# OFA-Sys/ONE-PEACE

Measured on AMD Instinct MI355X. Metric: pretrain samples/s (tri-modal global batch) ONE-PEACE-4B, higher is better.
Workload: dtype bf16

## Files before the change

include/onepeace_hip.h:

```cpp
#ifndef ONEPEACE_HIP_H
#define ONEPEACE_HIP_H

#include <stdint.h>

#ifdef __cplusplus
extern "C" {
#endif

int op_abi_version(void);
const char* op_last_error(void);

int op_prof_enable(int on);
int op_prof_reserve(int events);
int op_prof_collect(double* ms, int64_t* count, double* work, int n_families);

int op_layernorm_fwd(const void* x, const void* w, const void* b, void* y, float* mean, float* rstd, int64_t rows,
                     int64_t cols, float eps, int act_gelu, int dtype, const int* x_rows, void* stream);
int64_t op_layernorm_bwd_workspace_bytes(int64_t rows, int64_t cols);
int op_layernorm_bwd(const void* dy, const void* x, const void* w, const void* b, const float* mean, const float* rstd,
                     const void* add, void* dx, void* dw, void* db, void* workspace, int64_t rows, int64_t cols,
                     int act_gelu, int accumulate, int dtype, const int* x_rows, void* stream);

int op_gemm_nt(const void* A, int64_t lda, const void* B0, const void* B1, const void* B2, int64_t ldb, int64_t n_seg,
               const void* bias0, const void* bias1, const void* bias2, void* C, int64_t ldc, void* h0, void* h1,
               const void* resid, int64_t ldr, const void* gamma, const float* rowscale, int64_t rows_per_sample,
               const float* alpha, int64_t M, int64_t N, int64_t K, int epilogue, void* workspace, int64_t workspace_bytes,
               int64_t tune, const int* resid_rows, int64_t resid_rows_total, void* stream);
int op_gemm_tn(const void* A, int64_t lda, const void* B, int64_t ldb, void* C, int64_t ldc, int64_t M, int64_t N, int64_t K,
               int accumulate, void* workspace, int64_t workspace_bytes, int64_t tune, void* stream);
int op_gemm_nt_grouped(int64_t nprob, const void* const* A, const int64_t* M, int64_t lda, const void* const* B, int64_t ldb,
                       const void* const* bias, void* const* C, int64_t ldc, void* const* h0, void* const* h1,
                       const void* const* resid, int64_t ldr, const void* const* gamma, const float* const* rowscale,
                       const int64_t* rows_per_sample, int64_t N, int64_t K, int epilogue, int64_t tune, const int* const* resid_rows,
                       int64_t resid_rows_total, void* stream);
int op_gemm_nt_batched(const void* A, int64_t lda, int64_t stride_a, const void* W, int64_t ldb, int64_t stride_b, const void* bias,
                       int64_t stride_bias, void* C, int64_t ldc, int64_t stride_c, int64_t M, int64_t N, int64_t K, int64_t batch,
                       void* stream);
int op_audio_conv1_ln_gelu_fwd(const void* wav, int64_t stride, const void* w0, const void* b0, const void* lnw, const void* lnb, void* y,
                               float* mean, float* rstd, int64_t rows, int64_t C, float eps, void* stream);
int64_t op_audio_conv1_ln_gelu_bwd_workspace_bytes(int64_t C);
int op_audio_conv1_ln_gelu_bwd(const void* dy, const void* wav, int64_t stride, const void* w0, const void* b0, const void* lnw, const void* lnb,
                               const float* mean, const float* rstd, void* dw0, void* db0, void* dlnw, void* dlnb, void* workspace,
                               int64_t rows, int64_t C, int accumulate, void* stream);
int64_t op_gemm_tn_grouped_counter_bytes(void);
int64_t op_gemm_tn_grouped_plan(int64_t nprob, const int64_t* M, const int64_t* N, const int64_t* K, int64_t workgroups, int64_t tune,
                                int32_t* out, int64_t cap);
int op_gemm_tn_grouped(int64_t nprob, const void* const* A, const int64_t* lda, const void* const* B, const int64_t* ldb, void* const* C,
                       const int64_t* ldc, const int64_t* M, const int64_t* N, const int64_t* K, const int32_t* accumulate,
                       const void* const* W, const int64_t* ldw, float* const* rowdot, const void* const* rscale, void* counters,
                       int64_t tune, void* stream);
int op_gemm_tn_grouped_lists(int64_t nprob, const void* const* A, const int64_t* lda, const void* const* B, const int64_t* ldb, void* const* C,
                             const int64_t* ldc, const int64_t* M, const int64_t* N, const int64_t* K, const int32_t* accumulate,
                             const void* const* W, const int64_t* ldw, float* const* rowdot, const void* const* rscale,
                             const int32_t* const* ktiles, const int32_t* const* n_ktiles, void* counters, int64_t tune, void* stream);
int op_live_ktiles(int64_t nseg, const float* const* ps, const int64_t* row0, const int64_t* S, const int64_t* B, int64_t nprob,
                   const int64_t* prob_row0, const int64_t* prob_rows, int32_t* const* ktiles, int32_t* const* n_ktiles, void* stream);
int op_gemm_plan(int64_t M, int64_t N, int64_t K, int epilogue, int has_bias, int64_t workspace_bytes, int64_t tune, int* plan);

int op_quant_fp8_rows(const void* x, int64_t ldx, void* q, int64_t ldq, float* scale, int64_t rows, int64_t cols, void* stream);
int op_layernorm_fwd_q8(const void* x, const void* w, const void* b, void* y, float* mean, float* rstd, void* q8, float* q8_scale,
                        int64_t rows, int64_t cols, float eps, void* stream);
int op_ln_geglu_fwd_q8(const void* h0, const void* h1, int64_t ldh, const void* w, const void* b, void* y, float* mean, float* rstd, void* q8,
                       float* q8_scale, int64_t rows, int64_t cols, float eps, void* stream);
int op_gemm_nt_fp8(const void* A8, int64_t lda, const float* sa, const void* B0, const void* B1, int64_t ldb, const float* sb0,
                   const float* sb1, const void* bias, void* C, int64_t ldc, void* h0, void* h1, const void* resid, int64_t ldr,
                   const void* gamma, const float* rowscale, int64_t rows_per_sample, int64_t M, int64_t N, int64_t K, int epilogue,
                   int64_t tune, void* stream);

int op_attn_fwd(const void* q, const void* k, const void* v, int64_t ld, const void* bias, int64_t bias_batch_stride,
                const void* bias_frag, const void* key_pad, void* out, int64_t ldo, float* lse, int64_t lse_ld, int64_t B,
                int64_t S, int64_t Spad, int64_t heads, int64_t head_dim, float scale, int64_t tune, void* stream);
int64_t op_attn_bias_frag_elems(int64_t n_img, int64_t S);
int op_attn_bias_pack(const void* src, void* dst, int64_t n_img, int64_t S, int64_t Spad, void* stream);
int op_attn_bwd_delta(const void* dout, const void* out, int64_t ldo, float* delta, int64_t B, int64_t S, int64_t Spad,
                      int64_t heads, void* stream);
int64_t op_attn_bwd_dbias_slabs(int64_t B, int64_t S, int64_t heads, int64_t tune);
int op_attn_bwd(const void* q, const void* k, const void* v, int64_t ld, const void* dout, const void* out, int64_t ldo,
                const void* bias, const void* biasT, const void* bias_frag, int64_t bias_batch_stride, const void* key_pad,
                const float* lse, float* delta, void* dq,
                void* dk, void* dv, int64_t ldg, float* dbias, int64_t B, int64_t S, int64_t Spad, int64_t heads,
                int64_t head_dim, float scale, int64_t tune, void* stream);

int op_relpos_bias_build(const void* table, const int* bucket, int64_t bucket_ld, void* out, int64_t heads, int64_t S,
                         int64_t Spad, int transposed, void* stream);
int op_relpos_bias_bwd(const float* dbias, int64_t S, int64_t Spad, const int* pos, const int* seg, int64_t nseg, const int* bucket_seg,
                       int64_t num_rel, float* partial_ws, float* dtable, int64_t heads, void* stream);
int op_relpos_bias_build_ids(const void* table, const int* bucket, int64_t bucket_ld, const int* ids, void* out, int64_t B,
                             int64_t heads, int64_t K, int64_t Kpad, int transposed, void* stream);
int op_relpos_bias_fold_ids(const float* dbias, const int* ids, float* dense_ws, int64_t Sfull, int64_t B, int64_t heads, int64_t K,
                            int64_t Kpad, void* stream);

int op_transpose(const void* in, void* out, int64_t rows, int64_t cols, int64_t ld_in, int64_t ld_out, void* stream);
int op_transpose_scaled(const void* in, void* out, int64_t rows, int64_t cols, int64_t ld_in, int64_t ld_out, const void* scale,
                        void* stream);
int op_transpose_batched(const void* table, int64_t n, int64_t total_tiles, void* stream);
int64_t op_transpose_desc_bytes(void);
int64_t op_colsum_workspace_bytes(int64_t N);
int op_colsum_segments(const void* x, void* out0, void* out1, void* out2, void* workspace, int64_t M, int64_t n_seg,
                       int64_t seg_cols, int accumulate, void* stream);
int64_t op_resid_bwd_workspace_bytes(int64_t N);
int op_resid_bwd(const void* dout, const void* y, const void* gamma, const float* rowscale, int64_t rows_per_sample,
                 void* dbranch, void* dgamma, void* dbias, float* g0, void* workspace, int64_t M, int64_t N, int accumulate,
                 const int* dout_rows, void* stream);
int op_gamma_grad_finish(const float* rowdot, int64_t slots, const void* b0, const float* g00, const void* b1, const float* g01,
                         const void* b2, const float* g02, void* dgamma, int64_t N, int accumulate, void* stream);
int op_ln_geglu_bwd(const void* dy, const void* h0, const void* h1, const void* w, const float* mean, const float* rstd,
                    void* dh0, void* dh1, int64_t ldd, int64_t ldh, void* dw, void* db, void* workspace, int64_t rows,
                    int64_t cols, int accumulate, void* stream);
int op_ln_geglu_fwd(const void* h0, const void* h1, int64_t ldh, const void* w, const void* b, void* y, float* mean, float* rstd,
                    int64_t rows, int64_t cols, float eps, void* stream);
int op_colsum(const void* x, const void* y, const float* rowscale, int64_t rows_per_sample, const void* mul, void* out,
              void* workspace, int64_t M, int64_t N, int accumulate, int out_dtype, void* stream);
int op_geglu_bwd(const void* dg, const void* h0, const void* h1, void* dh0, void* dh1, int64_t numel, void* stream);
int op_scale_rows(const void* dout, const void* gamma, const float* rowscale, int64_t rows_per_sample, void* dbranch,
                  int64_t M, int64_t N, void* stream);

int op_l2norm_fwd(const void* x, void* y, float* inv_norm, int64_t rows, int64_t cols, float eps, int out_dtype, void* stream);
int op_l2norm_bwd(const void* dy, const void* y, const float* inv_norm, void* dx, int64_t rows, int64_t cols, int y_dtype,
                  void* stream);
int op_infonce_rows(float* sim, int64_t rows, int64_t n, int64_t ld, int64_t target0, float label_smoothing, float gscale,
                    float* row_loss, float* row_hit, float* row_dot, int write_grad, void* stream);

int op_adamw_step(void* p, const void* g, float* m, float* v, int64_t numel, float lr, float beta1, float beta2, float eps,
                  float weight_decay, int64_t step, float grad_scale, const float* grad_sqnorm, float clip_norm,
                  void* stream);
int op_adamw_step_groups(void* p, const void* g, float* m, float* v, int64_t numel, const int64_t* group_end8,
                         const float* group_lr_scale, const float* group_weight_decay, int64_t n_groups, float lr, float beta1,
                         float beta2, float eps, int64_t step, float grad_scale, const float* grad_sqnorm, float clip_norm,
                         void* stream);
int op_sqnorm(const void* x, int64_t numel, float* workspace, float* out, void* stream);

int op_rows_gather(const void* src, void* dst, const int* list, int64_t nseg, const int64_t* src_row0, const int64_t* dst_row0,
                   const int64_t* S, const int64_t* n_kept, const int64_t* dst_rows, const int64_t* n_samples, const int64_t* list_off,
                   int64_t dst_total, int64_t cols, void* stream);
int op_rows_merge(const void* base, const void* upd, void* out, const int* list, int64_t nseg, const int64_t* src_row0,
                  const int64_t* dst_row0, const int64_t* S, const int64_t* n_kept, const int64_t* dst_rows, const int64_t* n_samples,
                  const int64_t* list_off, int64_t total, int64_t cols, void* stream);
int op_rows_map(int* map, const int* list, int64_t nseg, const int64_t* src_row0, const int64_t* dst_row0, const int64_t* S,
                const int64_t* n_kept, const int64_t* dst_rows, const int64_t* n_samples, const int64_t* list_off, int64_t dst_total,
                void* stream);

int64_t op_sim_topk_splits(int64_t M, int64_t N, int64_t splits);
int64_t op_sim_topk_workspace_bytes(int64_t M, int64_t N, int64_t k, int64_t splits);
int op_sim_topk(const void* Q, int64_t ldq, const void* G, int64_t ldg, int64_t M, int64_t N, int64_t D, int64_t k, float* vals, int* idx,
                void* workspace, int64_t workspace_bytes, int64_t splits, void* stream);

int op_image_resize_normalize(const void* src, int64_t src_bytes, const int64_t* desc, const int64_t* desc_host, int64_t B,
                              const int* coef, int64_t coef_count, int64_t S, const float* mean, const float* stdev, void* out,
                              int out_dtype, void* workspace, int64_t workspace_bytes, void* stream);

int op_audio_normalize_pad(const void* src, int64_t src_bytes, const int64_t* desc, const int64_t* desc_host, int64_t B, int64_t max_len,
                           int64_t min_len, void* out, int64_t T, int out_dtype, void* workspace, int64_t workspace_bytes, void* stream);

int op_audio_resample(const void* src, int64_t src_bytes, const int64_t* desc, const int64_t* desc_host, int64_t B, const float* coef,
                      int64_t coef_count, void* out, int64_t out_bytes, void* stream);

int64_t op_average_precision_workspace_bytes(int64_t N, int64_t C);
int op_average_precision(const float* scores, int64_t ld_scores, const uint8_t* targets, int64_t ld_targets, int64_t N, int64_t C,
                         double* ap, int* npos, void* workspace, int64_t workspace_bytes, void* stream);

int op_row_loss(const void* logits, int dtype, int64_t ld, const void* targets, int target_dtype, int64_t ld_targets, int64_t B, int64_t C,
                int mode, float label_smoothing, float margin, float gscale, float* row_loss, float* row_correct, float* dlogits,
                float* sums, void* stream);
int op_box_loss(const void* logits, int dtype, const float* targets, int64_t B, float gscale, float* out, float* dlogits, void* stream);

#ifdef __cplusplus
}
#endif
#endif
```

one-peace_amd/csrc/layernorm.hip:

```cpp
#include "common.h"

namespace {

constexpr int LN_MAX_BLOCKS = 4096;
constexpr int g_ln_blocks_fwd = 512, g_ln_blocks_bwd = 512;
#ifndef OP_LN_GEGLU_BLOCKS_FWD
#define OP_LN_GEGLU_BLOCKS_FWD 2048
#endif
#ifndef OP_LN_GEGLU_BLOCKS_BWD
#define OP_LN_GEGLU_BLOCKS_BWD 512
#endif

template <int NW>
__device__ __forceinline__ float group_sum(float v, float* red) {
  v = wave_sum(v);
  if (NW == 1) return v;
  const int wid = threadIdx.x >> 6;
  __syncthreads();
  if ((threadIdx.x & 63) == 0) red[wid] = v;
  __syncthreads();
  float t = 0.f;
#pragma unroll
  for (int i = 0; i < NW; ++i) t += red[i];
  return t;
}

template <int NW>
__device__ __forceinline__ void group_sum2(float& a, float& b, float* red) {
  a = wave_sum(a);
  b = wave_sum(b);
  if (NW == 1) return;
  const int wid = threadIdx.x >> 6;
  __syncthreads();
  if ((threadIdx.x & 63) == 0) { red[wid] = a; red[NW + wid] = b; }
  __syncthreads();
  float ta = 0.f, tb = 0.f;
#pragma unroll
  for (int i = 0; i < NW; ++i) { ta += red[i]; tb += red[NW + i]; }
  a = ta;
  b = tb;
}

template <int NW>
__device__ __forceinline__ float group_amax(int m, float* red) {
  const float v = fp8_wave_amax(m);
  if (NW == 1) return v;
  const int wid = threadIdx.x >> 6;
  __syncthreads();
  if ((threadIdx.x & 63) == 0) red[wid] = v;
  __syncthreads();
  int t = __float_as_int(red[0]);
#pragma unroll
  for (int i = 1; i < NW; ++i) t = max(t, __float_as_int(red[i]));
  return __int_as_float(t);
}

template <typename T, int CH, int NW, bool GELU, bool NT, bool Q8 = false>
__global__ __launch_bounds__(256) void ln_fwd_kernel(const T* __restrict__ x, const T* __restrict__ w,
                                                     const T* __restrict__ b, T* __restrict__ y,
                                                     float* __restrict__ mean_out, float* __restrict__ rstd_out,
                                                     int64_t rows, int cols, float eps, uint8_t* __restrict__ q8 = nullptr,
                                                     float* __restrict__ q8_scale = nullptr, const int* __restrict__ xmap = nullptr) {
  __shared__ float red[4];
  constexpr int G = 64 * NW;
  const int tig = (NW == 1) ? (threadIdx.x & 63) : threadIdx.x;
  const int64_t row0 = (NW == 1) ? ((int64_t)blockIdx.x * 4 + (threadIdx.x >> 6)) : blockIdx.x;
  const int64_t rstep = (NW == 1) ? (int64_t)gridDim.x * 4 : gridDim.x;
  const float inv = 1.0f / (float)cols;

  float wv[CH][8], bv[CH][8];
#pragma unroll
  for (int i = 0; i < CH; ++i) {
    const int c = (tig + G * i) * 8;
#pragma unroll
    for (int j = 0; j < 8; ++j) { wv[i][j] = 1.f; bv[i][j] = 0.f; }
    if (c < cols) {
      if (w) Vec8<T>::load(w + c, wv[i]);
      if (b) Vec8<T>::load(b + c, bv[i]);
    }
  }
  typedef typename Vec8<T>::raw_t raw_t;
  raw_t cur[CH], nxt[CH];
  auto fetch = [&](int64_t src, raw_t (&dst)[CH]) {
#pragma unroll
    for (int i = 0; i < CH; ++i) {
      const int c = (tig + G * i) * 8;
      if (c < cols) {
        if (src >= 0) dst[i] = ldraw_sel<T, NT>(x + src * (int64_t)cols + c);
        else dst[i] = raw_t{};
      }
    }
  };
  int64_t nsrc = row0 + rstep < rows ? (xmap ? (int64_t)xmap[row0 + rstep] : row0 + rstep) : -1;
  if (row0 < rows) fetch(xmap ? (int64_t)xmap[row0] : row0, cur);
  for (int64_t row = row0; row < rows; row += rstep) {
    const int64_t nrow = row + rstep, nnrow = nrow + rstep;
    if (nrow < rows) fetch(nsrc, nxt);
    if (nnrow < rows) nsrc = xmap ? (int64_t)xmap[nnrow] : nnrow;
    float v[CH][8];
    float s = 0.f;
#pragma unroll
    for (int i = 0; i < CH; ++i) {
      const int c = (tig + G * i) * 8;
      if (c < cols) {
        Vec8<T>::cvt(cur[i], v[i]);
#pragma unroll
        for (int j = 0; j < 8; ++j) s += v[i][j];
      } else {
#pragma unroll
        for (int j = 0; j < 8; ++j) v[i][j] = 0.f;
      }
    }
    const float mean = group_sum<NW>(s, red) * inv;
    float ss = 0.f;
#pragma unroll
    for (int i = 0; i < CH; ++i) {
      const int c = (tig + G * i) * 8;
      if (c < cols) {
#pragma unroll
        for (int j = 0; j < 8; ++j) { const float d = v[i][j] - mean; ss += d * d; }
      }
    }
    const float rstd = rsqrtf(group_sum<NW>(ss, red) * inv + eps);
    T* yr = y + row * (int64_t)cols;
    int amax = 0;
#pragma unroll
    for (int i = 0; i < CH; ++i) {
      const int c = (tig + G * i) * 8;
      if (c < cols) {
        float o[8];
#pragma unroll
        for (int j = 0; j < 8; ++j) {
          float t = (v[i][j] - mean) * rstd * wv[i][j] + bv[i][j];
          o[j] = GELU ? gelu_erf(t) : t;
        }
        store_sel<T, NT>(yr + c, o);
        if constexpr (Q8) {
#pragma unroll
          for (int j = 0; j < 8; ++j) { v[i][j] = (float)(T)o[j]; amax = fp8_amax_acc(amax, v[i][j]); }
        }
      }
    }
    if constexpr (Q8) {
      float qinv;
      const float sc = fp8_row_scale(group_amax<NW>(amax, red), qinv);
      uint8_t* qr = q8 + row * (int64_t)cols;
#pragma unroll
      for (int i = 0; i < CH; ++i) {
        const int c = (tig + G * i) * 8;
        if (c < cols) *reinterpret_cast<u32x2*>(qr + c) = fp8_pack8(v[i], qinv);
      }
      if (tig == 0) q8_scale[row] = sc;
    }
    if (tig == 0) {
      if (mean_out) mean_out[row] = mean;
      if (rstd_out) rstd_out[row] = rstd;
    }
#pragma unroll
    for (int i = 0; i < CH; ++i) cur[i] = nxt[i];
  }
}

template <int CH, int NW, bool Q8 = false>
__global__ __launch_bounds__(NW == 1 ? 256 : 64 * NW) void ln_geglu_fwd_kernel(const bf16_t* __restrict__ h0, const bf16_t* __restrict__ h1,
                                                           int64_t ldh, const bf16_t* __restrict__ w, const bf16_t* __restrict__ b,
                                                           bf16_t* __restrict__ y, float* __restrict__ mean_out,
                                                           float* __restrict__ rstd_out, int64_t rows, int cols, float eps,
                                                           uint8_t* __restrict__ q8 = nullptr, float* __restrict__ q8_scale = nullptr) {
  __shared__ float red[4];
  constexpr int G = 64 * NW;
  const int tig = (NW == 1) ? (threadIdx.x & 63) : threadIdx.x;
  const int64_t row0 = (NW == 1) ? ((int64_t)blockIdx.x * 4 + (threadIdx.x >> 6)) : blockIdx.x;
  const int64_t rstep = (NW == 1) ? (int64_t)gridDim.x * 4 : gridDim.x;
  const float inv = 1.0f / (float)cols;
  float wv[CH][8], bv[CH][8];
#pragma unroll
  for (int i = 0; i < CH; ++i) {
    const int c = (tig + G * i) * 8;
#pragma unroll
    for (int j = 0; j < 8; ++j) { wv[i][j] = 1.f; bv[i][j] = 0.f; }
    if (c < cols) {
      if (w) Vec8<bf16_t>::load(w + c, wv[i]);
      if (b) Vec8<bf16_t>::load(b + c, bv[i]);
    }
  }
  bf16x8 c0[CH], c1[CH], n0[CH], n1[CH];
  if (row0 < rows) {
#pragma unroll
    for (int i = 0; i < CH; ++i) {
      const int c = (tig + G * i) * 8;
      if (c < cols) {
        c0[i] = Vec8<bf16_t>::ldraw_nt(h0 + row0 * ldh + c);
        c1[i] = Vec8<bf16_t>::ldraw_nt(h1 + row0 * ldh + c);
      }
    }
  }
  for (int64_t row = row0; row < rows; row += rstep) {
    const int64_t nrow = row + rstep;
    if (nrow < rows) {
#pragma unroll
      for (int i = 0; i < CH; ++i) {
        const int c = (tig + G * i) * 8;
        if (c < cols) {
          n0[i] = Vec8<bf16_t>::ldraw_nt(h0 + nrow * ldh + c);
          n1[i] = Vec8<bf16_t>::ldraw_nt(h1 + nrow * ldh + c);
        }
      }
    }
    float v[CH][8];
    float s = 0.f;
#pragma unroll
    for (int i = 0; i < CH; ++i) {
      const int c = (tig + G * i) * 8;
      if (c < cols) {
        float a[8], bb[8];
        Vec8<bf16_t>::cvt(c0[i], a);
        Vec8<bf16_t>::cvt(c1[i], bb);
#pragma unroll
        for (int j = 0; j < 8; ++j) {
          v[i][j] = (float)(bf16_t)(gelu_erf(a[j]) * bb[j]);
          s += v[i][j];
        }
      } else {
#pragma unroll
        for (int j = 0; j < 8; ++j) v[i][j] = 0.f;
      }
    }
    const float mean = group_sum<NW>(s, red) * inv;
    float ss = 0.f;
#pragma unroll
    for (int i = 0; i < CH; ++i) {
      const int c = (tig + G * i) * 8;
      if (c < cols) {
#pragma unroll
        for (int j = 0; j < 8; ++j) { const float d = v[i][j] - mean; ss += d * d; }
      }
    }
    const float rstd = rsqrtf(group_sum<NW>(ss, red) * inv + eps);
    bf16_t* yr = y + row * (int64_t)cols;
    int amax = 0;
#pragma unroll
    for (int i = 0; i < CH; ++i) {
      const int c = (tig + G * i) * 8;
      if (c < cols) {
        float o[8];
#pragma unroll
        for (int j = 0; j < 8; ++j) o[j] = (v[i][j] - mean) * rstd * wv[i][j] + bv[i][j];
        Vec8<bf16_t>::store_nt(yr + c, o);
        if constexpr (Q8) {
#pragma unroll
          for (int j = 0; j < 8; ++j) { v[i][j] = (float)(bf16_t)o[j]; amax = fp8_amax_acc(amax, v[i][j]); }
        }
      }
    }
    if constexpr (Q8) {
      float qinv;
      const float sc = fp8_row_scale(group_amax<NW>(amax, red), qinv);
      uint8_t* qr = q8 + row * (int64_t)cols;
#pragma unroll
      for (int i = 0; i < CH; ++i) {
        const int c = (tig + G * i) * 8;
        if (c < cols) *reinterpret_cast<u32x2*>(qr + c) = fp8_pack8(v[i], qinv);
      }
      if (tig == 0) q8_scale[row] = sc;
    }
    if (tig == 0) {
      if (mean_out) mean_out[row] = mean;
      if (rstd_out) rstd_out[row] = rstd;
    }
#pragma unroll
    for (int i = 0; i < CH; ++i) { c0[i] = n0[i]; c1[i] = n1[i]; }
  }
}

template <typename T, int CH, int NW, bool GELU, bool NT>
__global__ __launch_bounds__(256) void ln_bwd_kernel(const T* __restrict__ dy, const T* __restrict__ x,
                                                     const T* __restrict__ w, const T* __restrict__ b,
                                                     const float* __restrict__ mean_in,
                                                     const float* __restrict__ rstd_in, const T* __restrict__ add,
                                                     T* __restrict__ dx, float* __restrict__ ws, int64_t rows, int cols,
                                                     const int* __restrict__ xmap = nullptr) {
  extern __shared__ __attribute__((aligned(16))) float smem[];
  float* red = smem;
  constexpr int G = 64 * NW;
  const int tig = (NW == 1) ? (threadIdx.x & 63) : threadIdx.x;
  const int wid = threadIdx.x >> 6;
  const int64_t row0 = (NW == 1) ? ((int64_t)blockIdx.x * 4 + wid) : blockIdx.x;
  const int64_t rstep = (NW == 1) ? (int64_t)gridDim.x * 4 : gridDim.x;
  const float inv = 1.0f / (float)cols;

  float wv[CH][8], bv[CH][8], dwa[CH][8], dba[CH][8];
#pragma unroll
  for (int i = 0; i < CH; ++i) {
    const int c = (tig + G * i) * 8;
#pragma unroll
    for (int j = 0; j < 8; ++j) { wv[i][j] = 1.f; bv[i][j] = 0.f; dwa[i][j] = 0.f; dba[i][j] = 0.f; }
    if (c < cols) {
      if (w) Vec8<T>::load(w + c, wv[i]);
      if (GELU && b) Vec8<T>::load(b + c, bv[i]);
    }
  }
  typedef typename Vec8<T>::raw_t raw_t;
  raw_t curx[CH], curg[CH], nxtx[CH], nxtg[CH], addv[CH];
  int64_t src = row0 < rows ? (xmap ? (int64_t)xmap[row0] : row0) : -1;
  int64_t nsrc = row0 + rstep < rows ? (xmap ? (int64_t)xmap[row0 + rstep] : row0 + rstep) : -1, nnsrc = -1;
  if (row0 < rows) {
#pragma unroll
    for (int i = 0; i < CH; ++i) {
      const int c = (tig + G * i) * 8;
      if (c < cols) {
        if (src >= 0) curx[i] = ldraw_sel<T, NT>(x + src * (int64_t)cols + c);
        else curx[i] = raw_t{};
        curg[i] = ldraw_sel<T, NT>(dy + row0 * (int64_t)cols + c);
      }
    }
  }
  for (int64_t row = row0; row < rows; row += rstep) {
    const float mean = mean_in[row], rstd = rstd_in[row];
    const int64_t nrow = row + rstep, nnrow = nrow + rstep;
    if (nnrow < rows) nnsrc = xmap ? (int64_t)xmap[nnrow] : nnrow;
#pragma unroll
    for (int i = 0; i < CH; ++i) {
      const int c = (tig + G * i) * 8;
      if (c < cols) {
        if (add && src >= 0) addv[i] = ldraw_sel<T, NT>(add + src * (int64_t)cols + c);
        if (nrow < rows) {
          if (nsrc >= 0) nxtx[i] = ldraw_sel<T, NT>(x + nsrc * (int64_t)cols + c);
          else nxtx[i] = raw_t{};
          nxtg[i] = ldraw_sel<T, NT>(dy + nrow * (int64_t)cols + c);
        }
      }
    }
    float xh[CH][8], g[CH][8];
    float s1 = 0.f, s2 = 0.f;
#pragma unroll
    for (int i = 0; i < CH; ++i) {
      const int c = (tig + G * i) * 8;
      if (c < cols) {
        Vec8<T>::cvt(curx[i], xh[i]);
        Vec8<T>::cvt(curg[i], g[i]);
#pragma unroll
        for (int j = 0; j < 8; ++j) {
          xh[i][j] = (xh[i][j] - mean) * rstd;
          if (GELU) g[i][j] *= gelu_erf_grad(xh[i][j] * wv[i][j] + bv[i][j]);
          dwa[i][j] += g[i][j] * xh[i][j];
          dba[i][j] += g[i][j];
          const float gw = g[i][j] * wv[i][j];
          g[i][j] = gw;
          s1 += gw;
          s2 += gw * xh[i][j];
        }
      }
    }
    group_sum2<NW>(s1, s2, red);
    const float c1 = s1 * inv, c2 = s2 * inv;
    T* dr = dx + (src >= 0 ? src : 0) * (int64_t)cols;
#pragma unroll
    for (int i = 0; i < CH; ++i) {
      const int c = (tig + G * i) * 8;
      if (c < cols && src >= 0) {
        float o[8];
#pragma unroll
        for (int j = 0; j < 8; ++j) o[j] = rstd * (g[i][j] - c1 - xh[i][j] * c2);
        if (add) {
          float av[8];
          Vec8<T>::cvt(addv[i], av);
#pragma unroll
          for (int j = 0; j < 8; ++j) o[j] += av[j];
        }
        store_sel<T, NT>(dr + c, o);
      }
    }
#pragma unroll
    for (int i = 0; i < CH; ++i) { curx[i] = nxtx[i]; curg[i] = nxtg[i]; }
    src = nsrc;
    nsrc = nnsrc;
  }
  if (ws == nullptr) return;
  float* wsb = ws + (int64_t)blockIdx.x * 2 * cols;
  if (NW == 1) {
#pragma unroll
    for (int pass = 0; pass < 2; ++pass) {
      __syncthreads();
#pragma unroll
      for (int i = 0; i < CH; ++i) {
        const int c = (tig + G * i) * 8;
        if (c < cols) {
#pragma unroll
          for (int j = 0; j < 8; ++j) smem[wid * cols + c + j] = pass == 0 ? dwa[i][j] : dba[i][j];
        }
      }
      __syncthreads();
      for (int c = threadIdx.x; c < cols; c += 256)
        wsb[pass * cols + c] = smem[c] + smem[cols + c] + smem[2 * cols + c] + smem[3 * cols + c];
    }
  } else {
#pragma unroll
    for (int i = 0; i < CH; ++i) {
      const int c = (tig + G * i) * 8;
      if (c < cols) {
#pragma unroll
        for (int j = 0; j < 8; ++j) { wsb[c + j] = dwa[i][j]; wsb[cols + c + j] = dba[i][j]; }
      }
    }
  }
}

template <int CH, int NW>
__global__ __launch_bounds__(NW == 1 ? 256 : 64 * NW) void ln_geglu_bwd_kernel(const bf16_t* __restrict__ dy, const bf16_t* __restrict__ h0,
                                                           const bf16_t* __restrict__ h1, const bf16_t* __restrict__ w,
                                                           const float* __restrict__ mean_in,
                                                           const float* __restrict__ rstd_in, bf16_t* __restrict__ dh0,
                                                           bf16_t* __restrict__ dh1, int64_t ldd, int64_t ldh, float* __restrict__ ws,
                                                           int64_t rows, int cols) {
  extern __shared__ __attribute__((aligned(16))) float smem[];
  float* red = smem;
  constexpr int G = 64 * NW;
  const int tig = (NW == 1) ? (threadIdx.x & 63) : threadIdx.x;
  const int wid = threadIdx.x >> 6;
  const int64_t row0 = (NW == 1) ? ((int64_t)blockIdx.x * 4 + wid) : blockIdx.x;
  const int64_t rstep = (NW == 1) ? (int64_t)gridDim.x * 4 : gridDim.x;
  const float inv = 1.0f / (float)cols;
  float dwa[CH][8], dba[CH][8];
  bf16x8 wraw[CH];
#pragma unroll
  for (int i = 0; i < CH; ++i) {
    const int c = (tig + G * i) * 8;
#pragma unroll
    for (int j = 0; j < 8; ++j) { dwa[i][j] = 0.f; dba[i][j] = 0.f; }
#pragma unroll
    for (int j = 0; j < 8; ++j) wraw[i][j] = (bf16_t)1.0f;
    if (c < cols && w) wraw[i] = Vec8<bf16_t>::ldraw(w + c);
  }
  bf16x8 r0[CH], r1[CH], rg[CH], n0[CH], n1[CH], ng[CH];
  if (row0 < rows) {
#pragma unroll
    for (int i = 0; i < CH; ++i) {
      const int c = (tig + G * i) * 8;
      if (c < cols) {
        r0[i] = Vec8<bf16_t>::ldraw_nt(h0 + row0 * ldh + c);
        r1[i] = Vec8<bf16_t>::ldraw_nt(h1 + row0 * ldh + c);
        rg[i] = Vec8<bf16_t>::ldraw_nt(dy + row0 * (int64_t)cols + c);
      }
    }
  }
  for (int64_t row = row0; row < rows; row += rstep) {
    const float mean = mean_in[row], rstd = rstd_in[row];
    const int64_t base = row * (int64_t)cols;
    const int64_t nrow = row + rstep;
    if (nrow < rows) {
#pragma unroll
      for (int i = 0; i < CH; ++i) {
        const int c = (tig + G * i) * 8;
        if (c < cols) {
          n0[i] = Vec8<bf16_t>::ldraw_nt(h0 + nrow * ldh + c);
          n1[i] = Vec8<bf16_t>::ldraw_nt(h1 + nrow * ldh + c);
          ng[i] = Vec8<bf16_t>::ldraw_nt(dy + nrow * (int64_t)cols + c);
        }
      }
    }
    float gw[CH][8], cdfs[CH][8], gps[CH][8];
    float s1 = 0.f, s2 = 0.f;
#pragma unroll
    for (int i = 0; i < CH; ++i) {
      const int c = (tig + G * i) * 8;
      if (c < cols) {
        float a[8], b[8];
        Vec8<bf16_t>::cvt(r0[i], a);
        Vec8<bf16_t>::cvt(r1[i], b);
        Vec8<bf16_t>::cvt(rg[i], gw[i]);
        float wv[8];
        asm volatile("" : "+v"(wraw[i]));
        Vec8<bf16_t>::cvt(wraw[i], wv);
#pragma unroll
        for (int j = 0; j < 8; ++j) {
          float cdf, pdf;
          gelu_parts(a[j], cdf, pdf);
          cdfs[i][j] = cdf;
          gps[i][j] = cdf + a[j] * pdf;
          const float gval = (float)(bf16_t)(a[j] * cdf * b[j]);
          const float xh = (gval - mean) * rstd;
          const float d = gw[i][j];
          dwa[i][j] += d * xh;
          dba[i][j] += d;
          const float t = d * wv[j];
          gw[i][j] = t;
          s1 += t;
          s2 += t * xh;
        }
      }
    }
    group_sum2<NW>(s1, s2, red);
    const float c1 = s1 * inv, c2 = s2 * inv;
#pragma unroll
    for (int i = 0; i < CH; ++i) {
      const int c = (tig + G * i) * 8;
      if (c < cols) {
        float a[8], b[8], o0[8], o1[8];
        Vec8<bf16_t>::cvt(r0[i], a);
        Vec8<bf16_t>::cvt(r1[i], b);
#pragma unroll
        for (int j = 0; j < 8; ++j) {
          const float ge = a[j] * cdfs[i][j];
          const float xh = ((float)(bf16_t)(ge * b[j]) - mean) * rstd;
          const float dg = rstd * (gw[i][j] - c1 - xh * c2);
          o0[j] = dg * b[j] * gps[i][j];
          o1[j] = dg * ge;
        }
        Vec8<bf16_t>::store_nt(dh0 + row * ldd + c, o0);
        Vec8<bf16_t>::store_nt(dh1 + row * ldd + c, o1);
      }
    }
#pragma unroll
    for (int i = 0; i < CH; ++i) { r0[i] = n0[i]; r1[i] = n1[i]; rg[i] = ng[i]; }
  }
  if (ws == nullptr) return;
  float* wsb = ws + (int64_t)blockIdx.x * 2 * cols;
  if (NW == 1) {
#pragma unroll
    for (int pass = 0; pass < 2; ++pass) {
      __syncthreads();
#pragma unroll
      for (int i = 0; i < CH; ++i) {
        const int c = (tig + G * i) * 8;
        if (c < cols) {
#pragma unroll
          for (int j = 0; j < 8; ++j) smem[wid * cols + c + j] = pass == 0 ? dwa[i][j] : dba[i][j];
        }
      }
      __syncthreads();
      for (int c = threadIdx.x; c < cols; c += 256)
        wsb[pass * cols + c] = smem[c] + smem[cols + c] + smem[2 * cols + c] + smem[3 * cols + c];
    }
  } else {
#pragma unroll
    for (int i = 0; i < CH; ++i) {
      const int c = (tig + G * i) * 8;
      if (c < cols) {
#pragma unroll
        for (int j = 0; j < 8; ++j) { wsb[c + j] = dwa[i][j]; wsb[cols + c + j] = dba[i][j]; }
      }
    }
  }
}

inline int ln_grid(int64_t rows, int nw, int cap) {
  int64_t blocks = nw == 1 ? (rows + 3) / 4 : rows;
  if (blocks > cap) blocks = cap;
  if (blocks < 1) blocks = 1;
  return (int)blocks;
}

template <typename T, bool GELU>
int ln_fwd_dispatch(const void* x, const void* w, const void* b, void* y, float* mean, float* rstd, int64_t rows,
                    int cols, float eps, hipStream_t s, const int* xmap = nullptr) {
  const T* X = (const T*)x; const T* W = (const T*)w; const T* B = (const T*)b; T* Y = (T*)y;
  const bool nt = mean != nullptr && (int64_t)rows * cols * (int64_t)sizeof(T) >= ((int64_t)64 << 20);
#define LN_F(CH, NW)                                                                                                                      \
  do {                                                                                                                                    \
    if (nt) hipLaunchKernelGGL((ln_fwd_kernel<T, CH, NW, GELU, true>), dim3(ln_grid(rows, NW, g_ln_blocks_fwd)), dim3(256), 0, s, X, W, B, Y, mean, rstd, rows, cols, eps, (uint8_t*)nullptr, (float*)nullptr, xmap); \
    else hipLaunchKernelGGL((ln_fwd_kernel<T, CH, NW, GELU, false>), dim3(ln_grid(rows, NW, g_ln_blocks_fwd)), dim3(256), 0, s, X, W, B, Y, mean, rstd, rows, cols, eps, (uint8_t*)nullptr, (float*)nullptr, xmap); \
  } while (0)
  if (cols <= 512) LN_F(1, 1);
  else if (cols <= 1024) LN_F(2, 1);
  else if (cols <= 1536) LN_F(3, 1);
  else if (cols <= 2048) LN_F(4, 1);
  else if (cols <= 4096) LN_F(2, 4);
  else if (cols <= 6144) LN_F(3, 4);
  else if (cols <= 8192) LN_F(4, 4);
  else { op_set_error("layernorm: cols %d > 8192 unsupported", cols); return OP_ENOTSUP; }
#undef LN_F
  OP_LAUNCH_CHECK();
  return OP_OK;
}

template <typename T, bool GELU>
int ln_bwd_dispatch(const void* dy, const void* x, const void* w, const void* b, const float* mean, const float* rstd,
                    const void* add, void* dx, void* dw, void* db, float* ws, int64_t rows, int cols, int accumulate,
                    hipStream_t s, const int* xmap = nullptr) {
  const T* DY = (const T*)dy; const T* X = (const T*)x; const T* W = (const T*)w; const T* B = (const T*)b; T* DX = (T*)dx;
  const T* ADD = (const T*)add;
  int grid = 0;
  float* wsk = (dw || db) ? ws : nullptr;
  const bool nt = (int64_t)rows * cols * (int64_t)sizeof(T) >= ((int64_t)64 << 20);
#define LN_B(CH, NW)                                                                                        \
  do {                                                                                                      \
    grid = ln_grid(rows, NW, g_ln_blocks_bwd);                                                                               \
    size_t sh = (NW == 1) ? (size_t)4 * cols * sizeof(float) : 64;                                          \
    if (nt) hipLaunchKernelGGL((ln_bwd_kernel<T, CH, NW, GELU, true>), dim3(grid), dim3(256), sh, s, DY, X, W, B, mean,   \
                       rstd, ADD, DX, wsk, rows, cols, xmap);                                                    \
    else hipLaunchKernelGGL((ln_bwd_kernel<T, CH, NW, GELU, false>), dim3(grid), dim3(256), sh, s, DY, X, W, B, mean,   \
                       rstd, ADD, DX, wsk, rows, cols, xmap);                                                    \
  } while (0)
  if (cols <= 512) LN_B(1, 1);
  else if (cols <= 1024) LN_B(2, 1);
  else if (cols <= 1536) LN_B(3, 1);
  else if (cols <= 2048) LN_B(4, 1);
  else if (cols <= 4096) LN_B(2, 4);
  else if (cols <= 6144) LN_B(3, 4);
  else if (cols <= 8192) LN_B(4, 4);
  else { op_set_error("layernorm: cols %d > 8192 unsupported", cols); return OP_ENOTSUP; }
#undef LN_B
  OP_LAUNCH_CHECK();
  if (wsk) {
    hipLaunchKernelGGL((partials_reduce3_kernel<T>), dim3(ceil_div(cols, 32), 2), dim3(256), 0, s, ws, ws + cols,
                       (const float*)nullptr, (const bf16_t*)nullptr, (const bf16_t*)nullptr, (const bf16_t*)nullptr, (T*)dw,
                       (T*)db, (T*)nullptr, grid, (int64_t)2 * cols, cols, accumulate);
    OP_LAUNCH_CHECK();
  }
  return OP_OK;
}

}

extern "C" {


int64_t op_layernorm_bwd_workspace_bytes(int64_t rows, int64_t cols) {
  (void)rows;
  return (int64_t)LN_MAX_BLOCKS * 2 * cols * (int64_t)sizeof(float);
}

int op_layernorm_fwd(const void* x, const void* w, const void* b, void* y, float* mean, float* rstd, int64_t rows,
                     int64_t cols, float eps, int act_gelu, int dtype, const int* x_rows, void* stream) {
  OP_CHECK_ARG(x && y, "layernorm_fwd: null x/y");
  OP_CHECK_ARG(rows >= 0 && cols > 0 && cols % 8 == 0, "layernorm_fwd: cols=%lld must be a positive multiple of 8",
               (long long)cols);
  if (rows == 0) return OP_OK;
  hipStream_t s = (hipStream_t)stream;
  if (dtype == OP_DT_BF16)
    return act_gelu ? ln_fwd_dispatch<bf16_t, true>(x, w, b, y, mean, rstd, rows, (int)cols, eps, s, x_rows)
                    : ln_fwd_dispatch<bf16_t, false>(x, w, b, y, mean, rstd, rows, (int)cols, eps, s, x_rows);
  if (dtype == OP_DT_F32)
    return act_gelu ? ln_fwd_dispatch<float, true>(x, w, b, y, mean, rstd, rows, (int)cols, eps, s, x_rows)
                    : ln_fwd_dispatch<float, false>(x, w, b, y, mean, rstd, rows, (int)cols, eps, s, x_rows);
  op_set_error("layernorm_fwd: bad dtype %d", dtype);
  return OP_EINVAL;
}

int op_layernorm_fwd_q8(const void* x, const void* w, const void* b, void* y, float* mean, float* rstd, void* q8, float* q8_scale,
                        int64_t rows, int64_t cols, float eps, void* stream) {
  OP_CHECK_ARG(x && y && q8 && q8_scale, "layernorm_fwd_q8: null pointer");
  OP_CHECK_ARG(rows >= 0 && cols > 0 && cols % 8 == 0 && cols <= 8192, "layernorm_fwd_q8: cols=%lld unsupported", (long long)cols);
  if (rows == 0) return OP_OK;
  hipStream_t s = (hipStream_t)stream;
#define LN_Q(CH, NW)                                                                                                                         \
  hipLaunchKernelGGL((ln_fwd_kernel<bf16_t, CH, NW, false, false, true>), dim3(ln_grid(rows, NW, g_ln_blocks_fwd)), dim3(256), 0, s,        \
                     (const bf16_t*)x, (const bf16_t*)w, (const bf16_t*)b, (bf16_t*)y, mean, rstd, rows, (int)cols, eps, (uint8_t*)q8, q8_scale)
  if (cols <= 512) LN_Q(1, 1);
  else if (cols <= 1024) LN_Q(2, 1);
  else if (cols <= 1536) LN_Q(3, 1);
  else if (cols <= 2048) LN_Q(4, 1);
  else if (cols <= 4096) LN_Q(2, 4);
  else if (cols <= 6144) LN_Q(3, 4);
  else LN_Q(4, 4);
#undef LN_Q
  OP_LAUNCH_CHECK();
  return OP_OK;
}

int op_layernorm_bwd(const void* dy, const void* x, const void* w, const void* b, const float* mean, const float* rstd,
                     const void* add, void* dx, void* dw, void* db, void* workspace, int64_t rows, int64_t cols,
                     int act_gelu, int accumulate, int dtype, const int* x_rows, void* stream) {
  OP_CHECK_ARG(dy && x && dx && mean && rstd, "layernorm_bwd: null pointer");
  OP_CHECK_ARG(rows >= 0 && cols > 0 && cols % 8 == 0, "layernorm_bwd: cols=%lld must be a positive multiple of 8",
               (long long)cols);
  OP_CHECK_ARG(!(dw || db) || workspace, "layernorm_bwd: dw/db requested without workspace");
  if (rows == 0) return OP_OK;
  hipStream_t s = (hipStream_t)stream;
  if (dtype == OP_DT_BF16)
    return act_gelu ? ln_bwd_dispatch<bf16_t, true>(dy, x, w, b, mean, rstd, add, dx, dw, db, (float*)workspace, rows,
                                                    (int)cols, accumulate, s, x_rows)
                    : ln_bwd_dispatch<bf16_t, false>(dy, x, w, b, mean, rstd, add, dx, dw, db, (float*)workspace, rows,
                                                     (int)cols, accumulate, s, x_rows);
  if (dtype == OP_DT_F32)
    return act_gelu ? ln_bwd_dispatch<float, true>(dy, x, w, b, mean, rstd, add, dx, dw, db, (float*)workspace, rows,
                                                   (int)cols, accumulate, s, x_rows)
                    : ln_bwd_dispatch<float, false>(dy, x, w, b, mean, rstd, add, dx, dw, db, (float*)workspace, rows,
                                                    (int)cols, accumulate, s, x_rows);
  op_set_error("layernorm_bwd: bad dtype %d", dtype);
  return OP_EINVAL;
}

int op_ln_geglu_fwd(const void* h0, const void* h1, int64_t ldh, const void* w, const void* b, void* y, float* mean, float* rstd,
                    int64_t rows, int64_t cols, float eps, void* stream) {
  OP_CHECK_ARG(h0 && h1 && y, "ln_geglu_fwd: null pointer");
  if (ldh <= 0) ldh = cols;
  OP_CHECK_ARG(rows >= 0 && cols > 0 && cols % 8 == 0 && cols <= 8192 && ldh >= cols && ldh % 8 == 0, "ln_geglu_fwd: cols=%lld ldh=%lld unsupported",
               (long long)cols, (long long)ldh);
  if (rows == 0) return OP_OK;
  hipStream_t s = (hipStream_t)stream;
#define LNG_F(CH, NW)                                                                                                       \
  hipLaunchKernelGGL((ln_geglu_fwd_kernel<CH, NW>), dim3(ln_grid(rows, NW, OP_LN_GEGLU_BLOCKS_FWD)), dim3(NW == 1 ? 256 : 64 * NW), 0, s, \
                     (const bf16_t*)h0, (const bf16_t*)h1, ldh, (const bf16_t*)w, (const bf16_t*)b, (bf16_t*)y, mean, rstd, rows, \
                     (int)cols, eps)
  if (cols <= 512) LNG_F(1, 1);
  else if (cols <= 1024) LNG_F(2, 1);
  else if (cols <= 1536) LNG_F(3, 1);
  else if (cols <= 2048) LNG_F(4, 1);
  else if (cols <= 4096) LNG_F(2, 4);
  else if (cols <= 6144) LNG_F(3, 4);
  else LNG_F(4, 4);
#undef LNG_F
  OP_LAUNCH_CHECK();
  return OP_OK;
}

int op_ln_geglu_fwd_q8(const void* h0, const void* h1, int64_t ldh, const void* w, const void* b, void* y, float* mean, float* rstd, void* q8,
                       float* q8_scale, int64_t rows, int64_t cols, float eps, void* stream) {
  OP_CHECK_ARG(h0 && h1 && y && q8 && q8_scale, "ln_geglu_fwd_q8: null pointer");
  if (ldh <= 0) ldh = cols;
  OP_CHECK_ARG(rows >= 0 && cols > 0 && cols % 8 == 0 && cols <= 8192 && ldh >= cols && ldh % 8 == 0, "ln_geglu_fwd_q8: cols=%lld ldh=%lld unsupported",
               (long long)cols, (long long)ldh);
  if (rows == 0) return OP_OK;
  hipStream_t s = (hipStream_t)stream;
#define LNG_Q(CH, NW)                                                                                                       \
  hipLaunchKernelGGL((ln_geglu_fwd_kernel<CH, NW, true>), dim3(ln_grid(rows, NW, OP_LN_GEGLU_BLOCKS_FWD)), dim3(NW == 1 ? 256 : 64 * NW), 0, s, \
                     (const bf16_t*)h0, (const bf16_t*)h1, ldh, (const bf16_t*)w, (const bf16_t*)b, (bf16_t*)y, mean, rstd, rows, \
                     (int)cols, eps, (uint8_t*)q8, q8_scale)
  if (cols <= 512) LNG_Q(1, 1);
  else if (cols <= 1024) LNG_Q(2, 1);
  else if (cols <= 1536) LNG_Q(3, 1);
  else if (cols <= 2048) LNG_Q(4, 1);
  else if (cols <= 4096) LNG_Q(2, 4);
  else if (cols <= 6144) LNG_Q(3, 4);
  else LNG_Q(4, 4);
#undef LNG_Q
  OP_LAUNCH_CHECK();
  return OP_OK;
}

int op_ln_geglu_bwd(const void* dy, const void* h0, const void* h1, const void* w, const float* mean, const float* rstd,
                    void* dh0, void* dh1, int64_t ldd, int64_t ldh, void* dw, void* db, void* workspace, int64_t rows, int64_t cols,
                    int accumulate, void* stream) {
  OP_CHECK_ARG(dy && h0 && h1 && dh0 && dh1 && mean && rstd, "ln_geglu_bwd: null pointer");
  if (ldd <= 0) ldd = cols;
  if (ldh <= 0) ldh = cols;
  OP_CHECK_ARG(ldd >= cols && ldd % 8 == 0 && ldh >= cols && ldh % 8 == 0, "ln_geglu_bwd: row strides %lld / %lld", (long long)ldd, (long long)ldh);
  OP_CHECK_ARG(rows >= 0 && cols > 0 && cols % 8 == 0 && cols <= 8192, "ln_geglu_bwd: cols=%lld unsupported", (long long)cols);
  OP_CHECK_ARG(!(dw || db) || workspace, "ln_geglu_bwd: dw/db requested without workspace");
  if (rows == 0) return OP_OK;
  hipStream_t s = (hipStream_t)stream;
  float* wsk = (dw || db) ? (float*)workspace : nullptr;
  int grid = 0;
#define LNG_B(CH, NW)                                                                                              \
  do {                                                                                                             \
    grid = ln_grid(rows, NW, OP_LN_GEGLU_BLOCKS_BWD);                                                                     \
    size_t sh = (NW == 1) ? (size_t)4 * cols * sizeof(float) : 64;                                                 \
    hipLaunchKernelGGL((ln_geglu_bwd_kernel<CH, NW>), dim3(grid), dim3(NW == 1 ? 256 : 64 * NW), sh, s,           \
                       (const bf16_t*)dy, (const bf16_t*)h0, (const bf16_t*)h1, (const bf16_t*)w, mean, rstd,      \
                       (bf16_t*)dh0, (bf16_t*)dh1, ldd, ldh, wsk, rows, (int)cols);                                \
  } while (0)
  if (cols <= 512) LNG_B(1, 1);
  else if (cols <= 1024) LNG_B(2, 1);
  else if (cols <= 1536) LNG_B(3, 1);
  else if (cols <= 2048) LNG_B(4, 1);
  else if (cols <= 4096) LNG_B(2, 4);
  else if (cols <= 6144) LNG_B(3, 4);
  else LNG_B(4, 4);
#undef LNG_B
  OP_LAUNCH_CHECK();
  if (wsk) {
    hipLaunchKernelGGL((partials_reduce3_kernel<bf16_t>), dim3(ceil_div(cols, 32), 2), dim3(256), 0, s, wsk, wsk + cols,
                       (const float*)nullptr, (const bf16_t*)nullptr, (const bf16_t*)nullptr, (const bf16_t*)nullptr,
                       (bf16_t*)dw, (bf16_t*)db, (bf16_t*)nullptr, grid, (int64_t)2 * cols, (int)cols, accumulate);
    OP_LAUNCH_CHECK();
  }
  return OP_OK;
}

}
```

one-peace_amd/hip.py:

```python
import ctypes
import os
from ctypes import c_double, c_float, c_int, c_int64, c_void_p

import torch

_HERE = os.path.dirname(os.path.abspath(__file__))
LIB_PATH = os.environ.get("ONEPEACE_HIP_LIB") or os.path.join(_HERE, "lib", "libonepeace_hip.so")
_lib = None

DT_BF16, DT_F32 = 0, 1
EPI_BIAS, EPI_F32, EPI_GEGLU, EPI_RESID = 0, 1, 2, 3
PROF_GEMM, PROF_ATTN = 0, 1
ATTN_RESIDENT_MAX_S = 320

P = c_void_p
I64 = c_int64

SIGNATURES = {
    "op_abi_version": (c_int, []),
    "op_last_error": (ctypes.c_char_p, []),
    "op_prof_enable": (c_int, [c_int]),
    "op_prof_reserve": (c_int, [c_int]),
    "op_prof_collect": (c_int, [P, P, P, c_int]),
    "op_layernorm_fwd": (c_int, [P, P, P, P, P, P, I64, I64, c_float, c_int, c_int, P, P]),
    "op_layernorm_bwd_workspace_bytes": (I64, [I64, I64]),
    "op_attn_bwd_dbias_slabs": (I64, [I64, I64, I64, I64]),
    "op_layernorm_bwd": (c_int, [P, P, P, P, P, P, P, P, P, P, P, I64, I64, c_int, c_int, c_int, P, P]),
    "op_gemm_plan": (c_int, [c_int64, c_int64, c_int64, c_int, c_int, c_int64, I64, P]),
    "op_gemm_nt": (c_int, [P, I64, P, P, P, I64, I64, P, P, P, P, I64, P, P, P, I64, P, P, I64, P, I64, I64, I64,
                           c_int, P, I64, I64, P, I64, P]),
    "op_gemm_nt_grouped": (c_int, [I64, P, P, I64, P, I64, P, P, I64, P, P, P, I64, P, P, P, I64, I64, c_int, I64, P, I64, P]),
    "op_gemm_tn": (c_int, [P, I64, P, I64, P, I64, I64, I64, I64, c_int, P, I64, I64, P]),
    "op_gemm_tn_grouped_counter_bytes": (I64, []),
    "op_gemm_tn_grouped_plan": (I64, [I64, P, P, P, I64, I64, P, I64]),
    "op_gemm_tn_grouped": (c_int, [I64, P, P, P, P, P, P, P, P, P, P, P, P, P, P, P, I64, P]),
    "op_gemm_tn_grouped_lists": (c_int, [I64, P, P, P, P, P, P, P, P, P, P, P, P, P, P, P, P, P, I64, P]),
    "op_live_ktiles": (c_int, [I64, P, P, P, P, I64, P, P, P, P, P]),
    "op_gemm_nt_batched": (c_int, [P, I64, I64, P, I64, I64, P, I64, P, I64, I64, I64, I64, I64, I64, P]),
    "op_audio_conv1_ln_gelu_fwd": (c_int, [P, I64, P, P, P, P, P, P, P, I64, I64, c_float, P]),
    "op_audio_conv1_ln_gelu_bwd_workspace_bytes": (I64, [I64]),
    "op_audio_conv1_ln_gelu_bwd": (c_int, [P, P, I64, P, P, P, P, P, P, P, P, P, P, P, I64, I64, c_int, P]),
    "op_transpose": (c_int, [P, P, I64, I64, I64, I64, P]),
    "op_transpose_scaled": (c_int, [P, P, I64, I64, I64, I64, P, P]),
    "op_transpose_batched": (c_int, [P, I64, I64, P]),
    "op_transpose_desc_bytes": (I64, []),
    "op_colsum_workspace_bytes": (I64, [I64]),
    "op_colsum_segments": (c_int, [P, P, P, P, P, I64, I64, I64, c_int, P]),
    "op_resid_bwd_workspace_bytes": (I64, [I64]),
    "op_resid_bwd": (c_int, [P, P, P, P, I64, P, P, P, P, P, I64, I64, c_int, P, P]),
    "op_gamma_grad_finish": (c_int, [P, I64, P, P, P, P, P, P, P, I64, c_int, P]),
    "op_ln_geglu_bwd": (c_int, [P, P, P, P, P, P, P, P, I64, I64, P, P, P, I64, I64, c_int, P]),
    "op_ln_geglu_fwd": (c_int, [P, P, I64, P, P, P, P, P, I64, I64, c_float, P]),
    "op_colsum": (c_int, [P, P, P, I64, P, P, P, I64, I64, c_int, c_int, P]),
    "op_geglu_bwd": (c_int, [P, P, P, P, P, I64, P]),
    "op_scale_rows": (c_int, [P, P, P, I64, P, I64, I64, P]),
    "op_l2norm_fwd": (c_int, [P, P, P, I64, I64, c_float, c_int, P]),
    "op_l2norm_bwd": (c_int, [P, P, P, P, I64, I64, c_int, P]),
    "op_infonce_rows": (c_int, [P, I64, I64, I64, I64, c_float, c_float, P, P, P, c_int, P]),
    "op_adamw_step": (c_int, [P, P, P, P, I64, c_float, c_float, c_float, c_float, c_float, I64, c_float, P, c_float, P]),
    "op_adamw_step_groups": (c_int, [P, P, P, P, I64, P, P, P, I64, c_float, c_float, c_float, c_float, I64, c_float, P, c_float, P]),
    "op_sqnorm": (c_int, [P, I64, P, P, P]),
    "op_relpos_bias_build": (c_int, [P, P, I64, P, I64, I64, I64, c_int, P]),
    "op_relpos_bias_bwd": (c_int, [P, I64, I64, P, P, I64, P, I64, P, P, I64, P]),
    "op_relpos_bias_build_ids": (c_int, [P, P, I64, P, P, I64, I64, I64, I64, c_int, P]),
    "op_relpos_bias_fold_ids": (c_int, [P, P, P, I64, I64, I64, I64, I64, P]),
    "op_attn_fwd": (c_int, [P, P, P, I64, P, I64, P, P, P, I64, P, I64, I64, I64, I64, I64, I64, c_float, I64, P]),
    "op_attn_bias_frag_elems": (I64, [I64, I64]),
    "op_attn_bias_pack": (c_int, [P, P, I64, I64, I64, P]),
    "op_attn_bwd_delta": (c_int, [P, P, I64, P, I64, I64, I64, I64, P]),
    "op_attn_bwd": (c_int, [P, P, P, I64, P, P, I64, P, P, P, I64, P, P, P, P, P, P, I64, P, I64, I64, I64, I64, I64, c_float, I64, P]),
    "op_quant_fp8_rows": (c_int, [P, I64, P, I64, P, I64, I64, P]),
    "op_layernorm_fwd_q8": (c_int, [P, P, P, P, P, P, P, P, I64, I64, c_float, P]),
    "op_ln_geglu_fwd_q8": (c_int, [P, P, I64, P, P, P, P, P, P, P, I64, I64, c_float, P]),
    "op_gemm_nt_fp8": (c_int, [P, I64, P, P, P, I64, P, P, P, P, I64, P, P, P, I64, P, P, I64, I64, I64, I64, c_int, I64, P]),
    "op_rows_gather": (c_int, [P, P, P, I64, P, P, P, P, P, P, P, I64, I64, P]),
    "op_rows_merge": (c_int, [P, P, P, P, I64, P, P, P, P, P, P, P, I64, I64, P]),
    "op_rows_map": (c_int, [P, P, I64, P, P, P, P, P, P, P, I64, P]),
    "op_sim_topk_splits": (I64, [I64, I64, I64]),
    "op_sim_topk_workspace_bytes": (I64, [I64, I64, I64, I64]),
    "op_sim_topk": (c_int, [P, I64, P, I64, I64, I64, I64, I64, P, P, P, I64, I64, P]),
    "op_image_resize_normalize": (c_int, [P, I64, P, P, I64, P, I64, I64, P, P, P, c_int, P, I64, P]),
    "op_audio_normalize_pad": (c_int, [P, I64, P, P, I64, I64, I64, P, I64, c_int, P, I64, P]),
    "op_audio_resample": (c_int, [P, I64, P, P, I64, P, I64, P, I64, P]),
    "op_average_precision_workspace_bytes": (I64, [I64, I64]),
    "op_average_precision": (c_int, [P, I64, P, I64, I64, I64, P, P, P, I64, P]),
    "op_row_loss": (c_int, [P, c_int, I64, P, c_int, I64, I64, I64, c_int, c_float, c_float, c_float, P, P, P, P, P]),
    "op_box_loss": (c_int, [P, c_int, P, I64, c_float, P, P, P]),
}


PROBE_SIGNATURES = {
    "op_last_error": (ctypes.c_char_p, []),
    "op_probe_mfma16": (c_int, [P, P, P, c_int, P]),
    "op_probe_mfma32": (c_int, [P, P, P, c_int, P]),
    "op_probe_tr16": (c_int, [P, P, P, c_int, P]),
    "op_probe_glds": (c_int, [P, P, c_int, P, P]),
    "op_probe_mfma_f8": (c_int, [P, P, P, P, P, c_int, P]),
    "op_probe_mfma_rate": (c_int, [P, P, P, c_int, c_int, P]),
    "op_probe_lds_atomic": (c_int, [P, P, c_int, c_int, c_int, P]),
    "op_probe_occupy": (c_int, [P, ctypes.c_longlong, c_int, ctypes.c_longlong, P, P]),
}


class Tuning:

    def __init__(self):
        self.reset()

    def reset(self):
        self.tile_mode = 0
        self.fullline = 2
        self.tail_rows = 1
        self.gm = 0
        self.force_splits = 0
        self.glds = 1
        self.sched = int(os.environ.get("ONEPEACE_TUNE_SCHED", "0"))
        self.fp8_small = 0
        self.merge_dbias = 1
        self.resident = 1
        self.attn_waves = 0
        self.attn_pers = 1
        self.dbias_chunks_r2 = 0
        self.dkdv_keys = 0
        self.dbias_chunks = 0
        self.attn_pers_dkdv = 1
        self.attn_lone_keys = 1
        self.attn_pers_bwd = 1

    def gemm(self):
        fl = {2: 0, 0: 1, 1: 2, 3: 3}.get(self.fullline, 0)
        tr = 0 if self.tail_rows == 1 else self.tail_rows + 1
        return (self.tile_mode | fl << 2 | tr << 4 | (self.gm & 31) << 7 | (self.force_splits & 15) << 15
                | (0 if self.glds else 1) << 19 | (self.sched & 7) << 20)

    def attn_fwd(self):
        return (0 if self.resident & 1 else 1) | ((self.resident >> 1) & 3) << 1 | (self.attn_waves & 15) << 3 | (0 if self.attn_pers else 128)

    def attn_bwd(self):
        return ((0 if self.merge_dbias else 1) | (2 if self.dbias_chunks_r2 else 0) | (self.dkdv_keys & 3) << 2 | (self.dbias_chunks & 63) << 4
                | (0 if self.attn_pers_bwd else 1024) | (0 if self.attn_lone_keys else 2048) | (0 if self.attn_pers_dkdv else 4096))


TUNE = Tuning()


class _LibProxy:

    def __init__(self, cdll):
        self._cdll = cdll

    def __getattr__(self, name):
        return getattr(self._cdll, name)

    @staticmethod
    def op_gemm_set_tile(mode):
        old = TUNE.tile_mode
        if mode >= 60:
            TUNE.force_splits = mode - 60
        elif mode >= 50:
            TUNE.tail_rows = mode - 50
        elif mode >= 40:
            TUNE.gm = mode - 40
        elif mode >= 20:
            if 0 <= mode - 20 <= 3:
                TUNE.fullline = mode - 20
        elif mode >= 10:
            pass
        else:
            TUNE.tile_mode = mode
        return old

    @staticmethod
    def op_gemm_set_staging(glds):
        old, TUNE.glds = TUNE.glds, 1 if glds else 0
        return old

    @staticmethod
    def op_attn_set_merge_dbias(on):
        old, TUNE.merge_dbias = TUNE.merge_dbias, 1 if on else 0
        return old

    @staticmethod
    def op_attn_set_resident(mode):
        old, TUNE.resident = TUNE.resident, int(mode)
        return old


def lib():
    global _lib
    if _lib is None:
        if not os.path.exists(LIB_PATH):
            raise RuntimeError(
                "%s not found: build it with `python one-peace_amd/build.py` (hipcc, gfx950). "
                "There is no CPU fallback for the HIP path." % LIB_PATH)
        L = ctypes.CDLL(LIB_PATH)
        for name, (res, args) in SIGNATURES.items():
            fn = getattr(L, name)
            fn.restype = res
            fn.argtypes = args
        _lib = _LibProxy(L)
    return _lib


_probe_lib = None


def probe_lib():
    global _probe_lib
    if _probe_lib is None:
        path = os.path.join(os.path.dirname(LIB_PATH), "libonepeace_probe.so")
        if not os.path.exists(path):
            raise RuntimeError("%s not found: build it with `python one-peace_amd/build.py`" % path)
        L = ctypes.CDLL(path)
        for name, (res, args) in PROBE_SIGNATURES.items():
            fn = getattr(L, name)
            fn.restype = res
            fn.argtypes = args
        _probe_lib = L
    return _probe_lib


def _check_probe(rc, what):
    if rc != 0:
        msg = probe_lib().op_last_error()
        raise RuntimeError("%s failed (rc=%d): %s" % (what, rc, msg.decode() if msg else ""))


def available():
    return os.path.exists(LIB_PATH) and torch.cuda.is_available()


def _check(rc, what):
    if rc != 0:
        msg = lib().op_last_error()
        raise RuntimeError("%s failed (rc=%d): %s" % (what, rc, msg.decode() if msg else ""))


def ptr(t):
    return None if t is None else c_void_p(t.data_ptr())


def stream():
    return c_void_p(torch.cuda.current_stream().cuda_stream)


def _dt(t):
    if t.dtype == torch.bfloat16:
        return DT_BF16
    if t.dtype == torch.float32:
        return DT_F32
    raise TypeError("unsupported dtype %s" % t.dtype)


def _req(t, name, dtype=None):
    if t is None:
        return
    if not t.is_cuda:
        raise RuntimeError("%s must be a CUDA(HIP) tensor" % name)
    if not t.is_contiguous():
        raise RuntimeError("%s must be contiguous" % name)
    if dtype is not None and t.dtype != dtype:
        raise TypeError("%s must be %s, got %s" % (name, dtype, t.dtype))


def layernorm_fwd(x2d, w, b, eps=1e-5, gelu=False, want_stats=True, q8=False, x_rows=None):
    _req(x2d, "x")
    rows, cols = x2d.shape
    if x_rows is not None:
        assert not q8 and x_rows.dtype == torch.int32 and x_rows.is_contiguous()
        rows = x_rows.numel()
    y = torch.empty(rows, cols, dtype=x2d.dtype, device=x2d.device)
    mean = rstd = None
    if want_stats:
        mean = torch.empty(rows, dtype=torch.float32, device=x2d.device)
        rstd = torch.empty(rows, dtype=torch.float32, device=x2d.device)
    if q8:
        assert not gelu and x2d.dtype == torch.bfloat16
        q = torch.empty(rows, cols, dtype=torch.uint8, device=x2d.device)
        qs = torch.empty(rows, dtype=torch.float32, device=x2d.device)
        _check(lib().op_layernorm_fwd_q8(ptr(x2d), ptr(w), ptr(b), ptr(y), ptr(mean), ptr(rstd), ptr(q), ptr(qs), rows, cols, eps, stream()),
               "op_layernorm_fwd_q8")
        return y, mean, rstd, (q, qs)
    _check(lib().op_layernorm_fwd(ptr(x2d), ptr(w), ptr(b), ptr(y), ptr(mean), ptr(rstd), rows, cols, eps,
                                  int(gelu), _dt(x2d), ptr(x_rows), stream()), "op_layernorm_fwd")
    return y, mean, rstd


_ws_cache = {}


def workspace(nbytes, device, tag="ws"):
    key = (device, tag, torch.cuda.current_stream(device).cuda_stream)
    buf = _ws_cache.get(key)
    if buf is None or buf.numel() < nbytes:
        buf = torch.empty(max(int(nbytes), 1 << 20), dtype=torch.uint8, device=device)
        _ws_cache[key] = buf
    return buf


def layernorm_bwd(dy, x, w, b, mean, rstd, gelu=False, need_wgrad=True, dw=None, db=None, accumulate=False, add=None,
                  dx=None, x_rows=None):
    rows, cols = x.shape
    if x_rows is not None:
        assert dx is not None and dx.shape == x.shape and (add is None or add.shape == x.shape) and x_rows.dtype == torch.int32
        rows = x_rows.numel()
        assert dy.shape[0] == rows
    if dx is None:
        dx = torch.empty_like(x)
    ws = None
    if need_wgrad and w is not None:
        if dw is None:
            dw = torch.empty_like(w)
            db = torch.empty_like(w)
            accumulate = False
        ws = workspace(lib().op_layernorm_bwd_workspace_bytes(rows, cols), x.device, "ln")
    else:
        dw = db = None
    _check(lib().op_layernorm_bwd(ptr(dy), ptr(x), ptr(w), ptr(b), ptr(mean), ptr(rstd), ptr(add), ptr(dx), ptr(dw), ptr(db),
                                  ptr(ws), rows, cols, int(gelu), int(accumulate), _dt(x), ptr(x_rows), stream()), "op_layernorm_bwd")
    return dx, dw, db


SPLITK_WS_BYTES = 768 << 20
GEMM_ALGO_BYTES = [0, 0]


def gemm_nt(A, Bs, biases=None, out=None, epilogue=EPI_BIAS, n_seg=0, h0=None, h1=None, resid=None, gamma=None,
            rowscale=None, rows_per_sample=0, alpha=None, N=None, ldc=None, splitk=True, resid_rows=None):
    M, K = A.shape
    if resid_rows is not None:
        assert epilogue == EPI_RESID and out is not None and resid is not None and out.shape == resid.shape and resid_rows.numel() == M
        assert resid_rows.dtype == torch.int32 and resid_rows.is_contiguous()
    Bs = list(Bs) + [None] * (3 - len(Bs))
    biases = list(biases or []) + [None] * (3 - len(biases or []))
    if epilogue == EPI_GEGLU:
        Nn = Bs[0].shape[0]
    else:
        Nn = N if N is not None else sum(b.shape[0] for b in Bs if b is not None)
        if n_seg == 0:
            n_seg = Bs[0].shape[0]
    if out is None:
        out = torch.empty(M, Nn, dtype=torch.float32 if epilogue == EPI_F32 else torch.bfloat16, device=A.device)
    ldc_ = ldc if ldc is not None else out.stride(0)
    ws, ws_bytes = None, 0
    if splitk and epilogue in (EPI_BIAS, EPI_RESID) and (K >= 2048 or M <= 1024):
        ws = workspace(min(SPLITK_WS_BYTES, 32 * M * Nn), A.device, "gemm_splitk")
        ws_bytes = ws.numel()
    outs = 1 + (2 if h1 is not None else (1 if h0 is not None else 0))
    GEMM_ALGO_BYTES[0] += 2 * (M * K + Nn * K * (2 if epilogue == EPI_GEGLU else 1) + (M * Nn if resid is not None else 0)) \
        + out.element_size() * M * Nn * outs
    GEMM_ALGO_BYTES[1] += 1
    _check(lib().op_gemm_nt(ptr(A), A.stride(0), ptr(Bs[0]), ptr(Bs[1]), ptr(Bs[2]), Bs[0].stride(0), n_seg,
                            ptr(biases[0]), ptr(biases[1]), ptr(biases[2]), ptr(out), ldc_, ptr(h0), ptr(h1),
                            ptr(resid), resid.stride(0) if resid is not None else 0, ptr(gamma), ptr(rowscale),
                            rows_per_sample, ptr(alpha), M, Nn, K, epilogue, ptr(ws), ws_bytes, TUNE.gemm(), ptr(resid_rows),
                            out.shape[0] if resid_rows is not None else 0, stream()), "op_gemm_nt")
    return out


def _ptr_array(items, n):
    arr = (c_void_p * n)()
    for i, t in enumerate(items or ()):
        arr[i] = None if t is None else t.data_ptr()
    return arr


def gemm_nt_grouped(As, Ws, biases=None, outs=None, epilogue=EPI_BIAS, h0s=None, h1s=None, resids=None, gammas=None,
                    rowscales=None, rows_per_sample=None, resid_rows=None):
    n = len(As)
    K = As[0].shape[1]
    pairs = [w if isinstance(w, (tuple, list)) else (w, None) for w in Ws]
    N = pairs[0][0].shape[0]
    if outs is None:
        outs = [torch.empty(a.shape[0], N, dtype=torch.bfloat16, device=a.device) for a in As]
    lda, ldb, ldc = As[0].stride(0), pairs[0][0].stride(0), outs[0].stride(0)
    ldr = resids[0].stride(0) if resids and resids[0] is not None else 0
    if any(a.stride(0) != lda or a.shape[1] != K for a in As) or any(w[0].stride(0) != ldb or w[0].shape != (N, K) for w in pairs) \
            or any(o.stride(0) != ldc for o in outs) or (ldr and any(r.stride(0) != ldr for r in resids)):
        return None
    flatB, flatb = [], []
    for i, (w0, w1) in enumerate(pairs):
        flatB += [w0, w1]
        flatb += [biases[i] if biases else None, None]
    Ms = (c_int64 * n)(*[a.shape[0] for a in As])
    rps = (c_int64 * n)(*[(rows_per_sample[i] if rows_per_sample else 0) for i in range(n)])
    for i, a in enumerate(As):
        outs_n = 1 + (2 if h1s and h1s[i] is not None else (1 if h0s and h0s[i] is not None else 0))
        GEMM_ALGO_BYTES[0] += 2 * (a.shape[0] * K + N * K * (2 if epilogue == EPI_GEGLU else 1)
                                   + (a.shape[0] * N if resids and resids[i] is not None else 0)) + 2 * a.shape[0] * N * outs_n
    GEMM_ALGO_BYTES[1] += 1
    rc = lib().op_gemm_nt_grouped(n, _ptr_array(As, n), Ms, lda, _ptr_array(flatB, 2 * n), ldb, _ptr_array(flatb, 2 * n),
                                  _ptr_array(outs, n), ldc, _ptr_array(h0s, n), _ptr_array(h1s, n), _ptr_array(resids, n), ldr,
                                  _ptr_array(gammas, n), _ptr_array(rowscales, n), rps, N, K, epilogue, TUNE.gemm(),
                                  _ptr_array(resid_rows, n) if resid_rows is not None else None,
                                  outs[0].shape[0] if resid_rows is not None else 0, stream())
    if rc == -95:
        return None
    _check(rc, "op_gemm_nt_grouped")
    return outs


def quant_fp8_rows(x2d, out=None):
    rows, cols = x2d.shape
    if out is not None:
        q, scale = out
    else:
        q = torch.empty(rows, cols, dtype=torch.uint8, device=x2d.device)
        scale = torch.empty(rows, dtype=torch.float32, device=x2d.device)
    _check(lib().op_quant_fp8_rows(ptr(x2d), x2d.stride(0), ptr(q), q.stride(0), ptr(scale), rows, cols, stream()), "op_quant_fp8_rows")
    return q, scale


def gemm_nt_fp8(A8, sa, B8s, sbs, bias=None, out=None, epilogue=EPI_BIAS, h0=None, h1=None, resid=None, gamma=None, rowscale=None,
                rows_per_sample=0):
    M, K = A8.shape
    N = B8s[0].shape[0]
    if out is None:
        out = torch.empty(M, N, dtype=torch.bfloat16, device=A8.device)
    B1, sb1 = (B8s[1], sbs[1]) if len(B8s) > 1 else (None, None)
    _check(lib().op_gemm_nt_fp8(ptr(A8), A8.stride(0), ptr(sa), ptr(B8s[0]), ptr(B1), B8s[0].stride(0), ptr(sbs[0]), ptr(sb1),
                                ptr(bias), ptr(out), out.stride(0), ptr(h0), ptr(h1), ptr(resid),
                                resid.stride(0) if resid is not None else 0, ptr(gamma), ptr(rowscale), rows_per_sample, M, N, K,
                                epilogue, int(TUNE.fp8_small), stream()), "op_gemm_nt_fp8")
    return out


def gemm_plan(M, N, K, epilogue=EPI_BIAS, has_bias=True, workspace_bytes=SPLITK_WS_BYTES):
    out = (ctypes.c_int * 4)()
    _check(lib().op_gemm_plan(M, N, K, epilogue, int(has_bias), workspace_bytes, TUNE.gemm(), ctypes.cast(out, P)), "op_gemm_plan")
    return out[0], out[1], bool(out[2]), out[3]


def gemm_tn_supported(K, M, N, lda, ldb, ldc=0):
    return (K % 64 == 0 and M % 8 == 0 and N % 8 == 0 and lda % 8 == 0 and ldb % 8 == 0 and ldc % 8 == 0 and M >= 8 and N >= 8
            and 31 * lda + M < (1 << 30) and 31 * ldb + N < (1 << 30))


def gemm_nt_batched(A, W, bias, out, rows, K):
    G, N = W.shape[0], W.shape[1]
    assert W.is_contiguous() and out.is_contiguous() and out.shape == (G, rows, N) and A.stride(2) == 1
    GEMM_ALGO_BYTES[0] += 2 * G * (rows * K + N * K + rows * N)
    GEMM_ALGO_BYTES[1] += 1
    _check(lib().op_gemm_nt_batched(ptr(A), A.stride(1), A.stride(0), ptr(W), K, N * K, ptr(bias), N if bias is not None else 0, ptr(out), N,
                                    rows * N, rows, N, K, G, stream()), "op_gemm_nt_batched")
    return out


def audio_conv1_ln_gelu_fwd(wav, stride, w0, b0, lnw, lnb, rows, eps, slack_rows=0):
    C = w0.shape[0]
    assert w0.is_contiguous() and w0.numel() == C * 10 and wav.is_contiguous() and wav.numel() >= stride * (rows - 1) + 10
    y = torch.empty(rows + slack_rows, C, dtype=torch.bfloat16, device=wav.device)
    if slack_rows:
        y[rows:].zero_()
    mean = torch.empty(rows, dtype=torch.float32, device=wav.device)
    rstd = torch.empty(rows, dtype=torch.float32, device=wav.device)
    _check(lib().op_audio_conv1_ln_gelu_fwd(ptr(wav), stride, ptr(w0), ptr(b0), ptr(lnw), ptr(lnb), ptr(y), ptr(mean), ptr(rstd), rows, C, eps,
                                            stream()), "op_audio_conv1_ln_gelu_fwd")
    return y, mean, rstd


def audio_conv1_ln_gelu_bwd(dy, wav, stride, w0, b0, lnw, lnb, mean, rstd):
    rows, C = dy.shape
    mk = lambda ref, shape: torch.empty(shape, dtype=torch.bfloat16, device=dy.device) if ref is not None else None
    dw0, db0, dlw, dlb = torch.empty(C, 10, dtype=torch.bfloat16, device=dy.device), mk(b0, C), mk(lnw, C), mk(lnb, C)
    ws = workspace(lib().op_audio_conv1_ln_gelu_bwd_workspace_bytes(C), dy.device, "audio_conv1")
    _check(lib().op_audio_conv1_ln_gelu_bwd(ptr(dy), ptr(wav), stride, ptr(w0), ptr(b0), ptr(lnw), ptr(lnb), ptr(mean), ptr(rstd), ptr(dw0), ptr(db0),
                                            ptr(dlw), ptr(dlb), ptr(ws), rows, C, 0, stream()), "op_audio_conv1_ln_gelu_bwd")
    return dw0, db0, dlw, dlb


def gemm_tn_grouped_plan(sizes, workgroups=256, tune=0):
    n = len(sizes)
    cap = sum(((m + 255) // 256) * ((nn + 255) // 256) for m, nn, _ in sizes)
    out = (ctypes.c_int32 * (4 * cap))()
    arr = lambda j: (c_int64 * n)(*[q[j] for q in sizes])
    cnt = lib().op_gemm_tn_grouped_plan(n, arr(0), arr(1), arr(2), int(workgroups), int(tune), ctypes.cast(out, P), cap)
    if cnt < 0:
        raise RuntimeError("op_gemm_tn_grouped_plan failed (%d)" % cnt)
    return [tuple(out[4 * i:4 * i + 4]) for i in range(cnt)]


def gemm_tn(A_km, B_kn, out=None, accumulate=False, splitk=True):
    K, M = A_km.shape
    N = B_kn.shape[1]
    if out is None:
        out = torch.empty(M, N, dtype=torch.bfloat16, device=A_km.device)
        accumulate = False
    ws = workspace(SPLITK_WS_BYTES, A_km.device, "gemm_splitk") if splitk else None
    GEMM_ALGO_BYTES[0] += 2 * (K * M + K * N + M * N * (2 if accumulate else 1))
    GEMM_ALGO_BYTES[1] += 1
    _check(lib().op_gemm_tn(ptr(A_km), A_km.stride(0), ptr(B_kn), B_kn.stride(0), ptr(out), out.stride(0), M, N, K,
                            int(accumulate), ptr(ws), ws.numel() if ws is not None else 0, TUNE.gemm(), stream()), "op_gemm_tn")
    return out


_tn_counters = {}
TN_GROUP_MAX = 16


def live_ktiles(segs, probs, device):
    ns, n = len(segs), len(probs)
    sizes = [rows // 64 for _, rows in probs]
    buf = torch.empty(sum(sizes) + n, dtype=torch.int32, device=device)
    lists, off = [], n
    for p, k in enumerate(sizes):
        lists.append((buf[off:off + k], buf[p:p + 1]))
        off += k
    i64 = lambda k, vals: (c_int64 * k)(*[int(v) for v in vals])
    for ps, _, _, B in segs:
        assert ps is None or (ps.dtype == torch.float32 and ps.is_contiguous() and ps.numel() >= B and ps.device == buf.device)
    _check(lib().op_live_ktiles(ns, _ptr_array([q[0] for q in segs], ns), i64(ns, [q[1] for q in segs]), i64(ns, [q[2] for q in segs]),
                                i64(ns, [q[3] for q in segs]), n, i64(n, [q[0] for q in probs]), i64(n, [q[1] for q in probs]),
                                _ptr_array([q[0] for q in lists], n), _ptr_array([q[1] for q in lists], n), stream()), "op_live_ktiles")
    return lists


def gemm_tn_grouped(problems, tune=0, ktiles=None):
    n = len(problems)
    dev = problems[0][0].device
    key = (dev, torch.cuda.current_stream(dev).cuda_stream)
    ctr = _tn_counters.get(key)
    if ctr is None:
        ctr = _tn_counters[key] = torch.zeros(int(lib().op_gemm_tn_grouped_counter_bytes()), dtype=torch.uint8, device=dev)
    arr = lambda vals: (c_int64 * n)(*vals)
    As, Bs, Cs = [q[0] for q in problems], [q[1] for q in problems], [q[2] for q in problems]
    acc = (ctypes.c_int32 * n)(*[int(bool(q[3])) for q in problems])
    side = [tuple(q[4]) + (None,) * (3 - len(q[4])) if len(q) > 4 and q[4] is not None else (None, None, None) for q in problems]
    Ws, Rs, Ss = [x[0] for x in side], [x[1] for x in side], [x[2] for x in side]
    has_side = any(r is not None for r in Rs)
    for sc, r, a, b in zip(Ss, Rs, As, Bs):
        assert sc is None or (sc.dtype == torch.bfloat16 and sc.is_contiguous() and sc.numel() == a.shape[1])
        assert r is None or (r.dtype == torch.float32 and r.is_contiguous() and r.shape == (b.shape[1] // 128, a.shape[1])), "rowdot: fp32 [N / 128, M]"
    head = (n, _ptr_array(As, n), arr([a.stride(0) for a in As]), _ptr_array(Bs, n), arr([b.stride(0) for b in Bs]),
            _ptr_array(Cs, n), arr([c.stride(0) for c in Cs]), arr([a.shape[1] for a in As]),
            arr([b.shape[1] for b in Bs]), arr([a.shape[0] for a in As]), acc,
            _ptr_array(Ws, n) if has_side else None, arr([w.stride(0) if w is not None else 0 for w in Ws]) if has_side else None,
            _ptr_array(Rs, n) if has_side else None, _ptr_array(Ss, n) if any(x is not None for x in Ss) else None)
    if ktiles is not None and any(k is not None for k in ktiles):
        for k, a in zip(ktiles, As):
            assert k is None or (k[0].dtype == torch.int32 and k[1].dtype == torch.int32 and k[0].numel() >= a.shape[0] // 64)
        rc = lib().op_gemm_tn_grouped_lists(*head, _ptr_array([k[0] if k is not None else None for k in ktiles], n),
                                            _ptr_array([k[1] if k is not None else None for k in ktiles], n), ptr(ctr), int(tune), stream())
    else:
        rc = lib().op_gemm_tn_grouped(*head, ptr(ctr), int(tune), stream())
    if rc == -95:
        return False
    _check(rc, "op_gemm_tn_grouped")
    for a, b, c, ac in [q[:4] for q in problems]:
        K, M = a.shape
        GEMM_ALGO_BYTES[0] += 2 * (K * M + K * b.shape[1] + M * b.shape[1] * (2 if ac else 1))
    GEMM_ALGO_BYTES[1] += 1
    return True


def transpose(x2d, out=None, scale=None):
    rows, cols = x2d.shape
    if out is None:
        out = torch.empty(cols, rows, dtype=x2d.dtype, device=x2d.device)
    assert scale is None or (scale.dtype == torch.bfloat16 and scale.is_contiguous() and scale.numel() == rows)
    _check(lib().op_transpose_scaled(ptr(x2d), ptr(out), rows, cols, x2d.stride(0), out.stride(0), ptr(scale), stream()), "op_transpose")
    return out


def transpose_table(jobs, device):
    import struct
    assert lib().op_transpose_desc_bytes() == 56
    raw, tile0 = b"", 0
    for job in jobs:
        src, dst = job[:2]
        scale = job[2] if len(job) > 2 else None
        rows, cols = src.shape
        tx, ty = (cols + 63) // 64, (rows + 63) // 64
        raw += struct.pack("<QQiiqqiiQ", src.data_ptr(), dst.data_ptr(), rows, cols, src.stride(0), dst.stride(0), tile0, tx,
                           scale.data_ptr() if scale is not None else 0)
        tile0 += tx * ty
    table = torch.frombuffer(bytearray(raw), dtype=torch.uint8).to(device)
    return table, tile0


def transpose_batched(table, n, total_tiles):
    _check(lib().op_transpose_batched(ptr(table), n, total_tiles, stream()), "op_transpose_batched")


def colsum(x, y=None, rowscale=None, rows_per_sample=0, mul=None, out=None, accumulate=False, out_dtype=torch.bfloat16):
    M, N = x.shape
    if out is None:
        out = torch.empty(N, dtype=out_dtype, device=x.device)
        accumulate = False
    ws = workspace(lib().op_colsum_workspace_bytes(N), x.device, "colsum")
    _check(lib().op_colsum(ptr(x), ptr(y), ptr(rowscale), rows_per_sample, ptr(mul), ptr(out), ptr(ws), M, N,
                           int(accumulate), _dt(out), stream()), "op_colsum")
    return out


def colsum_segments(x, seg_cols, outs=None, accumulate=False):
    M, N = x.shape
    n_seg = N // seg_cols
    if outs is None:
        outs = [torch.empty(seg_cols, dtype=x.dtype, device=x.device) for _ in range(n_seg)]
        accumulate = False
    o = list(outs) + [None] * (3 - len(outs))
    ws = workspace(lib().op_colsum_workspace_bytes(N), x.device, "colsum")
    _check(lib().op_colsum_segments(ptr(x), ptr(o[0]), ptr(o[1]), ptr(o[2]), ptr(ws), M, n_seg, seg_cols, int(accumulate),
                                    stream()), "op_colsum_segments")
    return outs


def resid_bwd(dout, y=None, gamma=None, rowscale=None, rows_per_sample=0, dgamma=None, dbias=None, accumulate=False, g0=None,
              dout_rows=None):
    M, N = dout.shape
    if dout_rows is not None:
        assert dout_rows.dtype == torch.int32 and dout_rows.is_contiguous() and dout.is_contiguous()
        M = dout_rows.numel()
    out = torch.empty(M, N, dtype=dout.dtype, device=dout.device)
    if dgamma is True:
        dgamma = torch.empty(N, dtype=dout.dtype, device=dout.device)
    if dbias is True:
        dbias = torch.empty(N, dtype=dout.dtype, device=dout.device)
    ws = None
    if dgamma is not None or dbias is not None or g0 is not None:
        ws = workspace(lib().op_resid_bwd_workspace_bytes(N), dout.device, "resid")
    assert g0 is None or (g0.dtype == torch.float32 and g0.is_contiguous() and g0.numel() == N)
    _check(lib().op_resid_bwd(ptr(dout), ptr(y if dgamma is not None else None), ptr(gamma), ptr(rowscale), rows_per_sample,
                              ptr(out), ptr(dgamma), ptr(dbias), ptr(g0), ptr(ws), M, N, int(accumulate), ptr(dout_rows), stream()),
           "op_resid_bwd")
    return out, dgamma, dbias


def gamma_grad_finish(rowdot, pairs, dgamma, accumulate):
    assert rowdot.dtype == torch.float32 and rowdot.dim() == 2 and rowdot.is_contiguous() and len(pairs) <= 3 and dgamma.dtype == torch.bfloat16
    assert rowdot.shape[1] == dgamma.numel()
    flat = []
    for b, g0 in list(pairs) + [(None, None)] * (3 - len(pairs)):
        flat += [ptr(b), ptr(g0)]
    _check(lib().op_gamma_grad_finish(ptr(rowdot), rowdot.shape[0], *flat, ptr(dgamma), rowdot.shape[1], int(accumulate), stream()),
           "op_gamma_grad_finish")
    return dgamma


def ln_geglu_bwd(dy, h0, h1, w, mean, rstd, dw=None, db=None, accumulate=False, need_wgrad=True, dh0=None, dh1=None):
    rows, cols = h0.shape
    if dh0 is None:
        dh0, dh1 = torch.empty_like(h0), torch.empty_like(h1)
    assert dh0.stride(0) == dh1.stride(0) and dh0.stride(1) == 1 and dh1.stride(1) == 1
    assert h0.stride(0) == h1.stride(0) and h0.stride(1) == 1 and h1.stride(1) == 1
    ws = None
    if need_wgrad:
        if dw is None:
            dw, db, accumulate = torch.empty_like(w), torch.empty_like(w), False
        ws = workspace(lib().op_layernorm_bwd_workspace_bytes(rows, cols), h0.device, "ln")
    else:
        dw = db = None
    _check(lib().op_ln_geglu_bwd(ptr(dy), ptr(h0), ptr(h1), ptr(w), ptr(mean), ptr(rstd), ptr(dh0), ptr(dh1), dh0.stride(0),
                                 h0.stride(0), ptr(dw), ptr(db), ptr(ws), rows, cols, int(accumulate), stream()), "op_ln_geglu_bwd")
    return dh0, dh1, dw, db


def ln_geglu_fwd(h0, h1, w, b, eps=1e-5, want_stats=True, out=None, mean=None, rstd=None, q8=None):
    rows, cols = h0.shape
    assert h0.stride(0) == h1.stride(0) and h0.stride(1) == 1 and h1.stride(1) == 1
    y = out if out is not None else torch.empty(rows, cols, dtype=h0.dtype, device=h0.device)
    if want_stats and mean is None:
        mean = torch.empty(rows, dtype=torch.float32, device=h0.device)
        rstd = torch.empty(rows, dtype=torch.float32, device=h0.device)
    if q8 is not None:
        assert q8[0].is_contiguous() and q8[0].shape == (rows, cols) and y.is_contiguous()
        _check(lib().op_ln_geglu_fwd_q8(ptr(h0), ptr(h1), h0.stride(0), ptr(w), ptr(b), ptr(y), ptr(mean), ptr(rstd), ptr(q8[0]), ptr(q8[1]),
                                        rows, cols, eps, stream()), "op_ln_geglu_fwd_q8")
        return y, mean, rstd
    _check(lib().op_ln_geglu_fwd(ptr(h0), ptr(h1), h0.stride(0), ptr(w), ptr(b), ptr(y), ptr(mean), ptr(rstd), rows, cols, eps, stream()),
           "op_ln_geglu_fwd")
    return y, mean, rstd


def geglu_bwd(dg, h0, h1):
    dh0, dh1 = torch.empty_like(h0), torch.empty_like(h1)
    _check(lib().op_geglu_bwd(ptr(dg), ptr(h0), ptr(h1), ptr(dh0), ptr(dh1), dg.numel(), stream()), "op_geglu_bwd")
    return dh0, dh1


def scale_rows(dout, gamma=None, rowscale=None, rows_per_sample=0):
    M, N = dout.shape
    out = torch.empty_like(dout)
    _check(lib().op_scale_rows(ptr(dout), ptr(gamma), ptr(rowscale), rows_per_sample, ptr(out), M, N, stream()),
           "op_scale_rows")
    return out


def l2norm_fwd(x, out_dtype=torch.bfloat16, eps=1e-12):
    rows, cols = x.shape
    y = torch.empty(rows, cols, dtype=out_dtype, device=x.device)
    inv = torch.empty(rows, dtype=torch.float32, device=x.device)
    _check(lib().op_l2norm_fwd(ptr(x), ptr(y), ptr(inv), rows, cols, eps, _dt(y), stream()), "op_l2norm_fwd")
    return y, inv


def l2norm_bwd(dy, y, inv):
    rows, cols = y.shape
    dx = torch.empty(rows, cols, dtype=torch.bfloat16, device=y.device)
    _check(lib().op_l2norm_bwd(ptr(dy), ptr(y), ptr(inv), ptr(dx), rows, cols, _dt(y), stream()), "op_l2norm_bwd")
    return dx


def infonce_rows(sim, target0, label_smoothing=0.0, gscale=1.0, write_grad=True):
    rows, n = sim.shape
    dev = sim.device
    loss = torch.empty(rows, dtype=torch.float32, device=dev)
    hit = torch.empty(rows, dtype=torch.float32, device=dev)
    dot = torch.empty(rows, dtype=torch.float32, device=dev)
    _check(lib().op_infonce_rows(ptr(sim), rows, n, sim.stride(0), target0, label_smoothing, gscale, ptr(loss), ptr(hit),
                                 ptr(dot), int(write_grad), stream()), "op_infonce_rows")
    return loss, hit, dot


def adamw_step(p, g, m, v, lr, beta1, beta2, eps, weight_decay, step, grad_scale=1.0, grad_sqnorm=None, clip_norm=0.0):
    _check(lib().op_adamw_step(ptr(p), ptr(g), ptr(m), ptr(v), p.numel(), lr, beta1, beta2, eps, weight_decay, step,
                               grad_scale, ptr(grad_sqnorm), clip_norm, stream()), "op_adamw_step")


def adamw_step_groups(p, g, m, v, group_end8, group_lr_scale, group_wd, lr, beta1, beta2, eps, step, grad_scale=1.0,
                      grad_sqnorm=None, clip_norm=0.0):
    _check(lib().op_adamw_step_groups(ptr(p), ptr(g), ptr(m), ptr(v), p.numel(), ptr(group_end8), ptr(group_lr_scale),
                                      ptr(group_wd), group_end8.numel(), lr, beta1, beta2, eps, step, grad_scale, ptr(grad_sqnorm),
                                      clip_norm, stream()), "op_adamw_step_groups")


def sqnorm(x, out=None):
    if out is None:
        out = torch.empty(1, dtype=torch.float32, device=x.device)
    ws = workspace(4096, x.device, "sqnorm")
    _check(lib().op_sqnorm(ptr(x), x.numel(), ptr(ws), ptr(out), stream()), "op_sqnorm")
    return out


def relpos_bias_build(table, bucket_i32, S, Spad, transposed=False):
    heads = table.shape[1]
    out = torch.empty(heads, S, Spad, dtype=torch.bfloat16, device=table.device)
    _check(lib().op_relpos_bias_build(ptr(table), ptr(bucket_i32), bucket_i32.stride(0), ptr(out), heads, S, Spad,
                                      int(transposed), stream()), "op_relpos_bias_build")
    return out


PAIR_SEG = 32


def relpos_pairs(bucket_i32, S, num_rel):
    key = (S, num_rel, bucket_i32._version)
    cached = getattr(bucket_i32, "_op_pairs", None)
    if cached is not None and cached[0] == key:
        return cached[1]
    dev = bucket_i32.device
    vals, order = torch.sort(bucket_i32[:S, :S].reshape(-1).long(), stable=True)
    pair_off = torch.searchsorted(vals, torch.arange(num_rel + 1, device=dev))
    bucket_seg = torch.zeros(num_rel + 1, dtype=torch.int64, device=dev)
    bucket_seg[1:] = ((pair_off[1:] - pair_off[:-1] + PAIR_SEG - 1) // PAIR_SEG).cumsum(0)
    nseg = S * S // PAIR_SEG + num_rel
    t = torch.arange(nseg, device=dev)
    r = torch.searchsorted(bucket_seg[1:], t, right=True)
    rc = r.clamp(max=num_rel - 1)
    seg = torch.full((nseg + 1,), S * S, dtype=torch.int64, device=dev)
    seg[:nseg] = torch.where(r < num_rel, pair_off[rc] + (t - bucket_seg[rc]) * PAIR_SEG, S * S)
    res = (order.to(torch.int32), seg.to(torch.int32), bucket_seg.to(torch.int32), nseg)
    bucket_i32._op_pairs = (key, res)
    return res


def relpos_bias_bwd(dbias_f32, bucket_i32, num_rel, S, Spad):
    heads = dbias_f32.shape[0]
    pos, seg, bucket_seg, nseg = relpos_pairs(bucket_i32, S, num_rel)
    dtable = torch.empty(num_rel, heads, dtype=torch.float32, device=dbias_f32.device)
    partial = torch.empty(nseg, heads, dtype=torch.float32, device=dbias_f32.device)
    _check(lib().op_relpos_bias_bwd(ptr(dbias_f32), S, Spad, ptr(pos), ptr(seg), nseg, ptr(bucket_seg), num_rel, ptr(partial), ptr(dtable),
                                    heads, stream()), "op_relpos_bias_bwd")
    return dtable


def relpos_bias_build_ids(table, bucket_i32, ids_i32, Kpad, transposed=False):
    B, K = ids_i32.shape
    heads = table.shape[1]
    out = torch.empty(B, heads, K, Kpad, dtype=torch.bfloat16, device=table.device)
    _check(lib().op_relpos_bias_build_ids(ptr(table), ptr(bucket_i32), bucket_i32.stride(0), ptr(ids_i32), ptr(out), B, heads, K, Kpad,
                                          int(transposed), stream()), "op_relpos_bias_build_ids")
    return out


def relpos_bias_bwd_ids(dbias_f32, bucket_i32, ids_i32, num_rel):
    B, heads, K, Kpad = dbias_f32.shape
    Sfull = bucket_i32.shape[0]
    dense = torch.zeros(heads, Sfull, Sfull, dtype=torch.float32, device=dbias_f32.device)
    _check(lib().op_relpos_bias_fold_ids(ptr(dbias_f32), ptr(ids_i32), ptr(dense), Sfull, B, heads, K, Kpad, stream()),
           "op_relpos_bias_fold_ids")
    return relpos_bias_bwd(dense, bucket_i32, num_rel, Sfull, Sfull)


def attn_spad(S):
    return ((S + 127) // 128) * 128


def _bias_bstride(bias):
    return bias.stride(0) if bias is not None and bias.dim() == 4 else 0


def attn_bias_pack(image, S):
    n_img = image.numel() // (image.shape[-2] * image.shape[-1])
    out = torch.empty(lib().op_attn_bias_frag_elems(n_img, S), dtype=torch.bfloat16, device=image.device)
    _check(lib().op_attn_bias_pack(ptr(image), ptr(out), n_img, S, image.shape[-1], stream()), "op_attn_bias_pack")
    return out


def attn_fwd(q, k, v, ld, B, S, heads, scale, bias=None, key_pad=None, Spad=0, out=None, want_lse=True, bias_frag=None):
    dev = q.device
    H = heads * 64
    Spad = Spad or attn_spad(S)
    if out is None:
        out = torch.empty(B * S, H, dtype=torch.bfloat16, device=dev)
    lse = torch.empty(B, heads, Spad, dtype=torch.float32, device=dev) if want_lse else None
    _check(lib().op_attn_fwd(ptr(q), ptr(k), ptr(v), ld, ptr(bias), _bias_bstride(bias), ptr(bias_frag), ptr(key_pad), ptr(out), out.stride(0),
                             ptr(lse), Spad, B, S, Spad, heads, 64, scale, TUNE.attn_fwd(), stream()), "op_attn_fwd")
    return out, lse


def attn_bwd(q, k, v, ld, dout, out, lse, B, S, heads, scale, bias=None, biasT=None, key_pad=None, Spad=0, dqkv=None,
             want_dbias=False, bias_frag=None):
    dev = q.device
    H = heads * 64
    Spad = Spad or attn_spad(S)
    delta = torch.empty(B, heads, Spad, dtype=torch.float32, device=dev)
    assert out.stride(0) == dout.stride(0)
    if dqkv is None:
        dqkv = torch.empty(B * S, 3 * H, dtype=torch.bfloat16, device=dev)
    per_sample = bias is not None and bias.dim() == 4
    dbias = attn_dbias_buffer(B, S, heads, Spad, dev, per_sample) if want_dbias else None
    dq, dk, dv = dqkv[:, :H], dqkv[:, H:2 * H], dqkv[:, 2 * H:]
    attn_bwd_launch(q, k, v, ld, dout, bias, biasT, key_pad, lse, delta, dq, dk, dv, dqkv.stride(0), dbias, B, S, Spad, heads, scale,
                    bias_frag, out=out)
    if dbias is None:
        return dqkv, None
    return dqkv, (dbias if per_sample else dbias.sum(0))


def attn_bwd_launch(q, k, v, ld, dout, bias, biasT, key_pad, lse, delta, dq, dk, dv, ldg, dbias, B, S, Spad, heads, scale,
                    bias_frag=None, out=None):
    _check(lib().op_attn_bwd(ptr(q), ptr(k), ptr(v), ld, ptr(dout), ptr(out), dout.stride(0), ptr(bias), ptr(biasT), ptr(bias_frag),
                             _bias_bstride(bias),
                             ptr(key_pad), ptr(lse), ptr(delta), ptr(dq), ptr(dk), ptr(dv), ldg, ptr(dbias), B, S, Spad, heads,
                             64, scale, TUNE.attn_bwd(), stream()), "op_attn_bwd")


def attn_dbias_buffer(B, S, heads, Spad, device, per_sample=False):
    slabs = B if per_sample else lib().op_attn_bwd_dbias_slabs(B, S, heads, TUNE.attn_bwd())
    return torch.zeros(slabs, heads, S, Spad, dtype=torch.float32, device=device)


class profile_kernels:

    def __enter__(self):
        lib().op_prof_enable(1)
        return self

    def __exit__(self, *exc):
        lib().op_prof_enable(0)

    @staticmethod
    def collect(n=4):
        ms = (c_double * n)()
        cnt = (c_int64 * n)()
        work = (c_double * n)()
        lib().op_prof_collect(ms, cnt, work, n)
        return [dict(ms=ms[i], count=cnt[i], work=work[i]) for i in range(n)]


class KeptRows:

    def __init__(self, segs, lists, base, full_rows, scale, pad=256):
        n = len(segs)
        assert 1 <= n <= 4
        self.lists, self.full_rows, self.scale, self.nseg = lists, int(full_rows), float(scale), n
        self.S = [int(s[1]) for s in segs]
        self.n_samples = [int(s[2]) for s in segs]
        self.n_kept = [len(s[3]) for s in segs]
        self.src_row0 = [int(s[0]) for s in segs]
        self.dst_rows = [-(-(k * S) // pad) * pad for k, S in zip(self.n_kept, self.S)]
        self.dst_row0, self.off_kept, self.off_inv = [], [], []
        r, o = 0, int(base)
        for k, ns, dr in zip(self.n_kept, self.n_samples, self.dst_rows):
            self.dst_row0.append(r)
            self.off_kept.append(o)
            self.off_inv.append(o + k)
            r, o = r + dr, o + k + ns
        self.total, self.list_end = r, o
        arr = lambda v: (c_int64 * n)(*v)
        self._c = tuple(arr(v) for v in (self.src_row0, self.dst_row0, self.S, self.n_kept, self.dst_rows, self.n_samples))
        self._c_kept, self._c_inv = arr(self.off_kept), arr(self.off_inv)

    def kept_list(self, i):
        return self.lists[self.off_kept[i]:self.off_kept[i] + self.n_kept[i]]

    def rowmap(self):
        m = getattr(self, "_rowmap", None)
        if m is None:
            m = torch.empty(self.total, dtype=torch.int32, device=self.lists.device)
            c = self._c
            _check(lib().op_rows_map(ptr(m), ptr(self.lists), self.nseg, c[0], c[1], c[2], c[3], c[4], c[5], self._c_kept, self.total,
                                     stream()), "op_rows_map")
            self._rowmap = m
        return m


def pack_kept_lists(plans):
    out, bases = [], []
    for segs in plans:
        bases.append(len(out))
        for _, _, ns, kept in segs:
            inv = [-1] * ns
            for j, smp in enumerate(kept):
                inv[smp] = j
            out.extend(int(v) for v in kept)
            out.extend(inv)
    return torch.tensor(out if out else [0], dtype=torch.int32), bases


def rows_gather(src, kr):
    assert src.dim() == 2 and src.is_contiguous() and src.shape[0] == kr.full_rows and src.dtype == torch.bfloat16
    dst = torch.empty(kr.total, src.shape[1], dtype=src.dtype, device=src.device)
    c = kr._c
    _check(lib().op_rows_gather(ptr(src), ptr(dst), ptr(kr.lists), kr.nseg, c[0], c[1], c[2], c[3], c[4], c[5], kr._c_kept, kr.total,
                                src.shape[1], stream()), "op_rows_gather")
    return dst


def rows_merge(base, upd, kr, out=None):
    assert base.dim() == 2 and base.is_contiguous() and base.shape[0] == kr.full_rows and base.dtype == torch.bfloat16
    if upd is None:
        assert out is not None and out is not base and out.shape == base.shape and out.is_contiguous()
    else:
        assert upd.is_contiguous() and upd.shape[0] == kr.total and upd.dtype == torch.bfloat16 and base.shape[1] == upd.shape[1]
    if out is None:
        out = torch.empty_like(base)
    c = kr._c
    _check(lib().op_rows_merge(ptr(base), ptr(upd), ptr(out), ptr(kr.lists), kr.nseg, c[0], c[1], c[2], c[3], c[4], c[5], kr._c_inv,
                               kr.full_rows, base.shape[1], stream()), "op_rows_merge")
    return out


SIM_TOPK_MAX_K = 64


def sim_topk(q, g, k, splits=None):
    assert q.dtype == torch.bfloat16 and g.dtype == torch.bfloat16 and q.is_cuda and g.is_cuda, "sim_topk takes bf16 CUDA tensors"
    assert q.dim() == 2 and g.dim() == 2 and q.shape[1] == g.shape[1], "sim_topk: q [M, D] and g [N, D]"
    M, D = q.shape
    N = g.shape[0]
    if not 1 <= k <= min(N, SIM_TOPK_MAX_K):
        raise ValueError("sim_topk: need 1 <= k <= min(N, %d), got k = %d, N = %d" % (SIM_TOPK_MAX_K, k, N))

    def operand(x):
        if D % 32 or x.stride(1) != 1 or x.stride(0) % 8 or x.data_ptr() % 16:
            Dp = (D + 31) // 32 * 32
            y = torch.zeros(x.shape[0], Dp, dtype=x.dtype, device=x.device)
            y[:, :D] = x
            return y
        return x

    q, g = operand(q), operand(g)
    vals = torch.empty(M, k, dtype=torch.float32, device=q.device)
    idx = torch.empty(M, k, dtype=torch.int32, device=q.device)
    if M == 0:
        return vals, idx.long()
    s = int(splits or 0)
    ws_bytes = lib().op_sim_topk_workspace_bytes(M, N, k, s)
    ws = torch.empty(ws_bytes, dtype=torch.uint8, device=q.device) if ws_bytes else None
    _check(lib().op_sim_topk(ptr(q), q.stride(0), ptr(g), g.stride(0), M, N, q.shape[1], k, ptr(vals), ptr(idx), ptr(ws), ws_bytes, s,
                             stream()), "op_sim_topk")
    return vals, idx.long()


DT_U8 = 2
_IMAGE_OUT = {torch.bfloat16: DT_BF16, torch.float32: DT_F32, torch.uint8: DT_U8}


def image_resize_normalize(packed, mean=None, std=None, dtype=torch.bfloat16, device=None):
    if dtype not in _IMAGE_OUT:
        raise TypeError("image_resize_normalize: dtype must be bfloat16, float32 or uint8, got %s" % dtype)
    if dtype != torch.uint8 and (mean is None or std is None):
        raise ValueError("image_resize_normalize: mean and std are required for a normalised output")
    dev = torch.device(device) if device is not None else torch.device("cuda", torch.cuda.current_device())
    B, S = len(packed), packed.size
    out = torch.empty((B, S, S, 3) if dtype == torch.uint8 else (B, 3, S, S), dtype=dtype, device=dev)
    if B == 0:
        return out
    with torch.cuda.device(dev):
        buf = packed.host.to(dev, non_blocking=packed.host.is_pinned())
        ws = torch.empty(packed.workspace_bytes, dtype=torch.uint8, device=dev)
        base = buf.data_ptr()
        m = (c_float * 3)(*mean) if mean is not None else None
        sd = (c_float * 3)(*std) if std is not None else None
        _check(lib().op_image_resize_normalize(c_void_p(base), packed.src_bytes, c_void_p(base + packed.desc_off),
                                               packed.desc.ctypes.data_as(c_void_p), B, c_void_p(base + packed.coef_off),
                                               packed.coef_count, S, m, sd, ptr(out), _IMAGE_OUT[dtype], ptr(ws), ws.numel(), stream()),
               "op_image_resize_normalize")
    return out


def audio_normalize_pad(packed, dtype=torch.float32, device=None):
    if dtype not in (torch.bfloat16, torch.float32):
        raise TypeError("audio_normalize_pad: dtype must be bfloat16 or float32, got %s" % dtype)
    dev = torch.device(device) if device is not None else torch.device("cuda", torch.cuda.current_device())
    B, T = len(packed), packed.T
    out = torch.empty((B, T), dtype=dtype, device=dev)
    if B == 0:
        return out
    with torch.cuda.device(dev):
        buf = packed.host.to(dev, non_blocking=packed.host.is_pinned())
        ws = torch.empty(max(packed.workspace_bytes, 16), dtype=torch.uint8, device=dev)
        base = buf.data_ptr()
        _check(lib().op_audio_normalize_pad(c_void_p(base), packed.src_bytes, c_void_p(base + packed.desc_off),
                                            packed.desc.ctypes.data_as(c_void_p), B, packed.max_len, packed.min_len, ptr(out), T,
                                            DT_BF16 if dtype == torch.bfloat16 else DT_F32, ptr(ws), ws.numel(), stream()),
               "op_audio_normalize_pad")
    return out


def audio_resample(packed, device=None):
    dev = torch.device(device) if device is not None else torch.device("cuda", torch.cuda.current_device())
    with torch.cuda.device(dev):
        buf = torch.empty(packed.total_bytes, dtype=torch.uint8, device=dev)
        buf[:packed.host.numel()].copy_(packed.host, non_blocking=packed.host.is_pinned())
        base = buf.data_ptr()
        if packed.norm_desc is None:
            out = torch.zeros((len(packed), packed.rows), dtype=torch.float32, device=dev)
            out_ptr = out.data_ptr()
        else:
            out, out_ptr = buf, base + packed.out_off
        if len(packed.which):
            _check(lib().op_audio_resample(c_void_p(base), packed.src_bytes, c_void_p(base + packed.desc_off),
                                           packed.desc.ctypes.data_as(c_void_p), len(packed.which), c_void_p(base + packed.coef_off),
                                           packed.coef_count, c_void_p(out_ptr), packed.out_bytes, stream()), "op_audio_resample")
    return out


def audio_normalize_pad_device(buf, packed, dtype=torch.float32):
    if dtype not in (torch.bfloat16, torch.float32):
        raise TypeError("audio_normalize_pad_device: dtype must be bfloat16 or float32, got %s" % dtype)
    B, T = len(packed), packed.T
    out = torch.empty((B, T), dtype=dtype, device=buf.device)
    if B == 0:
        return out
    with torch.cuda.device(buf.device):
        ws = torch.empty(max(packed.workspace_bytes, 16), dtype=torch.uint8, device=buf.device)
        base = buf.data_ptr()
        _check(lib().op_audio_normalize_pad(c_void_p(base), packed.total_bytes, c_void_p(base + packed.norm_desc_off),
                                            packed.norm_desc.ctypes.data_as(c_void_p), B, packed.max_len, packed.min_len, ptr(out), T,
                                            DT_BF16 if dtype == torch.bfloat16 else DT_F32, ptr(ws), ws.numel(), stream()),
               "op_audio_normalize_pad")
    return out


def average_precision(scores, targets):
    assert scores.dtype == torch.float32 and targets.dtype == torch.uint8 and scores.is_cuda and targets.is_cuda, \
        "average_precision takes fp32 scores and uint8 targets on a CUDA device"
    assert scores.dim() == 2 and scores.shape == targets.shape, "average_precision: scores and targets [N, C]"
    N, C = scores.shape
    if N < 1 or C < 1:
        raise ValueError("average_precision: need N >= 1 and C >= 1, got [%d, %d]" % (N, C))
    if scores.stride(1) != 1 or scores.stride(0) < C:
        scores = scores.contiguous()
    if targets.stride(1) != 1 or targets.stride(0) < C:
        targets = targets.contiguous()
    with torch.cuda.device(scores.device):
        ap = torch.empty(C, dtype=torch.float64, device=scores.device)
        npos = torch.empty(C, dtype=torch.int32, device=scores.device)
        ws_bytes = lib().op_average_precision_workspace_bytes(N, C)
        ws = torch.empty(ws_bytes, dtype=torch.uint8, device=scores.device)
        _check(lib().op_average_precision(ptr(scores), scores.stride(0), ptr(targets), targets.stride(0), N, C, ptr(ap), ptr(npos),
                                          ptr(ws), ws_bytes, stream()), "op_average_precision")
    return ap, npos


ROW_LOSS_HARD, ROW_LOSS_SOFT, ROW_LOSS_MULTI, ROW_LOSS_HINGE = 0, 1, 2, 3


def row_loss(logits, targets, mode, label_smoothing=0.0, margin=1.0, gscale=1.0, write_grad=True):
    assert logits.is_cuda and logits.dim() == 2 and logits.stride(1) == 1, "row_loss takes CUDA logits [B, C] with unit column stride"
    B, C = logits.shape
    dense = mode in (ROW_LOSS_SOFT, ROW_LOSS_MULTI)
    if dense:
        assert targets.is_cuda and tuple(targets.shape) == (B, C) and targets.stride(1) == 1, "row_loss: targets [B, C], unit column stride"
        tdt, ldt = _dt(targets), targets.stride(0)
    else:
        _req(targets, "targets", torch.int64)
        assert tuple(targets.shape) == (B,), "row_loss: targets [B]"
        tdt, ldt = 0, 0
    dev = logits.device
    loss = torch.empty(B, dtype=torch.float32, device=dev)
    correct = torch.empty(B, dtype=torch.float32, device=dev)
    dlogits = torch.empty(B, C, dtype=torch.float32, device=dev) if write_grad else None
    sums = torch.zeros(2, dtype=torch.float32, device=dev) if B == 0 else torch.empty(2, dtype=torch.float32, device=dev)
    _check(lib().op_row_loss(ptr(logits), _dt(logits), logits.stride(0) if B > 1 else max(C, logits.stride(0)), ptr(targets), tdt,
                             ldt if B > 1 else max(C, ldt), B, C, mode, label_smoothing, margin, gscale, ptr(loss), ptr(correct),
                             ptr(dlogits), ptr(sums), stream()), "op_row_loss")
    return sums, loss, correct, dlogits


def box_loss(logits, targets, gscale=1.0, write_grad=True):
    _req(logits, "logits")
    _req(targets, "targets", torch.float32)
    assert logits.dim() == 2 and logits.shape[1] == 4 and tuple(targets.shape) == tuple(logits.shape), "box_loss: logits, targets [B, 4]"
    B = logits.shape[0]
    out = torch.full((2,), float("nan"), dtype=torch.float32, device=logits.device) if B == 0 else torch.empty(
        2, dtype=torch.float32, device=logits.device)
    dlogits = torch.empty(B, 4, dtype=torch.float32, device=logits.device) if write_grad else None
    _check(lib().op_box_loss(ptr(logits), _dt(logits), ptr(targets), B, gscale, ptr(out), ptr(dlogits), stream()), "op_box_loss")
    return out, dlogits


def mfma_rate_probe(seconds=1.0, waves_per_cu=8, data="normal", device=None):
    device = device or torch.device("cuda", torch.cuda.current_device())
    cus = torch.cuda.get_device_properties(device).multi_processor_count
    wgs = cus * max(1, (int(waves_per_cu) + 3) // 4)
    g = torch.Generator().manual_seed(1)
    img = (torch.randn(8 * 64 * 8, generator=g) * 0.5 if data == "normal" else torch.zeros(8 * 64 * 8)).to(device=device, dtype=torch.bfloat16)
    out = torch.empty(wgs * 256, dtype=torch.float32, device=device)
    clk = torch.zeros(wgs * 2, dtype=torch.int64, device=device)
    iters, ms = 20000, 0.0
    for leg in range(3):
        e0, e1 = torch.cuda.Event(enable_timing=True), torch.cuda.Event(enable_timing=True)
        e0.record(torch.cuda.current_stream(device))
        _check_probe(probe_lib().op_probe_mfma_rate(ptr(img), ptr(out), ptr(clk), wgs, iters, stream()), "op_probe_mfma_rate")
        e1.record(torch.cuda.current_stream(device))
        e1.synchronize()
        ms = e0.elapsed_time(e1)
        if leg == 0:
            iters = max(1, int(iters * seconds * 1e3 / ms))
    c = clk.view(wgs, 2).double().cpu()
    mhz = c[:, 0] / (c[:, 1] * 0.01)
    return {"tflops": wgs * 4 * iters * 64 * 16384.0 / (ms * 1e-3) / 1e12, "ms": ms, "workgroups": wgs,
            "mhz": {"mean": float(mhz.mean()), "min": float(mhz.min()), "max": float(mhz.max())}}
```

one-peace_amd/ops.py:

```python
import math
import os
import weakref

import torch
import torch.nn.functional as F

from . import hip

_wt_cache = {}
_cache_epoch = 0


_refresh_plan = None


def invalidate_weight_cache():
    global _cache_epoch
    _cache_epoch += 1


def refresh_weight_cache():
    global _cache_epoch, _refresh_plan
    _cache_epoch += 1
    if not FP8_FFN and (_fp8_cache or _fp8_derived_cache):
        _fp8_cache.clear()
        _fp8_pairs.clear()
        _fp8_derived_cache.clear()
    for k, (ref, _, qs) in list(_fp8_cache.items()):
        w = ref()
        if w is None:
            del _fp8_cache[k]
            continue
        hip.quant_fp8_rows(w.detach(), out=qs)
        _fp8_cache[k] = (ref, (w._version, w.data_ptr(), _cache_epoch), qs)
    live = [(k, v) for k, v in _wt_cache.items() if all(r() is not None for r in v[0]) and (v[3] is None or v[3]() is not None)]
    if not live:
        return
    sig = tuple((k, tuple(r().data_ptr() for r in v[0]), v[2].data_ptr(), v[3]().data_ptr() if v[3] is not None else 0) for k, v in live)
    if _refresh_plan is None or _refresh_plan[0] != sig:
        jobs = []
        for k, v in live:
            off = 0
            for r in v[0]:
                w = r().detach()
                jobs.append((w, v[2][:, off:off + w.shape[0]], v[3]().detach() if v[3] is not None else None))
                off += w.shape[0]
        table, tiles = hip.transpose_table(jobs, live[0][1][2].device)
        _refresh_plan = (sig, table, len(jobs), tiles)
    hip.transpose_batched(_refresh_plan[1], _refresh_plan[2], _refresh_plan[3])
    torch.autograd.graph.increment_version([v[2] for _, v in live])
    for k, v in live:
        _wt_cache[k] = (v[0], _wt_version(tuple(r() for r in v[0]), v[3]() if v[3] is not None else None), v[2], v[3])
    for k, (_, qs, tref) in list(_fp8_derived_cache.items()):
        t = tref()
        if t is None:
            del _fp8_derived_cache[k]
            continue
        hip.quant_fp8_rows(t, out=qs)
        _fp8_derived_cache[k] = ((_cache_epoch, t._version), qs, tref)


def _wt_version(ws, scale):
    return (tuple(w._version for w in ws), tuple(w.data_ptr() for w in ws), _cache_epoch,
            (scale._version, scale.data_ptr()) if scale is not None else None)


def _transposed(ws, scale=None):
    ws = ws if isinstance(ws, (tuple, list)) else (ws,)
    assert scale is None or len(ws) == 1
    key = tuple(id(w) for w in ws) + ((id(scale),) if scale is not None else ())
    ver = _wt_version(ws, scale)
    hit = _wt_cache.get(key)
    if hit is not None and all(r() is w for r, w in zip(hit[0], ws)) and (scale is None or (hit[3] is not None and hit[3]() is scale)):
        if hit[1] == ver:
            return hit[2]
        out = hit[2]
    else:
        out = None
        if len(_wt_cache) > 4096:
            for k in [k for k, v in _wt_cache.items() if any(r() is None for r in v[0]) or (v[3] is not None and v[3]() is None)]:
                del _wt_cache[k]
    src = ws[0] if len(ws) == 1 else torch.cat([w.detach() for w in ws], dim=0)
    t = hip.transpose(src.detach(), out, scale=scale.detach() if scale is not None else None)
    if out is not None:
        torch.autograd.graph.increment_version(t)
    _wt_cache[key] = (tuple(weakref.ref(w) for w in ws), ver, t, weakref.ref(scale) if scale is not None else None)
    return t


FP8_FFN = False
_fp8_cache = {}


FP8_FFN_DGRAD = os.environ.get("ONEPEACE_FP8_DGRAD", "1") != "0"


def set_fp8_ffn(on, dgrad=None):
    global FP8_FFN, FP8_FFN_DGRAD
    old, FP8_FFN = FP8_FFN, bool(on)
    if dgrad is not None:
        FP8_FFN_DGRAD = bool(dgrad)
    return old


_fp8_derived_cache = {}


def _fp8_derived(t):
    key = (t.data_ptr(), tuple(t.shape))
    ver = (_cache_epoch, t._version)
    hit = _fp8_derived_cache.get(key)
    if hit is not None and hit[2]() is t:
        if hit[0] != ver:
            hip.quant_fp8_rows(t, out=hit[1])
            _fp8_derived_cache[key] = (ver, hit[1], hit[2])
        return hit[1]
    if hit is None and len(_fp8_derived_cache) > 4096:
        for k in [k for k, v in _fp8_derived_cache.items() if v[2]() is None]:
            del _fp8_derived_cache[k]
    qs = hip.quant_fp8_rows(t, out=hit[1] if hit is not None else None)
    _fp8_derived_cache[key] = (ver, qs, weakref.ref(t))
    return qs


RECOMPUTE_CHEAP = os.environ.get("ONEPEACE_RECOMPUTE_CHEAP", "0") == "1"


def set_recompute_cheap(on):
    global RECOMPUTE_CHEAP
    old, RECOMPUTE_CHEAP = RECOMPUTE_CHEAP, bool(on)
    return old


def _fp8_weight(w):
    key = id(w)
    ver = (w._version, w.data_ptr(), _cache_epoch)
    hit = _fp8_cache.get(key)
    if hit is not None and hit[0]() is w:
        if hit[1] != ver:
            hip.quant_fp8_rows(w.detach(), out=hit[2])
            _fp8_cache[key] = (hit[0], ver, hit[2])
        return hit[2]
    if len(_fp8_cache) > 4096:
        for k in [k for k, v in _fp8_cache.items() if v[0]() is None]:
            del _fp8_cache[k]
    qs = hip.quant_fp8_rows(w.detach())
    _fp8_cache[key] = (weakref.ref(w), ver, qs)
    return qs


_fp8_pairs = {}


def _fp8_weight_pair(w0, w1):
    key = (id(w0), id(w1))
    hit = _fp8_pairs.get(key)
    if hit is None or hit[0]() is not w0 or hit[1]() is not w1:
        F0, K = w0.shape
        q = torch.empty(F0 + w1.shape[0], K, dtype=torch.uint8, device=w0.device)
        sc = torch.empty(F0 + w1.shape[0], dtype=torch.float32, device=w0.device)
        for w, lo, hi in ((w0, 0, F0), (w1, F0, q.shape[0])):
            view = (q[lo:hi], sc[lo:hi])
            hip.quant_fp8_rows(w.detach(), out=view)
            _fp8_cache[id(w)] = (weakref.ref(w), (w._version, w.data_ptr(), _cache_epoch), view)
        if len(_fp8_pairs) > 1024:
            for k in [k for k, v in _fp8_pairs.items() if v[0]() is None or v[1]() is None]:
                del _fp8_pairs[k]
        hit = _fp8_pairs[key] = (weakref.ref(w0), weakref.ref(w1), (q, sc))
    else:
        _fp8_weight(w0)
        _fp8_weight(w1)
    return hit[2]


def _round_up(n, m):
    return ((n + m - 1) // m) * m


def _t_pad(x2d):
    M, C = x2d.shape
    Mp = _round_up(M, 64)
    out = torch.empty(C, Mp, dtype=x2d.dtype, device=x2d.device)
    if Mp != M:
        out[:, M:].zero_()
    hip.transpose(x2d, out)
    return out


_tail_pads = {}


def _tail_pad(t, rows0, operand):
    r, cols = t.shape[0] - rows0, t.shape[1]
    key = (t.device, torch.cuda.current_stream(t.device).cuda_stream, operand, r, cols)
    buf = _tail_pads.get(key)
    if buf is None:
        if len(_tail_pads) > 64:
            _tail_pads.clear()
        buf = _tail_pads[key] = torch.zeros(64, cols, dtype=t.dtype, device=t.device)
    buf[:r].copy_(t[rows0:])
    return buf


def wgrad_tn_rows(K):
    return K - K % 64


def wgrad(dy, x, out=None, accumulate=False):
    K, M = dy.shape
    N = x.shape[1]
    K0 = wgrad_tn_rows(K)
    if K0 >= 64 and hip.gemm_tn_supported(K0, M, N, dy.stride(0), x.stride(0), out.stride(0) if out is not None else 0):
        out = hip.gemm_tn(dy[:K0], x[:K0], out, accumulate)
        if K0 != K:
            hip.gemm_tn(_tail_pad(dy, K0, 0), _tail_pad(x, K0, 1), out, True)
        return out
    if out is not None and accumulate:
        return out.add_(hip.gemm_nt(_t_pad(dy), [_t_pad(x)]))
    return hip.gemm_nt(_t_pad(dy), [_t_pad(x)], out=out)


GROUPED_WGRAD = os.environ.get("ONEPEACE_GROUPED_WGRAD", "1") != "0"
SKIP_ZERO_BACKWARD = os.environ.get("ONEPEACE_SKIP_ZERO_BACKWARD", "1") != "0"


def _live_ktiles(segs, probs, device):
    if not (SKIP_ZERO_BACKWARD and GROUPED_WGRAD) or all(q[0] is None for q in segs):
        return [None] * len(probs)
    if any(rows % 64 != 0 or rows < 64 for _, rows in probs) or len(segs) > 4 or len(probs) > 8:
        return [None] * len(probs)
    if any(ps is not None and (ps.dtype != torch.float32 or not ps.is_contiguous() or ps.numel() < B) for ps, _, _, B in segs):
        return [None] * len(probs)
    return hip.live_ktiles(segs, probs, device)


class _WgradQueue:

    def __init__(self):
        self.items, self.done, self.after, self.armed, self.epoch = [], [], [], False, 0
        self.lists = []

    def reset(self):
        self.items, self.done, self.after, self.armed = [], [], [], False
        self.lists = []
        self.epoch += 1

    @staticmethod
    def _span(out):
        lo = out.data_ptr()
        return lo, lo + ((out.shape[0] - 1) * out.stride(0) + out.shape[1]) * out.element_size()

    def add(self, dy, x, out, params, side=None, after=None, ktiles=None):
        lo, hi = self._span(out)
        for it in self.items:
            l2, h2 = self._span(it[2])
            if lo < h2 and l2 < hi:
                self.flush()
                break
        self.items.append((dy, x, out, True, side))
        self.lists.append(ktiles)
        self.done.extend(params)
        if after is not None:
            self.after.append(after)
        if not self.armed:
            self.armed = True
            epoch = self.epoch
            torch.autograd.Variable._execution_engine.queue_callback(lambda: self._end_of_backward(epoch))
        if len(self.items) >= hip.TN_GROUP_MAX:
            self.flush()

    def _end_of_backward(self, epoch):
        if epoch != self.epoch:
            return
        self.armed = False
        self.flush()

    def flush(self):
        items, done, after, lists = self.items, self.done, self.after, self.lists
        self.items, self.done, self.after, self.lists = [], [], [], []
        if items:
            kw = {"ktiles": lists} if any(k is not None for k in lists) else {}
            if len(items) == 1 or not hip.gemm_tn_grouped(items, **kw):
                for dy, x, out, _, side in items:
                    if side is None:
                        hip.gemm_tn(dy, x, out, True)
                    else:
                        prod = hip.gemm_tn(dy, x, None, False)
                        W, rowdot, gamma = side
                        out.addcmul_(prod, gamma.detach().unsqueeze(1))
                        rowdot.zero_()
                        for r0 in range(0, prod.shape[0], 256):
                            rowdot[0, r0:r0 + 256] = (W.detach()[r0:r0 + 256].float() * prod[r0:r0 + 256].float()).sum(1)
        for f in after:
            f()
        for q in done:
            _direct_grad_done(q)


_wgrad_queue = _WgradQueue()


def _wgrad_queueable(K, M, N, ldy, ldx, grad_view):
    return (GROUPED_WGRAD and K % 64 == 0 and K >= 64 and grad_view.stride(0) % 8 == 0 and grad_view.stride(1) == 1
            and grad_view.data_ptr() % 16 == 0
            and hip.gemm_tn_supported(K, M, N, ldy, ldx))


def wgrad_into(dy, x, grad_view, params, side=None, after=None, ktiles=None):
    K, M = dy.shape
    if _wgrad_queueable(K, M, x.shape[1], dy.stride(0), x.stride(0), grad_view):
        _wgrad_queue.add(dy, x, grad_view, params, side, after, ktiles)
        return
    assert side is None and after is None, "wgrad_into: a side product was promised for a problem the grouped launch does not take"
    wgrad(dy, x, out=grad_view, accumulate=True)
    for q in params:
        _direct_grad_done(q)


DGAMMA_FROM_WGRAD = os.environ.get("ONEPEACE_DGAMMA_FROM_WGRAD", "1") != "0"


def _rowdot_slots(device, weights):
    n = [w.shape[1] // 128 for w in weights]
    buf = torch.empty(sum(n), weights[0].shape[0], dtype=torch.float32, device=device)
    views, off = [], 0
    for k in n:
        views.append(buf[off:off + k])
        off += k
    return buf, views


def dgamma_from_wgrad_ok(rows, gamma, weights, biases, needs_g, needs_w):
    if not (DGAMMA_FROM_WGRAD and needs_g and all(needs_w) and gamma is not None and _direct_grad(gamma) and gamma.dtype == torch.bfloat16):
        return False
    for k, w in zip(rows, weights):
        if not (_direct_grad(w) and w.is_contiguous() and w.shape[0] % 256 == 0 and w.shape[1] % 256 == 0 and w.data_ptr() % 16 == 0
                and _wgrad_queueable(k, w.shape[0], w.shape[1], w.shape[0], w.shape[1], w.grad)):
            return False
    return all(b is None or _direct_grad(b) for b in biases)


def flush_wgrads():
    _wgrad_queue.flush()


def reset_wgrads():
    _wgrad_queue.reset()


def _direct_grad(param):
    return getattr(param, "_op_flat", False) and param.grad is not None


def _direct_grad_done(param):
    left = getattr(param, "_op_pending", 1) - 1
    param._op_pending = left
    if left <= 0:
        cb = getattr(param, "_op_on_final", None)
        if cb is not None:
            cb(param)


def gemm_any(A, W, bias=None, out_f32=False, alpha=None):
    M, K = A.shape
    N = W.shape[0]
    Kp, Np = _round_up(K, 64), _round_up(N, 8)
    if Kp != K:
        A = torch.nn.functional.pad(A, (0, Kp - K))
        W = torch.nn.functional.pad(W, (0, Kp - K))
    if Np != N:
        W = torch.nn.functional.pad(W, (0, 0, 0, Np - N))
        if bias is not None:
            bias = torch.nn.functional.pad(bias, (0, Np - N))
    A = A.contiguous()
    W = W.contiguous()
    if out_f32:
        out = hip.gemm_nt(A, [W], [bias] if bias is not None else None, epilogue=hip.EPI_F32, alpha=alpha)
    else:
        out = hip.gemm_nt(A, [W], [bias] if bias is not None else None)
    return out if Np == N else out[:, :N].contiguous()


def hip_eligible(x):
    return x.is_cuda and x.dtype == torch.bfloat16


def similarity_topk(query, gallery, k, splits=None):
    if hip_eligible(query) and hip_eligible(gallery):
        return hip.sim_topk(query, gallery, k, splits=splits)
    if not 1 <= k <= gallery.shape[0]:
        raise ValueError("similarity_topk: need 1 <= k <= N, got k = %d, N = %d" % (k, gallery.shape[0]))
    scores = query.float() @ gallery.float().t()
    scores = torch.where(scores == 0, torch.zeros_like(scores), scores)
    vals, idx = torch.sort(scores, dim=1, descending=True, stable=True)
    return vals[:, :k].contiguous(), idx[:, :k].contiguous()


def _average_precision_torch(scores, positive):
    N, C = scores.shape
    v, order = torch.sort(scores, dim=0, descending=True, stable=True)
    y = positive.gather(0, order).long()
    tp_upto = torch.cumsum(y, dim=0)
    pos = torch.arange(1, N + 1, device=scores.device).unsqueeze(1).expand(N, C)
    last = torch.ones(N, C, dtype=torch.bool, device=scores.device)
    last[:-1] = v[:-1] != v[1:]
    ends = torch.where(last, pos, torch.full_like(pos, N))
    cnt = torch.flip(torch.cummin(torch.flip(ends, (0,)), dim=0)[0], (0,))
    tp = tp_upto.gather(0, cnt - 1)
    terms = torch.where(y.bool(), tp.double() / cnt.double(), torch.zeros((), dtype=torch.float64, device=scores.device))
    npos = y.sum(0)
    ap = torch.where(npos > 0, terms.sum(0) / npos.clamp(min=1).double(), torch.zeros((), dtype=torch.float64, device=scores.device))
    return ap, npos


def average_precision(scores, targets):
    if scores.dim() != 2 or tuple(scores.shape) != tuple(targets.shape):
        raise ValueError("average_precision: scores and targets must be [N, C] of one shape, got %s and %s" % (
            tuple(scores.shape), tuple(targets.shape)))
    if scores.shape[0] < 1 or scores.shape[1] < 1:
        raise ValueError("average_precision: need N >= 1 and C >= 1, got %s" % (tuple(scores.shape),))
    if not scores.is_floating_point():
        raise ValueError("average_precision: scores must be floating point, got %s" % scores.dtype)
    targets = targets.to(scores.device)
    scores = scores.float()
    bad_target = ((targets != 0) & (targets != 1)).any() if targets.is_floating_point() else torch.zeros((), dtype=torch.bool, device=scores.device)
    has_nan, bad_target = torch.stack([torch.isnan(scores).any(), bad_target]).tolist()
    if has_nan:
        raise ValueError("average_precision: scores contain NaN")
    if bad_target:
        raise ValueError("average_precision: float targets must be 0 or 1")
    positive = targets != 0
    if scores.is_cuda:
        ap, npos = hip.average_precision(scores, positive.to(torch.uint8))
        return ap, npos.long()
    return _average_precision_torch(scores, positive)


def _is_pil(im):
    return type(im).__module__.startswith("PIL.") and hasattr(im, "convert")


def preprocess_images(images, size, mean=None, std=None, dtype=torch.float32, device="cpu"):
    import numpy as np

    from . import imageprep
    mean = imageprep.CLIP_MEAN if mean is None else tuple(mean)
    std = imageprep.CLIP_STD if std is None else tuple(std)
    imageprep.check_size(size)
    dev = torch.device(device)
    if dev.type == "cuda":
        arrs = [np.asarray(im.convert("RGB")) if _is_pil(im) else im for im in images]
        packed = imageprep.pack_images(arrs, size)
        kdt = dtype if dtype in (torch.bfloat16, torch.float32) else torch.float32
        return hip.image_resize_normalize(packed, mean, std, kdt, dev).to(dtype)
    from PIL import Image
    out = []
    for im in images:
        im = im.convert("RGB") if _is_pil(im) else Image.fromarray(imageprep.as_rgb_array(im))
        u8 = torch.from_numpy(np.array(im.resize((size, size), Image.BICUBIC), dtype=np.uint8))
        out.append(imageprep.to_tensor_normalize(u8, mean, std))
    return torch.stack(out).to(device=dev, dtype=dtype) if out else torch.empty(0, 3, size, size, dtype=dtype, device=dev)


def _audio_item(item, sample_rate, resample):
    import os

    import numpy as np

    from . import audioprep
    rate = sample_rate
    if isinstance(item, tuple) and len(item) == 2 and (torch.is_tensor(item[0]) or isinstance(item[0], (np.ndarray, list, str, bytes, os.PathLike))):
        item, rate = item
        audioprep._check_rates(rate, sample_rate)
    if isinstance(item, (str, bytes, os.PathLike)):
        item, rate = audioprep.read_wav(item)
    if not resample:
        audioprep.check_rate(rate, sample_rate)
    return audioprep.as_clip(item), int(rate)


def resample_audio(clips, rates, sample_rate=16000, device="cpu"):
    import numpy as np

    from . import audioprep
    if len(rates) != len(clips):
        raise ValueError("resample_audio: %d clips and %d rates" % (len(clips), len(rates)))
    arrs = [audioprep.as_clip(c) for c in clips]
    for r in rates:
        audioprep._check_rates(r, sample_rate)
    dev = torch.device(device)
    same = [int(r) == int(sample_rate) for r in rates]
    if dev.type == "cuda":
        packed = audioprep.pack_resample(arrs, rates, sample_rate)
        lengths = packed.lengths
        wavs = hip.audio_resample(packed, dev)
        for i, a in enumerate(arrs):
            if same[i]:
                wavs[i, : lengths[i]] = torch.from_numpy(audioprep.mono64(a).astype(np.float32)).to(dev)
        wavs = wavs[:, : max(lengths, default=0)]
    else:
        feats = [audioprep.mono64(a).astype(np.float32) if same[i] else audioprep.resample(a, int(rates[i]), int(sample_rate))
                 for i, a in enumerate(arrs)]
        lengths = [w.shape[0] for w in feats]
        wavs = torch.zeros(len(feats), max(lengths, default=0))
        for i, w in enumerate(feats):
            wavs[i, : lengths[i]] = torch.from_numpy(w)
        wavs = wavs.to(dev)
    return wavs, torch.tensor(lengths, dtype=torch.int64)


def preprocess_audio(clips, sample_rate=16000, max_seconds=15, min_seconds=1, dtype=torch.float32, device="cpu", resample=False):
    from . import audioprep
    items = [_audio_item(c, sample_rate, resample) for c in clips]
    arrs, rates = [a for a, _ in items], [r for _, r in items]
    max_len, min_len = int(sample_rate * max_seconds), int(sample_rate * min_seconds)
    dev = torch.device(device)
    other = any(r != int(sample_rate) for r in rates)
    if dev.type == "cuda":
        kdt = dtype if dtype in (torch.bfloat16, torch.float32) else torch.float32
        if other:
            packed = audioprep.pack_resample(arrs, rates, sample_rate, norm=(max_len, min_len))
            wavs = hip.audio_normalize_pad_device(hip.audio_resample(packed, dev), packed, kdt)
            return wavs.to(dtype), torch.tensor(packed.out_lengths, dtype=torch.int64)
        packed = audioprep.pack_clips(arrs, max_len, min_len)
        return hip.audio_normalize_pad(packed, kdt, dev).to(dtype), torch.tensor(packed.lengths, dtype=torch.int64)
    if other:
        arrs = [a if r == int(sample_rate) else audioprep.resample(a, r, int(sample_rate)) for a, r in items]
    feats = [audioprep.postprocess(a, sample_rate, max_seconds, min_seconds) for a in arrs]
    wavs = torch.zeros(len(feats), max([w.numel() for w in feats], default=0))
    for i, w in enumerate(feats):
        wavs[i, : w.numel()] = w
    return wavs.to(device=dev, dtype=dtype), torch.tensor([w.numel() for w in feats], dtype=torch.int64)


class LayerNormFn(torch.autograd.Function):
    @staticmethod
    def forward(ctx, x, w, b, eps, gelu):
        shape = x.shape
        x2 = x.reshape(-1, shape[-1])
        if not x2.is_contiguous():
            x2 = x2.contiguous()
        need = any(ctx.needs_input_grad[:3])
        y, mean, rstd = hip.layernorm_fwd(x2, w, b, eps, gelu=gelu, want_stats=need)
        if need:
            ctx.save_for_backward(x2, w, b, mean, rstd)
            ctx.gelu = gelu
        return y.view(shape)

    @staticmethod
    def backward(ctx, dy):
        x2, w, b, mean, rstd = ctx.saved_tensors
        dy2 = dy.reshape(x2.shape)
        if not dy2.is_contiguous():
            dy2 = dy2.contiguous()
        dx, dw, db = hip.layernorm_bwd(dy2, x2, w, b, mean, rstd, gelu=ctx.gelu,
                                       need_wgrad=w is not None and (ctx.needs_input_grad[1] or ctx.needs_input_grad[2]))
        return dx.view(dy.shape), dw, db, None, None


def layer_norm(x, w, b, eps=1e-5, gelu=False):
    return LayerNormFn.apply(x, w, b, eps, gelu)


class LinearFn(torch.autograd.Function):
    @staticmethod
    def forward(ctx, x, w, b):
        shape = x.shape
        x2 = x.reshape(-1, shape[-1])
        if not x2.is_contiguous():
            x2 = x2.contiguous()
        y = gemm_any(x2, w, b)
        ctx.save_for_backward(x2, w)
        ctx.has_bias = b is not None
        return y.view(*shape[:-1], w.shape[0])

    @staticmethod
    def backward(ctx, dy):
        x2, w = ctx.saved_tensors
        dy2 = dy.reshape(-1, w.shape[0])
        if not dy2.is_contiguous():
            dy2 = dy2.contiguous()
        dx = dw = db = None
        if ctx.needs_input_grad[0]:
            dx = gemm_any(dy2, _transposed(w)).view(*dy.shape[:-1], w.shape[1])
        if ctx.needs_input_grad[1]:
            if dy2.shape[1] % 8 == 0 and x2.shape[1] % 8 == 0:
                dw = wgrad(dy2, x2)
            else:
                dw = gemm_any(_t_pad(dy2), _t_pad(x2))
        if ctx.has_bias and ctx.needs_input_grad[2]:
            dy8 = dy2 if dy2.shape[1] % 8 == 0 else torch.nn.functional.pad(dy2, (0, 8 - dy2.shape[1] % 8))
            db = hip.colsum(dy8.contiguous())[: w.shape[0]]
        return dx, dw, db


def linear(x, w, b=None):
    return LinearFn.apply(x, w, b)


class RelPosBias:

    def __init__(self, table, bucket_i32, S, ids=None):
        self.ids = ids
        self.S, self.Spad = S, hip.attn_spad(S)
        self.num_rel, self.heads = table.shape
        self.bucket = bucket_i32
        self.table = table
        self.acc = None
        self._imageT = None
        self._frag = None
        self.image = _RelPosImageFn.apply(table, self)

    @property
    def frag(self):
        if self._frag is None:
            self._frag = hip.attn_bias_pack(self.image.detach(), self.S)
        return self._frag

    @property
    def imageT(self):
        if self._imageT is None:
            if self.ids is not None:
                self._imageT = hip.relpos_bias_build_ids(self.table.detach(), self.bucket, self.ids, self.Spad, transposed=True)
            else:
                self._imageT = hip.relpos_bias_build(self.table.detach(), self.bucket, self.S, self.Spad, transposed=True)
        return self._imageT

    def grad_accumulator(self, B):
        if self.acc is None:
            self.acc = hip.attn_dbias_buffer(B, self.S, self.heads, self.Spad, self.image.device, per_sample=self.ids is not None)
        elif self.ids is None:
            need = hip.lib().op_attn_bwd_dbias_slabs(B, self.S, self.heads, hip.TUNE.attn_bwd())
            if need > self.acc.shape[0]:
                grown = torch.zeros(need, *self.acc.shape[1:], dtype=self.acc.dtype, device=self.acc.device)
                grown[:self.acc.shape[0]] = self.acc
                self.acc = grown
        return self.acc


class DenseBias:

    def __init__(self, dense):
        B, self.heads, self.S, _ = dense.shape
        self.B, self.Spad = B, hip.attn_spad(self.S)
        self.acc = None
        self._imageT = None
        self._frag = None
        self.image = _DenseBiasFn.apply(dense, self)

    @property
    def frag(self):
        if self._frag is None:
            self._frag = hip.attn_bias_pack(self.image.detach(), self.S)
        return self._frag

    @property
    def imageT(self):
        if self._imageT is None:
            img = self.image.detach()
            t = torch.zeros_like(img)
            t[..., : self.S] = img[..., : self.S].transpose(2, 3)
            self._imageT = t
        return self._imageT

    def grad_accumulator(self, B):
        if self.acc is None:
            self.acc = hip.attn_dbias_buffer(B, self.S, self.heads, self.Spad, self.image.device, per_sample=True)
        return self.acc


class _DenseBiasFn(torch.autograd.Function):
    @staticmethod
    def forward(ctx, dense, handle):
        ctx.handle_ref = weakref.ref(handle)
        ctx.S = dense.shape[-1]
        B, heads, S, _ = dense.shape
        img = torch.zeros(B, heads, S, hip.attn_spad(S), dtype=dense.dtype, device=dense.device)
        img[..., :S] = dense
        return img

    @staticmethod
    def backward(ctx, _unused):
        h = ctx.handle_ref()
        if h is None or h.acc is None:
            return torch.zeros(_unused.shape[:-1] + (ctx.S,), dtype=_unused.dtype, device=_unused.device), None
        g = h.acc[..., : ctx.S].to(_unused.dtype)
        h.acc = None
        return g, None


class _RelPosImageFn(torch.autograd.Function):
    @staticmethod
    def forward(ctx, table, handle):
        ctx.handle_ref = weakref.ref(handle)
        ctx.shape = tuple(table.shape)
        if handle.ids is not None:
            return hip.relpos_bias_build_ids(table, handle.bucket, handle.ids, handle.Spad)
        return hip.relpos_bias_build(table, handle.bucket, handle.S, handle.Spad)

    @staticmethod
    def backward(ctx, _unused):
        h = ctx.handle_ref()
        if h is None or h.acc is None:
            return torch.zeros(ctx.shape, dtype=torch.bfloat16, device=_unused.device), None
        if h.ids is not None:
            dtable = hip.relpos_bias_bwd_ids(h.acc, h.bucket, h.ids, h.num_rel)
        else:
            dtable = hip.relpos_bias_bwd(h.acc.sum(0), h.bucket, h.num_rel, h.S, h.Spad)
        h.acc = None
        return dtable.to(torch.bfloat16), None


_DIRECT_WEIGHTS = ("wq", "wk", "wv", "wo", "w0", "w1", "w2")
ATTN_PARAMS = ("ln1_w", "ln1_b", "wq", "bq", "wk", "wv", "bv", "aln_w", "aln_b", "wo", "bo", "g1")
FFN_PARAMS = ("ln2_w", "ln2_b", "w0", "w1", "fln_w", "fln_b", "w2", "b2", "g2")
LAYER_PARAMS = ATTN_PARAMS + FFN_PARAMS


class StreamSeg:
    __slots__ = ("name", "B", "S", "row0", "bias", "key_pad", "pad")

    def __init__(self, name, B, S, row0, bias=None, key_pad=None, pad=0):
        self.name, self.B, self.S, self.row0, self.bias, self.key_pad, self.pad = name, B, S, row0, bias, key_pad, pad

    @property
    def tokens(self):
        return self.B * self.S

    @property
    def rows(self):
        return self.B * self.S + self.pad

    @property
    def end(self):
        return self.row0 + self.B * self.S + self.pad

    def frag(self, limit):
        return self.bias.frag if self.bias is not None and self.S <= limit else None


def _attn_forward(x2, P, segs, heads, scale, rowscale, rps, keep, want_y=True, xmap=None, out=None):
    H = x2.shape[1]
    xln1, mean1, rstd1 = hip.layernorm_fwd(x2, P["ln1_w"], P["ln1_b"], want_stats=keep, x_rows=xmap)
    if H % 128 == 0:
        Nr = xln1.shape[0]
        full = _qkv_rows_that_fill_whole_rounds(Nr, 3 * H) if QKV_ROUND_SPLIT else Nr
        if full < Nr:
            qkv = torch.empty(Nr, 3 * H, dtype=x2.dtype, device=x2.device)
            for lo, hi in ((0, full), (full, Nr)):
                hip.gemm_nt(xln1[lo:hi], [P["wq"], P["wk"], P["wv"]], [P["bq"], None, P["bv"]], n_seg=H, N=3 * H, out=qkv[lo:hi])
        else:
            qkv = hip.gemm_nt(xln1, [P["wq"], P["wk"], P["wv"]], [P["bq"], None, P["bv"]], n_seg=H, N=3 * H)
    else:
        qkv = torch.empty(xln1.shape[0], 3 * H, dtype=x2.dtype, device=x2.device)
        for i, (w, b) in enumerate(((P["wq"], P["bq"]), (P["wk"], None), (P["wv"], P["bv"]))):
            hip.gemm_nt(xln1, [w], [b] if b is not None else None, out=qkv[:, i * H:(i + 1) * H], ldc=3 * H)
    attn = torch.empty_like(xln1)
    lses = []
    for sg in segs:
        r = slice(sg.row0, sg.end)
        _, lse = hip.attn_fwd(qkv[r, :H], qkv[r, H:2 * H], qkv[r, 2 * H:], 3 * H, sg.B, sg.S, heads, scale,
                              sg.bias.image.detach() if sg.bias is not None else None, sg.key_pad, hip.attn_spad(sg.S), out=attn[r],
                              want_lse=keep, bias_frag=sg.frag(hip.ATTN_RESIDENT_MAX_S))
        lses.append(lse)
        if sg.pad:
            attn[sg.end - sg.pad:sg.end].zero_()
    if P["aln_w"] is not None:
        aln, mean_a, rstd_a = hip.layernorm_fwd(attn, P["aln_w"], P["aln_b"], want_stats=keep)
    else:
        aln, mean_a, rstd_a = attn, None, None
    y1 = torch.empty_like(xln1) if keep and want_y else None
    x_mid = hip.gemm_nt(aln, [P["wo"]], [P["bo"]], epilogue=hip.EPI_RESID, resid=x2, gamma=P["g1"], rowscale=rowscale,
                        rows_per_sample=rps, h0=y1, out=out, resid_rows=xmap)
    if not keep:
        return x_mid, None
    acts = dict(xln1=xln1, mean1=mean1, rstd1=rstd1, qkv=qkv, attn=attn, aln=aln, mean_a=mean_a, rstd_a=rstd_a, y1=y1)
    for i, lse in enumerate(lses):
        acts["lse%d" % i] = lse
    return x_mid, acts


QKV_ROUND_SPLIT = os.environ.get("ONEPEACE_QKV_ROUND_SPLIT", "1") != "0"
SKIP_ROW_TABLES = os.environ.get("ONEPEACE_SKIP_ROW_TABLES", "1") != "0"


def _row_tables(kept):
    return kept is not None and SKIP_ROW_TABLES and not FP8_FFN


def _qkv_rows_that_fill_whole_rounds(rows, n_out, cus=256, max_tail=512):
    tn, tm = (n_out + 255) // 256, (rows + 255) // 256
    rounds = -(-tm * tn // cus)
    tm_main = (rounds - 1) * cus // tn
    full = tm_main * 256
    return full if 0 < rows - full <= max_tail and tm_main > 0 else rows


GEGLU_SPLIT = os.environ.get("ONEPEACE_GEGLU_SPLIT", "1") != "0"
SEPARATE_DELTA = os.environ.get("ONEPEACE_SEPARATE_DELTA", "0") == "1"


def _geglu_split(Fd, fln_w):
    return GEGLU_SPLIT and fln_w is not None and Fd % 256 == 0


def _register_direct(ctx, names, params, needs):
    ctx.direct = tuple((n, q) for n, q, ng in zip(names, params, needs) if ng and q is not None and _direct_grad(q))
    for _, q in ctx.direct:
        q._op_pending = getattr(q, "_op_pending", 0) + 1


def _targets(direct, *names):
    if all(n in direct for n in names):
        return [direct[n].grad for n in names], True
    return [None] * len(names), False


def _finish(direct, G, names, values, accumulated):
    for n, v in zip(names, values):
        if accumulated:
            _direct_grad_done(direct[n])
        else:
            G[n] = v


def _return_grads(names, params, G, direct):
    out = []
    for n, q in zip(names, params):
        g = G.get(n) if q is not None else None
        if g is not None and n in direct:
            direct[n].grad.add_(g.view_as(direct[n].grad))
            _direct_grad_done(direct[n])
            g = None
        out.append(g)
    return out


def _resid_backward(dout, y, gamma, ps, S, gname, bname, direct, G, needs, g0=None, rows=None, fold=None):
    names = tuple(n for n, present in ((gname, gamma is not None and g0 is None), (bname, True)) if present and needs.get(n))
    tgt, acc = _targets(direct, *names) if names else ([], False)
    t = dict(zip(names, tgt))
    dgamma = (t[gname] if acc else True) if gname in t else None
    dbias = (t[bname] if acc else True) if bname in t else None
    dy, dg, db = hip.resid_bwd(dout, y if dgamma is not None else None, gamma, ps, S, dgamma=dgamma, dbias=dbias, accumulate=acc, g0=g0,
                               dout_rows=rows)
    if fold is not None and gname in t:
        if not acc:
            fold[gname] = fold[gname] + dg.float() if gname in fold else dg.float()
        names = tuple(n for n in names if n != gname)
    _finish(direct, G, names, tuple({gname: dg, bname: db}[n] for n in names), acc)
    return dy


def _adjacent_grads(direct, names):
    if not all(n in direct for n in names):
        return None
    order = sorted(names, key=lambda n: direct[n].grad.data_ptr())
    for a, b in zip(order, order[1:]):
        ga, gb = direct[a].grad, direct[b].grad
        if not ga.is_contiguous() or ga.data_ptr() + ga.numel() * ga.element_size() != gb.data_ptr() or ga.shape[1:] != gb.shape[1:]:
            return None
    return order


def _span(direct, order):
    g0 = direct[order[0]].grad
    return torch.as_strided(g0, (sum(direct[n].grad.shape[0] for n in order), g0.shape[1]), (g0.shape[1], 1))


def _weight_grad_fn(ctx, G):
    direct = dict(ctx.direct)

    def weight_grad(name, dyv, xv, side=None, after=None, ktiles=None):
        target = direct.get(name)
        if target is not None:
            wgrad_into(dyv, xv, target.grad, (target,), side, after, ktiles)
        else:
            assert side is None and after is None
            G[name] = wgrad(dyv, xv)
    return weight_grad, direct


def _gamma_finish_hook(rowdot, gamma_param, pairs, done):
    def run():
        hip.gamma_grad_finish(rowdot, pairs, gamma_param.grad, True)
        if done:
            _direct_grad_done(gamma_param)
    return run


def _save(ctx, keep, acts, *tensors):
    if keep:
        ctx.act_names = [k for k, v in acts.items() if v is not None]
        ctx.save_for_backward(*tensors, *[acts[k] for k in ctx.act_names])
    else:
        ctx.act_names = None
        ctx.save_for_backward(*tensors)


def _restore(ctx, saved_acts, optional):
    A = dict(zip(ctx.act_names, saved_acts))
    for k in optional:
        A.setdefault(k, None)
    return A


class AttnBranchFn(torch.autograd.Function):

    @staticmethod
    def forward(ctx, x2, segs, rowscale, rps, heads, save_acts, kept, *rest):
        nseg = len(segs)
        params = rest[nseg:]
        P = dict(zip(ATTN_PARAMS, params))
        need_grad = any(ctx.needs_input_grad) and bool(int(save_acts) & 2)
        keep = bool(int(save_acts) & 1) and need_grad
        first_param = 7 + nseg
        needs = dict(zip(ATTN_PARAMS, ctx.needs_input_grad[first_param:]))
        x_full = x2
        mapped = _row_tables(kept)
        if kept is not None and not mapped:
            x2 = hip.rows_gather(x_full, kept)
        H = x2.shape[1]
        N = kept.total if mapped else x2.shape[0]
        scale = (H // heads) ** -0.5
        ctx.dg_fused = need_grad and dgamma_from_wgrad_ok([N], P["g1"], [P["wo"]], [P["bo"]], needs["g1"], [needs["wo"]])
        if mapped:
            x_mid = torch.empty_like(x_full)
            _, acts = _attn_forward(x_full, P, segs, heads, scale, rowscale, rps, keep, want_y=needs["g1"] and not ctx.dg_fused,
                                    xmap=kept.rowmap(), out=x_mid)
            hip.rows_merge(x_full, None, kept, out=x_mid)
        else:
            x_mid, acts = _attn_forward(x2, P, segs, heads, scale, rowscale, rps, keep, want_y=needs["g1"] and not ctx.dg_fused)
            if kept is not None:
                x_mid = hip.rows_merge(x_full, x_mid, kept)
        ctx.kept, ctx.mapped = kept, mapped
        ctx.segs, ctx.dims, ctx.n_params, ctx.first_param = segs, (N, H, heads, scale, rps), len(params), first_param
        ctx.direct = ()
        if need_grad:
            _register_direct(ctx, ATTN_PARAMS, params, ctx.needs_input_grad[first_param:])
        if keep:
            if not needs["wo"]:
                acts["aln"] = None if P["aln_w"] is not None else acts["aln"]
            if not (needs["wq"] or needs["wk"] or needs["wv"]):
                acts["xln1"] = None
        ctx.cheap = keep and bool(int(save_acts) & 4)
        if ctx.cheap:
            acts["xln1"] = None
            if P["aln_w"] is not None:
                acts["aln"] = None
        _save(ctx, keep, acts, x2, rowscale, *params)
        return x_mid

    @staticmethod
    def backward(ctx, dx_mid):
        x2, rowscale, *rest = ctx.saved_tensors
        params, saved_acts = rest[:ctx.n_params], rest[ctx.n_params:]
        N, H, heads, scale, rps = ctx.dims
        segs = ctx.segs
        nseg = len(segs)
        P = dict(zip(ATTN_PARAMS, params))
        needs = {n: bool(ng) and q is not None for n, q, ng in zip(ATTN_PARAMS, params, ctx.needs_input_grad[ctx.first_param:])}
        need_x = bool(ctx.needs_input_grad[0])
        want_dbias = [sg.bias is not None and sg.bias.image.requires_grad for sg in segs]
        kept, mapped = ctx.kept, ctx.mapped
        xmap = kept.rowmap() if mapped else None
        if ctx.act_names is not None:
            A = _restore(ctx, saved_acts, ("mean_a", "rstd_a", "y1", "xln1", "aln"))
            if ctx.cheap:
                if needs["wq"] or needs["wk"] or needs["wv"]:
                    A["xln1"] = hip.layernorm_fwd(x2, P["ln1_w"], P["ln1_b"], x_rows=xmap)[0]
                if needs["wo"] and P["aln_w"] is not None:
                    A["aln"] = hip.layernorm_fwd(A["attn"], P["aln_w"], P["aln_b"])[0]
        else:
            _, A = _attn_forward(x2, P, segs, heads, scale, rowscale, rps, True, want_y=not ctx.dg_fused, xmap=xmap,
                                 out=torch.empty_like(x2) if mapped else None)
        if not dx_mid.is_contiguous():
            dx_mid = dx_mid.contiguous()
        dx_full = dx_mid
        if kept is not None and not mapped:
            dx_mid = hip.rows_gather(dx_full, kept)
        G = {}
        weight_grad, direct = _weight_grad_fn(ctx, G)
        kt1 = None
        if rowscale is not None and kept is None and N % rps == 0 and not any(sg.pad for sg in segs) and sum(sg.rows for sg in segs) == N:
            kt1 = _live_ktiles([(rowscale, 0, rps, N // rps)], [(0, N)], dx_mid.device)[0]
        if ctx.dg_fused:
            g0 = torch.empty(H, dtype=torch.float32, device=dx_mid.device)
            dy1 = _resid_backward(dx_mid, None, P["g1"], rowscale, rps, "g1", "bo", direct, G, needs, g0=g0, rows=xmap)
            rowdot, (rd_wo,) = _rowdot_slots(dx_mid.device, [P["wo"]])
            weight_grad("wo", dy1, A["aln"], side=(P["wo"], rd_wo, P["g1"]),
                        after=_gamma_finish_hook(rowdot, direct["g1"], [(P["bo"], g0)] if P["bo"] is not None else [], True), ktiles=kt1)
            wo_t = _transposed(P["wo"], scale=P["g1"])
        else:
            dy1 = _resid_backward(dx_mid, A["y1"], P["g1"], rowscale, rps, "g1", "bo", direct, G, needs, rows=xmap)
            if needs["wo"]:
                weight_grad("wo", dy1, A["aln"], ktiles=kt1)
            wo_t = None
        upstream = ("ln1_w", "ln1_b", "wq", "bq", "wk", "wv", "bv", "aln_w", "aln_b")
        dx = None
        if need_x or any(want_dbias) or any(needs[n] for n in upstream):
            daln = hip.gemm_nt(dy1, [wo_t if wo_t is not None else _transposed(P["wo"])])
            if P["aln_w"] is not None:
                want = needs["aln_w"] or needs["aln_b"]
                (tw, tb), acc = _targets(direct, "aln_w", "aln_b") if want else ((None, None), False)
                dattn, dw_, db_ = hip.layernorm_bwd(daln, A["attn"], P["aln_w"], P["aln_b"], A["mean_a"], A["rstd_a"], dw=tw, db=tb,
                                                    accumulate=acc, need_wgrad=want)
                if want:
                    _finish(direct, G, ("aln_w", "aln_b"), (dw_, db_), acc)
            else:
                dattn = daln
            qkv_names = ("wq", "wk", "wv")
            order = _adjacent_grads(direct, qkv_names) if all(needs[n] for n in qkv_names) and H % 8 == 0 else None
            cols = tuple(order) if order else qkv_names
            slot = {n: i for i, n in enumerate(cols)}
            qkv = A["qkv"]
            dqkv = torch.empty_like(qkv)
            for i, sg in enumerate(segs):
                r = slice(sg.row0, sg.end)
                if sg.pad:
                    dqkv[sg.end - sg.pad:sg.end].zero_()
                dparts = {n: dqkv[r, slot[n] * H:(slot[n] + 1) * H] for n in qkv_names}
                _attn_backward(qkv[r], dattn[r], A["attn"][r], A["lse%d" % i], sg.B, sg.S, heads, scale,
                               sg.bias.image.detach() if sg.bias is not None else None, sg.bias.imageT if sg.bias is not None else None,
                               sg.key_pad, sg.bias.grad_accumulator(sg.B) if want_dbias[i] else None, sg.frag(384),
                               dparts["wq"], dparts["wk"], dparts["wv"])
            bias_of = {"wq": "bq", "wv": "bv"}
            bnames = tuple(bias_of[n] for n in cols if n in bias_of and needs[bias_of[n]])
            if bnames:
                tgt, acc = _targets(direct, *bnames)
                if H % 8 == 0:
                    outs = [None, None, None]
                    for n, t_ in zip(bnames, tgt):
                        outs[slot["wq" if n == "bq" else "wv"]] = t_ if acc else torch.empty(H, dtype=dqkv.dtype, device=dqkv.device)
                    hip.colsum_segments(dqkv, H, outs, accumulate=acc)
                    _finish(direct, G, bnames, tuple(outs[slot["wq" if n == "bq" else "wv"]] for n in bnames), acc)
                else:
                    sums = hip.colsum(dqkv)
                    for n in bnames:
                        i = slot["wq" if n == "bq" else "wv"]
                        G[n] = sums[i * H:(i + 1) * H]
            if order:
                wgrad_into(dqkv, A["xln1"], _span(direct, order), [direct[n] for n in order], ktiles=kt1)
            elif any(n in direct for n in qkv_names) or not all(needs[n] for n in qkv_names):
                for n in qkv_names:
                    if needs[n]:
                        weight_grad(n, dqkv[:, slot[n] * H:(slot[n] + 1) * H], A["xln1"], ktiles=kt1)
            else:
                dW = wgrad(dqkv, A["xln1"])
                G["wq"], G["wk"], G["wv"] = dW[:H], dW[H:2 * H], dW[2 * H:]
            if need_x or needs["ln1_w"] or needs["ln1_b"]:
                dxln1 = hip.gemm_nt(dqkv, [_transposed(tuple(P[n] for n in cols))])
                want = needs["ln1_w"] or needs["ln1_b"]
                (tw, tb), acc = _targets(direct, "ln1_w", "ln1_b") if want else ((None, None), False)
                dx, dw_, db_ = hip.layernorm_bwd(dxln1, x2, P["ln1_w"], P["ln1_b"], A["mean1"], A["rstd1"], add=dx_mid, dw=tw, db=tb,
                                                 accumulate=acc, need_wgrad=want, dx=torch.empty_like(dx_full) if mapped else None,
                                                 x_rows=xmap)
                if want:
                    _finish(direct, G, ("ln1_w", "ln1_b"), (dw_, db_), acc)
        if dx is None and need_x:
            dx = dx_full
        elif dx is not None and mapped:
            hip.rows_merge(dx_full, None, kept, out=dx)
        elif dx is not None and kept is not None:
            dx = hip.rows_merge(dx_full, dx, kept)
        flush_wgrads()
        grads = _return_grads(ATTN_PARAMS, params, G, direct)
        dimgs = []
        for sg, w in zip(segs, want_dbias):
            if w and not getattr(sg.bias, "_grad_routed", False):
                sg.bias._grad_routed = True
                img = sg.bias.image
                dimgs.append(torch.zeros((), dtype=img.dtype, device=img.device).expand(img.shape))
            else:
                dimgs.append(None)
        return (dx, None, None, None, None, None, None, *dimgs, *grads)


FFN_SHARED = ("ln2_w", "ln2_b", "g2")
FFN_OWN = ("w0", "w1", "fln_w", "fln_b", "w2", "b2")


class FfnBranchMultiFn(torch.autograd.Function):

    @staticmethod
    def _compute(x2, segs, pss, params, keep, want_y, grad=None, xmap=None):
        nseg = len(segs)
        shared = dict(zip(FFN_SHARED, params[:3]))
        own = [dict(zip(FFN_OWN, params[3 + 6 * i:9 + 6 * i])) for i in range(nseg)]
        H = x2.shape[1]
        N = xmap.numel() if xmap is not None else x2.shape[0]
        Fd = own[0]["w0"].shape[0]
        dev, dt = x2.device, x2.dtype
        has_fln = own[0]["fln_w"] is not None
        split = (keep if grad is None else grad) and _geglu_split(Fd, own[0]["fln_w"])
        fp8 = FP8_FFN and H % 128 == 0 and Fd % 128 == 0
        gq = None
        if fp8 and split:
            xln2, mean2, rstd2, (xq, xs) = hip.layernorm_fwd(x2, shared["ln2_w"], shared["ln2_b"], want_stats=keep, q8=True)
            gq, gs = torch.empty(N, Fd, dtype=torch.uint8, device=dev), torch.empty(N, dtype=torch.float32, device=dev)
        else:
            xln2, mean2, rstd2 = hip.layernorm_fwd(x2, shared["ln2_w"], shared["ln2_b"], want_stats=keep, x_rows=xmap)
            if fp8:
                xq, xs = hip.quant_fp8_rows(xln2)
        if split:
            hh = torch.empty(N, 2 * Fd, dtype=dt, device=dev)
            g, h0, h1 = None, hh[:, :Fd], hh[:, Fd:]
        else:
            g = torch.empty(N, Fd, dtype=dt, device=dev)
            h0 = torch.empty(N, Fd, dtype=dt, device=dev) if keep else None
            h1 = torch.empty(N, Fd, dtype=dt, device=dev) if keep else None
        gln = torch.empty(N, Fd, dtype=dt, device=dev) if has_fln else g
        mean_f = torch.empty(N, dtype=torch.float32, device=dev) if (keep or split) and has_fln else None
        rstd_f = torch.empty(N, dtype=torch.float32, device=dev) if (keep or split) and has_fln else None
        L = hip.lib()
        for sg, P in zip(segs, own):
            r = slice(sg.row0, sg.end)
            if split:
                if fp8:
                    w01q, w01s = _fp8_weight_pair(P["w0"], P["w1"])
                    hip.gemm_nt_fp8(xq[r], xs[r], [w01q], [w01s], out=hh[r])
                else:
                    hip.gemm_nt(xln2[r], [P["w0"], P["w1"]], n_seg=Fd, N=2 * Fd, out=hh[r])
                hip.ln_geglu_fwd(h0[r], h1[r], P["fln_w"], P["fln_b"], out=gln[r], mean=mean_f[r], rstd=rstd_f[r],
                                 q8=(gq[r], gs[r]) if fp8 else None)
                continue
            if fp8:
                (w0q, w0s), (w1q, w1s) = _fp8_weight(P["w0"]), _fp8_weight(P["w1"])
                hip.gemm_nt_fp8(xq[r], xs[r], [w0q, w1q], [w0s, w1s], epilogue=hip.EPI_GEGLU, h0=h0[r] if keep else None,
                                h1=h1[r] if keep else None, out=g[r])
            else:
                hip.gemm_nt(xln2[r], [P["w0"], P["w1"]], epilogue=hip.EPI_GEGLU, h0=h0[r] if keep else None, h1=h1[r] if keep else None,
                            out=g[r])
            if has_fln:
                hip._check(L.op_layernorm_fwd(hip.ptr(g[r]), hip.ptr(P["fln_w"]), hip.ptr(P["fln_b"]), hip.ptr(gln[r]),
                                              hip.ptr(mean_f[r]) if keep else None, hip.ptr(rstd_f[r]) if keep else None, sg.rows, Fd, 1e-5, 0,
                                              hip.DT_BF16, None, hip.stream()), "op_layernorm_fwd")
        y2 = torch.empty(N, H, dtype=dt, device=dev) if keep and want_y else None
        out = torch.empty_like(x2)
        rs = [slice(sg.row0, sg.end) for sg in segs]
        if fp8:
            if gq is None:
                gq, gs = hip.quant_fp8_rows(gln)
            for sg, P, r, ps in zip(segs, own, rs, pss):
                w2q, w2s = _fp8_weight(P["w2"])
                hip.gemm_nt_fp8(gq[r], gs[r], [w2q], [w2s], bias=P["b2"], epilogue=hip.EPI_RESID, resid=x2[r], gamma=shared["g2"], rowscale=ps,
                                rows_per_sample=sg.S, h0=y2[r] if y2 is not None else None, out=out[r])
            acts = dict(xln2=xln2, mean2=mean2, rstd2=rstd2, h0=h0, h1=h1, gln=gln, mean_f=mean_f, rstd_f=rstd_f, y2=y2) if keep else None
            return out, acts
        tabs = [xmap[r] for r in rs] if xmap is not None else None
        grouped = nseg > 1 and hip.gemm_nt_grouped(
            [gln[r] for r in rs], [P["w2"] for P in own], biases=[P["b2"] for P in own],
            outs=[out[r] for r in rs] if tabs is None else [out] * nseg, epilogue=hip.EPI_RESID,
            h0s=[y2[r] for r in rs] if y2 is not None else None, resids=[x2[r] for r in rs] if tabs is None else [x2] * nseg,
            gammas=[shared["g2"]] * nseg, rowscales=list(pss), rows_per_sample=[sg.S for sg in segs], resid_rows=tabs) is not None
        if not grouped:
            for i, (sg, P, r, ps) in enumerate(zip(segs, own, rs, pss)):
                hip.gemm_nt(gln[r], [P["w2"]], [P["b2"]], epilogue=hip.EPI_RESID, resid=x2[r] if tabs is None else x2, gamma=shared["g2"],
                            rowscale=ps, rows_per_sample=sg.S, h0=y2[r] if y2 is not None else None, out=out[r] if tabs is None else out,
                            resid_rows=tabs[i] if tabs is not None else None)
        acts = dict(xln2=xln2, mean2=mean2, rstd2=rstd2, h0=h0, h1=h1, gln=gln, mean_f=mean_f, rstd_f=rstd_f, y2=y2) if keep else None
        return out, acts

    @staticmethod
    def forward(ctx, x2, segs, pss, save_acts, kept, *params):
        nseg = len(segs)
        Fd = params[3].shape[0]
        need_grad = any(ctx.needs_input_grad) and bool(int(save_acts) & 2)
        keep = bool(int(save_acts) & 1) and need_grad
        needs = ctx.needs_input_grad[5:]
        has_fln = params[5] is not None
        x_full = x2
        mapped = _row_tables(kept)
        if kept is not None and not mapped:
            x2 = hip.rows_gather(x_full, kept)
        H = x2.shape[1]
        N = kept.total if mapped else x2.shape[0]
        w2s, b2s = [params[3 + 6 * i + 4] for i in range(nseg)], [params[3 + 6 * i + 5] for i in range(nseg)]
        ctx.dg_fused = need_grad and dgamma_from_wgrad_ok([sg.rows for sg in segs], params[2], w2s, b2s, bool(needs[2]),
                                                           [bool(needs[3 + 6 * i + 4]) for i in range(nseg)])
        out, acts = FfnBranchMultiFn._compute(x2, segs, pss, params, keep, bool(needs[2]) and not ctx.dg_fused, grad=bool(int(save_acts) & 2),
                                              xmap=kept.rowmap() if mapped else None)
        if mapped:
            hip.rows_merge(x_full, None, kept, out=out)
        elif kept is not None:
            out = hip.rows_merge(x_full, out, kept)
        ctx.kept, ctx.mapped = kept, mapped
        ctx.segs, ctx.n_params, ctx.dims = segs, len(params), (N, H, Fd)
        ctx.direct = ()
        names = list(FFN_SHARED) + ["%s@%d" % (n, i) for i in range(nseg) for n in FFN_OWN]
        ctx.names = names
        if need_grad:
            _register_direct(ctx, names, params, needs)
        if keep:
            nd = dict(zip(names, needs))
            if not any(nd["w0@%d" % i] or nd["w1@%d" % i] for i in range(nseg)):
                acts["xln2"] = None
            if has_fln and not any(nd["w2@%d" % i] for i in range(nseg)):
                acts["gln"] = None
        ctx.cheap = keep and bool(int(save_acts) & 4)
        if ctx.cheap:
            acts["xln2"] = None
            if _geglu_split(Fd, params[5]):
                acts["gln"] = None
        _save(ctx, keep, acts or {}, x2, *[ps for ps in pss], *params)
        ctx.n_ps = len(pss)
        return out

    @staticmethod
    def backward(ctx, dout):
        x2, *rest = ctx.saved_tensors
        pss, rest = rest[:ctx.n_ps], rest[ctx.n_ps:]
        params, saved_acts = rest[:ctx.n_params], rest[ctx.n_params:]
        segs, names = ctx.segs, ctx.names
        nseg = len(segs)
        N, H, Fd = ctx.dims
        P = dict(zip(names, params))
        needs = {n: bool(ng) and q is not None for n, q, ng in zip(names, params, ctx.needs_input_grad[5:])}
        need_x = bool(ctx.needs_input_grad[0])
        kept, mapped = ctx.kept, ctx.mapped
        xmap = kept.rowmap() if mapped else None
        if ctx.act_names is not None:
            A = _restore(ctx, saved_acts, ("mean_f", "rstd_f", "y2", "gln", "xln2"))
            if ctx.cheap:
                if any(needs["%s@%d" % (n, i)] for i in range(nseg) for n in ("w0", "w1")):
                    A["xln2"] = hip.layernorm_fwd(x2, P["ln2_w"], P["ln2_b"], x_rows=xmap)[0]
                if A["gln"] is None and any(needs["w2@%d" % i] for i in range(nseg)):
                    A["gln"] = torch.empty(N, Fd, dtype=x2.dtype, device=x2.device)
                    for i, sg in enumerate(segs):
                        r = slice(sg.row0, sg.end)
                        hip.ln_geglu_fwd(A["h0"][r], A["h1"][r], P["fln_w@%d" % i], P["fln_b@%d" % i], out=A["gln"][r], want_stats=False)
        else:
            _, A = FfnBranchMultiFn._compute(x2, segs, pss, params, True, not ctx.dg_fused, xmap=xmap)
        if not dout.is_contiguous():
            dout = dout.contiguous()
        dout_full = dout
        if kept is not None and not mapped:
            dout = hip.rows_gather(dout_full, kept)
        G = {}
        weight_grad, direct = _weight_grad_fn(ctx, G)
        has_fln = P["fln_w@0"] is not None
        dev, dt = dout.device, dout.dtype
        upstream = need_x or needs["ln2_w"] or needs["ln2_b"] or any(
            needs["%s@%d" % (n, i)] for i in range(nseg) for n in ("w0", "w1", "fln_w", "fln_b"))
        dh = torch.empty(N, 2 * Fd, dtype=dt, device=dev) if upstream else None
        dgln = torch.empty(N, Fd, dtype=dt, device=dev) if upstream else None
        colsets = []
        fold = {} if nseg > 1 else None
        fused = ctx.dg_fused
        fp8b = FP8_FFN and FP8_FFN_DGRAD and H % 128 == 0 and Fd % 128 == 0
        (rowdot, rd_views), pairs = (_rowdot_slots(dev, [P["w2@%d" % i] for i in range(nseg)]), []) if fused else ((None, None), None)
        kts = [None] * nseg
        if kept is None and not any(sg.pad for sg in segs):
            kts = _live_ktiles([(pss[i], sg.row0, sg.S, sg.B) for i, sg in enumerate(segs)], [(sg.row0, sg.rows) for sg in segs], dev)
        for i, sg in enumerate(segs):
            r = slice(sg.row0, sg.end)
            k = lambda n: "%s@%d" % (n, i)
            g0 = None
            if fused:
                g0 = torch.empty(H, dtype=torch.float32, device=dev)
                if P[k("b2")] is not None:
                    pairs.append((P[k("b2")], g0))
            dy2 = _resid_backward(dout_full if mapped else dout[r], A["y2"][r] if A["y2"] is not None else None, P["g2"], pss[i], sg.S,
                                  "g2", k("b2"), direct, G, needs, g0=g0, rows=xmap[r] if mapped else None, fold=fold)
            if fused:
                weight_grad(k("w2"), dy2, A["gln"][r], side=(P[k("w2")], rd_views[i], P["g2"]),
                            after=_gamma_finish_hook(rowdot, direct["g2"], pairs, True) if i == nseg - 1 else None, ktiles=kts[i])
            elif needs[k("w2")]:
                weight_grad(k("w2"), dy2, A["gln"][r], ktiles=kts[i])
            if not upstream:
                colsets.append(None)
                continue
            w2t = _transposed(P[k("w2")], scale=P["g2"] if fused else None)
            if fp8b:
                hip.gemm_nt_fp8(*hip.quant_fp8_rows(dy2), *[[x] for x in _fp8_derived(w2t)], out=dgln[r])
            else:
                hip.gemm_nt(dy2, [w2t], out=dgln[r])
            pair = (k("w0"), k("w1"))
            order = _adjacent_grads(direct, pair) if needs[pair[0]] and needs[pair[1]] and Fd % 8 == 0 else None
            cols = tuple(order) if order else pair
            colsets.append(cols)
            dpart = {n: dh[r, j * Fd:(j + 1) * Fd] for j, n in enumerate(cols)}
            if has_fln:
                want = needs[k("fln_w")] or needs[k("fln_b")]
                (tw, tb2), acc = _targets(direct, k("fln_w"), k("fln_b")) if want else ((None, None), False)
                _, _, dw_, db2_ = hip.ln_geglu_bwd(dgln[r], A["h0"][r], A["h1"][r], P[k("fln_w")], A["mean_f"][r], A["rstd_f"][r], dw=tw,
                                                   db=tb2, accumulate=acc, need_wgrad=want, dh0=dpart[pair[0]], dh1=dpart[pair[1]])
                if want:
                    _finish(direct, G, (k("fln_w"), k("fln_b")), (dw_, db2_), acc)
            else:
                d0, d1 = hip.geglu_bwd(dgln[r], A["h0"][r], A["h1"][r])
                dpart[pair[0]].copy_(d0)
                dpart[pair[1]].copy_(d1)
            if order:
                wgrad_into(dh[r], A["xln2"][r], _span(direct, order), [direct[n] for n in order], ktiles=kts[i])
            else:
                for n in pair:
                    if needs[n]:
                        weight_grad(n, dpart[n], A["xln2"][r], ktiles=kts[i])
        if fold is not None and needs["g2"] and not fused:
            if "g2" in fold:
                G["g2"] = fold["g2"].to(dt)
            else:
                _direct_grad_done(direct["g2"])
        dx = None
        if upstream and (need_x or needs["ln2_w"] or needs["ln2_b"]):
            dxln2 = torch.empty(N, H, dtype=dt, device=dev)
            rs = [slice(sg.row0, sg.end) for sg in segs]
            wts = [_transposed(tuple(P[n] for n in cols)) for cols in colsets]
            if fp8b:
                for r, wt in zip(rs, wts):
                    hip.gemm_nt_fp8(*hip.quant_fp8_rows(dh[r]), *[[x] for x in _fp8_derived(wt)], out=dxln2[r])
            elif nseg == 1 or hip.gemm_nt_grouped([dh[r] for r in rs], wts, outs=[dxln2[r] for r in rs]) is None:
                for r, wt in zip(rs, wts):
                    hip.gemm_nt(dh[r], [wt], out=dxln2[r])
            want = needs["ln2_w"] or needs["ln2_b"]
            (tw, tb), acc = _targets(direct, "ln2_w", "ln2_b") if want else ((None, None), False)
            dx, dw_, db_ = hip.layernorm_bwd(dxln2, x2, P["ln2_w"], P["ln2_b"], A["mean2"], A["rstd2"], add=dout, dw=tw, db=tb,
                                             accumulate=acc, need_wgrad=want, dx=torch.empty_like(dout_full) if mapped else None, x_rows=xmap)
            if want:
                _finish(direct, G, ("ln2_w", "ln2_b"), (dw_, db_), acc)
        if dx is None and need_x:
            dx = dout_full
        elif dx is not None and mapped:
            hip.rows_merge(dout_full, None, kept, out=dx)
        elif dx is not None and kept is not None:
            dx = hip.rows_merge(dout_full, dx, kept)
        grads = _return_grads(names, params, G, direct)
        return (dx, None, None, None, None, *grads)


def ffn_branch_multi(x2, segs, pss, shared, own, save_acts=True, kept=None):
    flat = list(shared)
    for o in own:
        flat += list(o)
    return FfnBranchMultiFn.apply(x2, segs, tuple(pss), _save_flags(save_acts), kept, *flat)


_SCALE_ROWS = {}


def kept_segments(kept, segs, device):
    out = []
    for i, sg in enumerate(segs):
        key_pad = sg.key_pad.index_select(0, kept.kept_list(i)) if sg.key_pad is not None else None
        out.append(StreamSeg(sg.name, kept.n_kept[i], sg.S, kept.dst_row0[i], sg.bias, key_pad, pad=kept.dst_rows[i] - kept.n_kept[i] * sg.S))
    key = (device, kept.scale)
    vec = _SCALE_ROWS.get(key)
    if vec is None or vec.numel() < kept.total + 8:
        if len(_SCALE_ROWS) > 256:
            _SCALE_ROWS.clear()
        vec = _SCALE_ROWS[key] = torch.full((max(kept.full_rows, kept.total) + 8,), kept.scale, dtype=torch.float32, device=device)
    return out, vec


def _attn_backward(qkv, dattn, attn, lse, B, S, heads, scale, bias_img, biasT, key_pad, dbias_acc, bias_frag, dq, dk, dv):
    H = heads * 64
    dev = qkv.device
    Spad = hip.attn_spad(S)
    delta = torch.empty(B, heads, Spad, dtype=torch.float32, device=dev)
    if attn.stride(0) != dattn.stride(0) or SEPARATE_DELTA:
        hip._check(hip.lib().op_attn_bwd_delta(hip.ptr(dattn), hip.ptr(attn), dattn.stride(0), hip.ptr(delta), B, S, Spad, heads,
                                               hip.stream()), "op_attn_bwd_delta")
        attn = None
    hip.attn_bwd_launch(qkv[:, :H], qkv[:, H:2 * H], qkv[:, 2 * H:], 3 * H, dattn, bias_img, biasT, key_pad, lse, delta, dq, dk,
                        dv, dq.stride(0), dbias_acc, B, S, Spad, heads, scale, bias_frag, out=attn)


def attn_branch(x, bias, key_pad, ps, heads, params, save_acts=False):
    B, S, H = x.shape
    seg = StreamSeg("x", B, S, 0, bias, key_pad)
    out = AttnBranchFn.apply(x.reshape(B * S, H), [seg], ps, S, heads, _save_flags(save_acts), None, bias.image if bias is not None else None, *params)
    return out.view(B, S, H)


def attn_branch_multi(x2, segs, ps_rows, heads, params, save_acts=False, kept=None):
    return AttnBranchFn.apply(x2, segs, ps_rows, 1, heads, _save_flags(save_acts), kept,
                              *[sg.bias.image if sg.bias is not None else None for sg in segs], *params)


def _save_flags(save_acts):
    return int(bool(save_acts)) | (2 if torch.is_grad_enabled() else 0) | (4 if RECOMPUTE_CHEAP and save_acts else 0)


def ffn_branch(x, ps, params, save_acts=False):
    B, S, H = x.shape
    P = dict(zip(FFN_PARAMS, params))
    out = ffn_branch_multi(x.reshape(B * S, H), [StreamSeg("x", B, S, 0)], [ps], [P[n] for n in FFN_SHARED], [[P[n] for n in FFN_OWN]],
                           save_acts)
    return out.view(B, S, H)


class L2NormalizeFn(torch.autograd.Function):

    @staticmethod
    def forward(ctx, x):
        y, inv = hip.l2norm_fwd(x.contiguous())
        ctx.save_for_backward(y, inv)
        return y

    @staticmethod
    def backward(ctx, dy):
        y, inv = ctx.saved_tensors
        return hip.l2norm_bwd(dy.contiguous(), y, inv)


def l2_normalize(x):
    return L2NormalizeFn.apply(x)


class InfoNCEFn(torch.autograd.Function):

    @staticmethod
    def forward(ctx, a_local, b_local, a_all, b_all, scale, rank, label_smoothing):
        b = a_local.shape[0]
        t0 = rank * b
        scale_f = scale.detach().float().reshape(1)
        sims, rows = [], []
        for loc, allv in ((a_local, b_all), (b_local, a_all)):
            sim = gemm_any(loc.detach(), allv.detach(), out_f32=True, alpha=scale_f)
            loss_r, hit_r, dot_r = hip.infonce_rows(sim, t0, label_smoothing, gscale=0.5 / b, write_grad=True)
            sims.append(sim)
            rows.append((loss_r, hit_r, dot_r))
        loss = 0.5 * (rows[0][0].mean() + rows[1][0].mean())
        ctx.save_for_backward(a_local, b_local, a_all, b_all, scale_f, sims[0], sims[1], rows[0][2], rows[1][2])
        ctx.scale_dtype = scale.dtype
        hits_a, hits_b = rows[0][1].sum(), rows[1][1].sum()
        ctx.mark_non_differentiable(hits_a, hits_b)
        return loss, hits_a, hits_b

    @staticmethod
    def backward(ctx, gl, _ga, _gb):
        a_local, b_local, a_all, b_all, scale_f, ds_ab, ds_ba, dot_ab, dot_ba = ctx.saved_tensors
        g = gl.float()
        coef = (g * scale_f).reshape(1)
        da = gemm_any(ds_ab.to(torch.bfloat16), hip.transpose(b_all.contiguous()), out_f32=True, alpha=coef)
        db = gemm_any(ds_ba.to(torch.bfloat16), hip.transpose(a_all.contiguous()), out_f32=True, alpha=coef)
        dscale = (g * (dot_ab.sum() + dot_ba.sum()) / scale_f).reshape(()).to(ctx.scale_dtype)
        return da.to(a_local.dtype), db.to(b_local.dtype), None, None, dscale, None, None


def info_nce(a_local, b_local, a_all, b_all, scale, rank=0, label_smoothing=0.0):
    return InfoNCEFn.apply(a_local, b_local, a_all, b_all, scale, rank, label_smoothing)


class DclFn(torch.autograd.Function):

    @staticmethod
    def forward(ctx, student, teacher, scale, label_smoothing, block):
        m, H = student.shape
        teacher = teacher.detach().contiguous()
        teacher_t = hip.transpose(teacher)
        alpha = torch.full((1,), float(scale), dtype=torch.float32, device=student.device)
        dstudent = torch.empty(m, H, dtype=torch.float32, device=student.device)
        total = torch.zeros((), dtype=torch.float32, device=student.device)
        for r0 in range(0, m, block):
            rows = student[r0:r0 + block].detach().contiguous()
            sim = gemm_any(rows, teacher, out_f32=True, alpha=alpha)
            loss_r, _, _ = hip.infonce_rows(sim, r0, label_smoothing, gscale=1.0 / m, write_grad=True)
            total += loss_r.sum()
            dstudent[r0:r0 + block] = gemm_any(sim.to(torch.bfloat16), teacher_t, out_f32=True, alpha=alpha)
            del sim
        ctx.save_for_backward(dstudent)
        ctx.dtype = student.dtype
        return total / m

    @staticmethod
    def backward(ctx, g):
        (dstudent,) = ctx.saved_tensors
        return (dstudent * g.float()).to(ctx.dtype), None, None, None, None


def dcl_loss(student, teacher, scale, label_smoothing=0.0, block=4096):
    return DclFn.apply(student, teacher, scale, label_smoothing, block)


def loss_hip_eligible(logits):
    return logits.is_cuda and logits.dim() == 2 and logits.dtype in (torch.bfloat16, torch.float32)


class RowLossFn(torch.autograd.Function):

    @staticmethod
    def forward(ctx, logits, targets, mode, label_smoothing, margin):
        x = logits.detach()
        if x.stride(1) != 1:
            x = x.contiguous()
        sums, _, _, dlogits = hip.row_loss(x, targets, mode, label_smoothing, margin, write_grad=ctx.needs_input_grad[0])
        if dlogits is not None:
            ctx.save_for_backward(dlogits)
        ctx.dtype = logits.dtype
        loss, counter = sums[0], sums[1]
        ctx.mark_non_differentiable(counter)
        return loss, counter

    @staticmethod
    def backward(ctx, g, _gc):
        (dlogits,) = ctx.saved_tensors
        return (dlogits * g.float()).to(ctx.dtype), None, None, None, None


def _dense_targets(targets, logits):
    targets = targets.to(logits.device)
    if targets.dtype not in (torch.bfloat16, torch.float32):
        targets = targets.float()
    return targets if targets.stride(1) == 1 else targets.contiguous()


def classify_loss(logits, targets, use_multi_label=False, label_smoothing=0.0):
    if loss_hip_eligible(logits):
        if use_multi_label or targets.dim() == 2:
            if tuple(targets.shape) != tuple(logits.shape):
                raise ValueError("classify_loss: targets %s do not match logits %s" % (tuple(targets.shape), tuple(logits.shape)))
            mode = hip.ROW_LOSS_MULTI if use_multi_label else hip.ROW_LOSS_SOFT
            return RowLossFn.apply(logits, _dense_targets(targets, logits), mode, 0.0, 1.0)
        if tuple(targets.shape) != (logits.shape[0],):
            raise ValueError("classify_loss: targets %s do not match logits %s" % (tuple(targets.shape), tuple(logits.shape)))
        return RowLossFn.apply(logits, targets.to(logits.device, torch.int64).contiguous(), hip.ROW_LOSS_HARD, float(label_smoothing), 1.0)
    if use_multi_label:
        loss = F.binary_cross_entropy_with_logits(logits, targets, reduction="sum")
        with torch.no_grad():
            n_correct = targets.gather(1, logits.argmax(1, keepdim=True)).sum()
    elif targets.dim() == 2:
        log_probs = F.log_softmax(logits, dim=-1, dtype=torch.float32)
        loss = (-targets * log_probs).sum()
        with torch.no_grad():
            n_correct = (log_probs.exp() * targets).sum()
    else:
        loss = F.cross_entropy(logits, targets, label_smoothing=label_smoothing, reduction="sum")
        with torch.no_grad():
            n_correct = logits.argmax(1).eq(targets).sum()
    return loss, n_correct


def hinge_loss(logits, targets, margin=1.0):
    if loss_hip_eligible(logits):
        if tuple(targets.shape) != (logits.shape[0],):
            raise ValueError("hinge_loss: targets %s do not match logits %s" % (tuple(targets.shape), tuple(logits.shape)))
        return RowLossFn.apply(logits, targets.to(logits.device, torch.int64).contiguous(), hip.ROW_LOSS_HINGE, 0.0, float(margin))
    positive_logits = logits.gather(1, targets.unsqueeze(1))
    loss = torch.max(torch.tensor(0.0).to(logits.device), margin + logits - positive_logits).sum()
    n_correct = logits.argmax(1).eq(targets).sum()
    return loss, n_correct


def giou_diagonal(boxes1, boxes2):
    if boxes1.dtype not in (torch.float32, torch.float64):
        boxes1, boxes2 = boxes1.float(), boxes2.float()
    area1 = (boxes1[:, 2] - boxes1[:, 0]) * (boxes1[:, 3] - boxes1[:, 1])
    area2 = (boxes2[:, 2] - boxes2[:, 0]) * (boxes2[:, 3] - boxes2[:, 1])
    wh = (torch.min(boxes1[:, 2:], boxes2[:, 2:]) - torch.max(boxes1[:, :2], boxes2[:, :2])).clamp(min=0)
    inter = wh[:, 0] * wh[:, 1]
    union = area1 + area2 - inter
    iou = inter / union
    whi = (torch.max(boxes1[:, 2:], boxes2[:, 2:]) - torch.min(boxes1[:, :2], boxes2[:, :2])).clamp(min=0)
    areai = whi[:, 0] * whi[:, 1]
    return iou - (areai - union) / areai


def box_loss_torch(logits, targets, nsentences=None):
    output_coords = logits.sigmoid()
    loss = F.l1_loss(output_coords, targets, reduction="sum")
    loss = loss / (logits.shape[0] if nsentences is None else nsentences)
    valid_indices = (output_coords[:, :2] < output_coords[:, 2:]).all(1)
    ious = giou_diagonal(output_coords[valid_indices], targets[valid_indices])
    return loss + (1 - ious).mean()


class BoxLossFn(torch.autograd.Function):
    @staticmethod
    def forward(ctx, logits, targets):
        out, dlogits = hip.box_loss(logits.detach().contiguous(), targets, write_grad=ctx.needs_input_grad[0])
        if dlogits is not None:
            ctx.save_for_backward(dlogits)
        ctx.dtype = logits.dtype
        return out[0]

    @staticmethod
    def backward(ctx, g):
        (dlogits,) = ctx.saved_tensors
        return (dlogits * g.float()).to(ctx.dtype), None


def box_loss(logits, targets):
    if logits.dim() != 2 or logits.shape[1] != 4 or tuple(targets.shape) != tuple(logits.shape):
        raise ValueError("box_loss: logits and targets must be [B, 4], got %s and %s" % (tuple(logits.shape), tuple(targets.shape)))
    if loss_hip_eligible(logits):
        return BoxLossFn.apply(logits, targets.to(logits.device, torch.float32).contiguous())
    return box_loss_torch(logits, targets)
```

Before: 193.5.

## Skip dead-sample rows in layernorm and LN-GeGLU backward kernels

Adds live-row variants of the layernorm backward and LN-GeGLU backward kernels. They take per-sample keep masks (the drop-path rowscale) and skip loading x, dy, h0 and h1 for rows whose sample scale is zero, treating those rows as zero gradients. The attention and FFN branch backward passes route through these variants when live k-tiles are available, which saves memory traffic for dropped samples. In exchange there is a per-row mask lookup and more kernel template instantiations. dx for dead rows comes only from the residual add.

Measured after the change: 192.3. Within noise of the previous version (-0.6%).

```diff
diff --git a/include/onepeace_hip.h b/include/onepeace_hip.h
--- a/include/onepeace_hip.h
+++ b/include/onepeace_hip.h
@@ -55,6 +55,12 @@
                              const int32_t* const* ktiles, const int32_t* const* n_ktiles, void* counters, int64_t tune, void* stream);
 int op_live_ktiles(int64_t nseg, const float* const* ps, const int64_t* row0, const int64_t* S, const int64_t* B, int64_t nprob,
                    const int64_t* prob_row0, const int64_t* prob_rows, int32_t* const* ktiles, int32_t* const* n_ktiles, void* stream);
+int op_layernorm_bwd_live(const void* dy, const void* x, const void* w, const float* mean, const float* rstd, const void* add, void* dx,
+                          void* dw, void* db, void* workspace, int64_t rows, int64_t cols, int accumulate, int64_t nseg,
+                          const float* const* ps, const int64_t* row0, const int64_t* S, const int64_t* B, void* stream);
+int op_ln_geglu_bwd_live(const void* dy, const void* h0, const void* h1, const void* w, const float* mean, const float* rstd,
+                         void* dh0, void* dh1, int64_t ldd, int64_t ldh, void* dw, void* db, void* workspace, int64_t rows,
+                         int64_t cols, int accumulate, const float* ps, int64_t rows_per_sample, void* stream);
 int op_gemm_plan(int64_t M, int64_t N, int64_t K, int epilogue, int has_bias, int64_t workspace_bytes, int64_t tune, int* plan);
 
 int op_quant_fp8_rows(const void* x, int64_t ldx, void* q, int64_t ldq, float* scale, int64_t rows, int64_t cols, void* stream);
diff --git a/one-peace_amd/csrc/layernorm.hip b/one-peace_amd/csrc/layernorm.hip
--- a/one-peace_amd/csrc/layernorm.hip
+++ b/one-peace_amd/csrc/layernorm.hip
@@ -1,4 +1,5 @@
 #include "common.h"
+#include <cstring>
 
 namespace {
 
@@ -53,6 +54,20 @@
 #pragma unroll
   for (int i = 1; i < NW; ++i) t = max(t, __float_as_int(red[i]));
   return __int_as_float(t);
+}
+
+constexpr int LIVE_MAX_SEG = 4;
+struct LiveRows {
+  int nseg;
+  struct { const float* ps; int64_t row0, end; int rps; } seg[LIVE_MAX_SEG];
+};
+__device__ __forceinline__ int row_live(const LiveRows& L, int64_t row) {
+  bool live = true;
+#pragma unroll
+  for (int i = 0; i < LIVE_MAX_SEG; ++i)
+    if (i < L.nseg && L.seg[i].ps != nullptr && row >= L.seg[i].row0 && row < L.seg[i].end)
+      live = L.seg[i].ps[(unsigned)(row - L.seg[i].row0) / (unsigned)L.seg[i].rps] != 0.f;
+  return __builtin_amdgcn_readfirstlane((int)live);
 }
 
 template <typename T, int CH, int NW, bool GELU, bool NT, bool Q8 = false>
@@ -273,13 +288,13 @@
   }
 }
 
-template <typename T, int CH, int NW, bool GELU, bool NT>
+template <typename T, int CH, int NW, bool GELU, bool NT, bool LIVE = false>
 __global__ __launch_bounds__(256) void ln_bwd_kernel(const T* __restrict__ dy, const T* __restrict__ x,
                                                      const T* __restrict__ w, const T* __restrict__ b,
                                                      const float* __restrict__ mean_in,
                                                      const float* __restrict__ rstd_in, const T* __restrict__ add,
                                                      T* __restrict__ dx, float* __restrict__ ws, int64_t rows, int cols,
-                                                     const int* __restrict__ xmap = nullptr) {
+                                                     const int* __restrict__ xmap = nullptr, const LiveRows live = LiveRows{}) {
   extern __shared__ __attribute__((aligned(16))) float smem[];
   float* red = smem;
   constexpr int G = 64 * NW;
@@ -304,30 +319,39 @@
   raw_t curx[CH], curg[CH], nxtx[CH], nxtg[CH], addv[CH];
   int64_t src = row0 < rows ? (xmap ? (int64_t)xmap[row0] : row0) : -1;
   int64_t nsrc = row0 + rstep < rows ? (xmap ? (int64_t)xmap[row0 + rstep] : row0 + rstep) : -1, nnsrc = -1;
+  int lv = 1, nlv = 1, nnlv = 1;
+  if (LIVE) {
+    lv = row0 < rows ? row_live(live, row0) : 0;
+    nlv = row0 + rstep < rows ? row_live(live, row0 + rstep) : 0;
+  }
   if (row0 < rows) {
 #pragma unroll
     for (int i = 0; i < CH; ++i) {
       const int c = (tig + G * i) * 8;
       if (c < cols) {
-        if (src >= 0) curx[i] = ldraw_sel<T, NT>(x + src * (int64_t)cols + c);
+        if (src >= 0 && lv) curx[i] = ldraw_sel<T, NT>(x + src * (int64_t)cols + c);
         else curx[i] = raw_t{};
-        curg[i] = ldraw_sel<T, NT>(dy + row0 * (int64_t)cols + c);
+        if (lv) curg[i] = ldraw_sel<T, NT>(dy + row0 * (int64_t)cols + c);
+        else curg[i] = raw_t{};
       }
     }
   }
   for (int64_t row = row0; row < rows; row += rstep) {
-    const float mean = mean_in[row], rstd = rstd_in[row];
+    float mean = 0.f, rstd = 0.f;
+    if (lv) { mean = mean_in[row]; rstd = rstd_in[row]; }
     const int64_t nrow = row + rstep, nnrow = nrow + rstep;
     if (nnrow < rows) nnsrc = xmap ? (int64_t)xmap[nnrow] : nnrow;
+    if (LIVE && nnrow < rows) nnlv = row_live(live, nnrow);
 #pragma unroll
     for (int i = 0; i < CH; ++i) {
       const int c = (tig + G * i) * 8;
       if (c < cols) {
         if (add && src >= 0) addv[i] = ldraw_sel<T, NT>(add + src * (int64_t)cols + c);
         if (nrow < rows) {
-          if (nsrc >= 0) nxtx[i] = ldraw_sel<T, NT>(x + nsrc * (int64_t)cols + c);
+          if (nsrc >= 0 && nlv) nxtx[i] = ldraw_sel<T, NT>(x + nsrc * (int64_t)cols + c);
           else nxtx[i] = raw_t{};
-          nxtg[i] = ldraw_sel<T, NT>(dy + nrow * (int64_t)cols + c);
+          if (nlv) nxtg[i] = ldraw_sel<T, NT>(dy + nrow * (int64_t)cols + c);
+          else nxtg[i] = raw_t{};
         }
       }
     }
@@ -375,6 +399,8 @@
     for (int i = 0; i < CH; ++i) { curx[i] = nxtx[i]; curg[i] = nxtg[i]; }
     src = nsrc;
     nsrc = nnsrc;
+    lv = nlv;
+    nlv = nnlv;
   }
   if (ws == nullptr) return;
   float* wsb = ws + (int64_t)blockIdx.x * 2 * cols;
@@ -406,13 +432,13 @@
   }
 }
 
-template <int CH, int NW>
+template <int CH, int NW, bool LIVE = false>
 __global__ __launch_bounds__(NW == 1 ? 256 : 64 * NW) void ln_geglu_bwd_kernel(const bf16_t* __restrict__ dy, const bf16_t* __restrict__ h0,
                                                            const bf16_t* __restrict__ h1, const bf16_t* __restrict__ w,
                                                            const float* __restrict__ mean_in,
                                                            const float* __restrict__ rstd_in, bf16_t* __restrict__ dh0,
                                                            bf16_t* __restrict__ dh1, int64_t ldd, int64_t ldh, float* __restrict__ ws,
-                                                           int64_t rows, int cols) {
+                                                           int64_t rows, int cols, const LiveRows live = LiveRows{}) {
   extern __shared__ __attribute__((aligned(16))) float smem[];
   float* red = smem;
   constexpr int G = 64 * NW;
@@ -433,29 +459,44 @@
     if (c < cols && w) wraw[i] = Vec8<bf16_t>::ldraw(w + c);
   }
   bf16x8 r0[CH], r1[CH], rg[CH], n0[CH], n1[CH], ng[CH];
+  int lv = 1, nlv = 1, nnlv = 1;
+  if (LIVE) {
+    lv = row0 < rows ? row_live(live, row0) : 0;
+    nlv = row0 + rstep < rows ? row_live(live, row0 + rstep) : 0;
+  }
+  const bf16x8 zero8 = {(bf16_t)0.f, (bf16_t)0.f, (bf16_t)0.f, (bf16_t)0.f, (bf16_t)0.f, (bf16_t)0.f, (bf16_t)0.f, (bf16_t)0.f};
   if (row0 < rows) {
 #pragma unroll
     for (int i = 0; i < CH; ++i) {
       const int c = (tig + G * i) * 8;
       if (c < cols) {
-        r0[i] = Vec8<bf16_t>::ldraw_nt(h0 + row0 * ldh + c);
-        r1[i] = Vec8<bf16_t>::ldraw_nt(h1 + row0 * ldh + c);
-        rg[i] = Vec8<bf16_t>::ldraw_nt(dy + row0 * (int64_t)cols + c);
+        if (lv) {
+          r0[i] = Vec8<bf16_t>::ldraw_nt(h0 + row0 * ldh + c);
+          r1[i] = Vec8<bf16_t>::ldraw_nt(h1 + row0 * ldh + c);
+          rg[i] = Vec8<bf16_t>::ldraw_nt(dy + row0 * (int64_t)cols + c);
+        } else {
+          r0[i] = r1[i] = rg[i] = zero8;
+        }
       }
     }
   }
   for (int64_t row = row0; row < rows; row += rstep) {
-    const float mean = mean_in[row], rstd = rstd_in[row];
-    const int64_t base = row * (int64_t)cols;
+    float mean = 0.f, rstd = 0.f;
+    if (lv) { mean = mean_in[row]; rstd = rstd_in[row]; }
     const int64_t nrow = row + rstep;
+    if (LIVE && nrow + rstep < rows) nnlv = row_live(live, nrow + rstep);
     if (nrow < rows) {
 #pragma unroll
       for (int i = 0; i < CH; ++i) {
         const int c = (tig + G * i) * 8;
         if (c < cols) {
-          n0[i] = Vec8<bf16_t>::ldraw_nt(h0 + nrow * ldh + c);
-          n1[i] = Vec8<bf16_t>::ldraw_nt(h1 + nrow * ldh + c);
-          ng[i] = Vec8<bf16_t>::ldraw_nt(dy + nrow * (int64_t)cols + c);
+          if (nlv) {
+            n0[i] = Vec8<bf16_t>::ldraw_nt(h0 + nrow * ldh + c);
+            n1[i] = Vec8<bf16_t>::ldraw_nt(h1 + nrow * ldh + c);
+            ng[i] = Vec8<bf16_t>::ldraw_nt(dy + nrow * (int64_t)cols + c);
+          } else {
+            n0[i] = n1[i] = ng[i] = zero8;
+          }
         }
       }
     }
@@ -513,6 +554,8 @@
     }
 #pragma unroll
     for (int i = 0; i < CH; ++i) { r0[i] = n0[i]; r1[i] = n1[i]; rg[i] = ng[i]; }
+    lv = nlv;
+    nlv = nnlv;
   }
   if (ws == nullptr) return;
   float* wsb = ws + (int64_t)blockIdx.x * 2 * cols;
@@ -611,6 +654,52 @@
   return OP_OK;
 }
 
+inline bool live_rows_fill(LiveRows& L, int64_t nseg, const float* const* ps, const int64_t* row0, const int64_t* S, const int64_t* B) {
+  memset(&L, 0, sizeof(L));
+  if (nseg < 1 || nseg > LIVE_MAX_SEG || !ps || !row0 || !S || !B) return false;
+  L.nseg = (int)nseg;
+  for (int i = 0; i < (int)nseg; ++i) {
+    if (row0[i] < 0 || S[i] < 1 || B[i] < 1 || S[i] >= ((int64_t)1 << 31) || S[i] * B[i] >= ((int64_t)1 << 31)) return false;
+    L.seg[i].ps = ps[i]; L.seg[i].row0 = row0[i]; L.seg[i].end = row0[i] + S[i] * B[i]; L.seg[i].rps = (int)S[i];
+  }
+  return true;
+}
+
+int ln_bwd_live_dispatch(const void* dy, const void* x, const void* w, const float* mean, const float* rstd, const void* add, void* dx,
+                         void* dw, void* db, float* ws, int64_t rows, int cols, int accumulate, const LiveRows& L, hipStream_t s) {
+  typedef bf16_t T;
+  const T* DY = (const T*)dy; const T* X = (const T*)x; const T* W = (const T*)w; T* DX = (T*)dx; const T* ADD = (const T*)add;
+  int grid = 0;
+  float* wsk = (dw || db) ? ws : nullptr;
+  const bool nt = (int64_t)rows * cols * (int64_t)sizeof(T) >= ((int64_t)64 << 20);
+#define LN_BL(CH, NW)                                                                                                                 \
+  do {                                                                                                                                \
+    grid = ln_grid(rows, NW, g_ln_blocks_bwd);                                                                                        \
+    size_t sh = (NW == 1) ? (size_t)4 * cols * sizeof(float) : 64;                                                                    \
+    if (nt) hipLaunchKernelGGL((ln_bwd_kernel<T, CH, NW, false, true, true>), dim3(grid), dim3(256), sh, s, DY, X, W, (const T*)nullptr, mean, \
+                       rstd, ADD, DX, wsk, rows, cols, (const int*)nullptr, L);                                                       \
+    else hipLaunchKernelGGL((ln_bwd_kernel<T, CH, NW, false, false, true>), dim3(grid), dim3(256), sh, s, DY, X, W, (const T*)nullptr, mean, \
+                       rstd, ADD, DX, wsk, rows, cols, (const int*)nullptr, L);                                                       \
+  } while (0)
+  if (cols <= 512) LN_BL(1, 1);
+  else if (cols <= 1024) LN_BL(2, 1);
+  else if (cols <= 1536) LN_BL(3, 1);
+  else if (cols <= 2048) LN_BL(4, 1);
+  else if (cols <= 4096) LN_BL(2, 4);
+  else if (cols <= 6144) LN_BL(3, 4);
+  else if (cols <= 8192) LN_BL(4, 4);
+  else { op_set_error("layernorm: cols %d > 8192 unsupported", cols); return OP_ENOTSUP; }
+#undef LN_BL
+  OP_LAUNCH_CHECK();
+  if (wsk) {
+    hipLaunchKernelGGL((partials_reduce3_kernel<T>), dim3(ceil_div(cols, 32), 2), dim3(256), 0, s, ws, ws + cols,
+                       (const float*)nullptr, (const bf16_t*)nullptr, (const bf16_t*)nullptr, (const bf16_t*)nullptr, (T*)dw,
+                       (T*)db, (T*)nullptr, grid, (int64_t)2 * cols, cols, accumulate);
+    OP_LAUNCH_CHECK();
+  }
+  return OP_OK;
+}
+
 }
 
 extern "C" {
@@ -680,6 +769,18 @@
                                                     (int)cols, accumulate, s, x_rows);
   op_set_error("layernorm_bwd: bad dtype %d", dtype);
   return OP_EINVAL;
+}
+
+int op_layernorm_bwd_live(const void* dy, const void* x, const void* w, const float* mean, const float* rstd, const void* add, void* dx,
+                          void* dw, void* db, void* workspace, int64_t rows, int64_t cols, int accumulate, int64_t nseg,
+                          const float* const* ps, const int64_t* row0, const int64_t* S, const int64_t* B, void* stream) {
+  OP_CHECK_ARG(dy && x && dx && mean && rstd, "layernorm_bwd_live: null pointer");
+  OP_CHECK_ARG(rows >= 0 && cols > 0 && cols % 8 == 0, "layernorm_bwd_live: cols=%lld must be a positive multiple of 8", (long long)cols);
+  OP_CHECK_ARG(!(dw || db) || workspace, "layernorm_bwd_live: dw/db requested without workspace");
+  LiveRows L;
+  OP_CHECK_ARG(live_rows_fill(L, nseg, ps, row0, S, B), "layernorm_bwd_live: bad segment table (1 ... %d segments)", LIVE_MAX_SEG);
+  if (rows == 0) return OP_OK;
+  return ln_bwd_live_dispatch(dy, x, w, mean, rstd, add, dx, dw, db, (float*)workspace, rows, (int)cols, accumulate, L, (hipStream_t)stream);
 }
 
 int op_ln_geglu_fwd(const void* h0, const void* h1, int64_t ldh, const void* w, const void* b, void* y, float* mean, float* rstd,
@@ -730,9 +831,9 @@
   return OP_OK;
 }
 
-int op_ln_geglu_bwd(const void* dy, const void* h0, const void* h1, const void* w, const float* mean, const float* rstd,
-                    void* dh0, void* dh1, int64_t ldd, int64_t ldh, void* dw, void* db, void* workspace, int64_t rows, int64_t cols,
-                    int accumulate, void* stream) {
+static int ln_geglu_bwd_impl(const void* dy, const void* h0, const void* h1, const void* w, const float* mean, const float* rstd,
+                             void* dh0, void* dh1, int64_t ldd, int64_t ldh, void* dw, void* db, void* workspace, int64_t rows, int64_t cols,
+                             int accumulate, const LiveRows* L, void* stream) {
   OP_CHECK_ARG(dy && h0 && h1 && dh0 && dh1 && mean && rstd, "ln_geglu_bwd: null pointer");
   if (ldd <= 0) ldd = cols;
   if (ldh <= 0) ldh = cols;
@@ -747,9 +848,12 @@
   do {                                                                                                             \
     grid = ln_grid(rows, NW, OP_LN_GEGLU_BLOCKS_BWD);                                                                     \
     size_t sh = (NW == 1) ? (size_t)4 * cols * sizeof(float) : 64;                                                 \
-    hipLaunchKernelGGL((ln_geglu_bwd_kernel<CH, NW>), dim3(grid), dim3(NW == 1 ? 256 : 64 * NW), sh, s,           \
+    if (L) hipLaunchKernelGGL((ln_geglu_bwd_kernel<CH, NW, true>), dim3(grid), dim3(NW == 1 ? 256 : 64 * NW), sh, s, \
                        (const bf16_t*)dy, (const bf16_t*)h0, (const bf16_t*)h1, (const bf16_t*)w, mean, rstd,      \
-                       (bf16_t*)dh0, (bf16_t*)dh1, ldd, ldh, wsk, rows, (int)cols);                                \
+                       (bf16_t*)dh0, (bf16_t*)dh1, ldd, ldh, wsk, rows, (int)cols, *L);                            \
+    else hipLaunchKernelGGL((ln_geglu_bwd_kernel<CH, NW>), dim3(grid), dim3(NW == 1 ? 256 : 64 * NW), sh, s,       \
+                       (const bf16_t*)dy, (const bf16_t*)h0, (const bf16_t*)h1, (const bf16_t*)w, mean, rstd,      \
+                       (bf16_t*)dh0, (bf16_t*)dh1, ldd, ldh, wsk, rows, (int)cols, LiveRows{});                    \
   } while (0)
   if (cols <= 512) LNG_B(1, 1);
   else if (cols <= 1024) LNG_B(2, 1);
@@ -769,4 +873,22 @@
   return OP_OK;
 }
 
-}
+int op_ln_geglu_bwd(const void* dy, const void* h0, const void* h1, const void* w, const float* mean, const float* rstd,
+                    void* dh0, void* dh1, int64_t ldd, int64_t ldh, void* dw, void* db, void* workspace, int64_t rows, int64_t cols,
+                    int accumulate, void* stream) {
+  return ln_geglu_bwd_impl(dy, h0, h1, w, mean, rstd, dh0, dh1, ldd, ldh, dw, db, workspace, rows, cols, accumulate, nullptr, stream);
+}
+
+int op_ln_geglu_bwd_live(const void* dy, const void* h0, const void* h1, const void* w, const float* mean, const float* rstd,
+                         void* dh0, void* dh1, int64_t ldd, int64_t ldh, void* dw, void* db, void* workspace, int64_t rows, int64_t cols,
+                         int accumulate, const float* ps, int64_t rows_per_sample, void* stream) {
+  OP_CHECK_ARG(ps && rows_per_sample >= 1 && rows % rows_per_sample == 0, "ln_geglu_bwd_live: ps / rows_per_sample=%lld for %lld rows",
+               (long long)rows_per_sample, (long long)rows);
+  if (rows == 0) return OP_OK;
+  LiveRows L;
+  const int64_t zero = 0, nb = rows / rows_per_sample;
+  OP_CHECK_ARG(live_rows_fill(L, 1, &ps, &zero, &rows_per_sample, &nb), "ln_geglu_bwd_live: bad rows");
+  return ln_geglu_bwd_impl(dy, h0, h1, w, mean, rstd, dh0, dh1, ldd, ldh, dw, db, workspace, rows, cols, accumulate, &L, stream);
+}
+
+}
diff --git a/one-peace_amd/hip.py b/one-peace_amd/hip.py
--- a/one-peace_amd/hip.py
+++ b/one-peace_amd/hip.py
@@ -36,6 +36,8 @@
     "op_gemm_tn_grouped": (c_int, [I64, P, P, P, P, P, P, P, P, P, P, P, P, P, P, P, I64, P]),
     "op_gemm_tn_grouped_lists": (c_int, [I64, P, P, P, P, P, P, P, P, P, P, P, P, P, P, P, P, P, I64, P]),
     "op_live_ktiles": (c_int, [I64, P, P, P, P, I64, P, P, P, P, P]),
+    "op_layernorm_bwd_live": (c_int, [P, P, P, P, P, P, P, P, P, P, I64, I64, c_int, I64, P, P, P, P, P]),
+    "op_ln_geglu_bwd_live": (c_int, [P, P, P, P, P, P, P, P, I64, I64, P, P, P, I64, I64, c_int, P, I64, P]),
     "op_gemm_nt_batched": (c_int, [P, I64, I64, P, I64, I64, P, I64, P, I64, I64, I64, I64, I64, I64, P]),
     "op_audio_conv1_ln_gelu_fwd": (c_int, [P, I64, P, P, P, P, P, P, P, I64, I64, c_float, P]),
     "op_audio_conv1_ln_gelu_bwd_workspace_bytes": (I64, [I64]),
@@ -299,7 +301,7 @@
 
 
 def layernorm_bwd(dy, x, w, b, mean, rstd, gelu=False, need_wgrad=True, dw=None, db=None, accumulate=False, add=None,
-                  dx=None, x_rows=None):
+                  dx=None, x_rows=None, live=None):
     rows, cols = x.shape
     if x_rows is not None:
         assert dx is not None and dx.shape == x.shape and (add is None or add.shape == x.shape) and x_rows.dtype == torch.int32
@@ -316,6 +318,16 @@
         ws = workspace(lib().op_layernorm_bwd_workspace_bytes(rows, cols), x.device, "ln")
     else:
         dw = db = None
+    if live is not None:
+        assert not gelu and x_rows is None and x.dtype == torch.bfloat16
+        ns = len(live)
+        i64 = lambda vals: (c_int64 * ns)(*[int(v) for v in vals])
+        for ps, _, _, B in live:
+            assert ps is None or (ps.dtype == torch.float32 and ps.is_contiguous() and ps.numel() >= B and ps.device == x.device)
+        _check(lib().op_layernorm_bwd_live(ptr(dy), ptr(x), ptr(w), ptr(mean), ptr(rstd), ptr(add), ptr(dx), ptr(dw), ptr(db), ptr(ws), rows,
+                                           cols, int(accumulate), ns, _ptr_array([q[0] for q in live], ns), i64([q[1] for q in live]),
+                                           i64([q[2] for q in live]), i64([q[3] for q in live]), stream()), "op_layernorm_bwd_live")
+        return dx, dw, db
     _check(lib().op_layernorm_bwd(ptr(dy), ptr(x), ptr(w), ptr(b), ptr(mean), ptr(rstd), ptr(add), ptr(dx), ptr(dw), ptr(db),
                                   ptr(ws), rows, cols, int(gelu), int(accumulate), _dt(x), ptr(x_rows), stream()), "op_layernorm_bwd")
     return dx, dw, db
@@ -638,7 +650,7 @@
     return dgamma
 
 
-def ln_geglu_bwd(dy, h0, h1, w, mean, rstd, dw=None, db=None, accumulate=False, need_wgrad=True, dh0=None, dh1=None):
+def ln_geglu_bwd(dy, h0, h1, w, mean, rstd, dw=None, db=None, accumulate=False, need_wgrad=True, dh0=None, dh1=None, live=None):
     rows, cols = h0.shape
     if dh0 is None:
         dh0, dh1 = torch.empty_like(h0), torch.empty_like(h1)
@@ -651,6 +663,13 @@
         ws = workspace(lib().op_layernorm_bwd_workspace_bytes(rows, cols), h0.device, "ln")
     else:
         dw = db = None
+    if live is not None:
+        ps, S = live
+        assert ps.dtype == torch.float32 and ps.is_contiguous() and rows % S == 0 and ps.numel() >= rows // S and ps.device == h0.device
+        _check(lib().op_ln_geglu_bwd_live(ptr(dy), ptr(h0), ptr(h1), ptr(w), ptr(mean), ptr(rstd), ptr(dh0), ptr(dh1), dh0.stride(0),
+                                          h0.stride(0), ptr(dw), ptr(db), ptr(ws), rows, cols, int(accumulate), ptr(ps), S, stream()),
+               "op_ln_geglu_bwd_live")
+        return dh0, dh1, dw, db
     _check(lib().op_ln_geglu_bwd(ptr(dy), ptr(h0), ptr(h1), ptr(w), ptr(mean), ptr(rstd), ptr(dh0), ptr(dh1), dh0.stride(0),
                                  h0.stride(0), ptr(dw), ptr(db), ptr(ws), rows, cols, int(accumulate), stream()), "op_ln_geglu_bwd")
     return dh0, dh1, dw, db
diff --git a/one-peace_amd/ops.py b/one-peace_amd/ops.py
--- a/one-peace_amd/ops.py
+++ b/one-peace_amd/ops.py
@@ -222,6 +222,7 @@
 
 GROUPED_WGRAD = os.environ.get("ONEPEACE_GROUPED_WGRAD", "1") != "0"
 SKIP_ZERO_BACKWARD = os.environ.get("ONEPEACE_SKIP_ZERO_BACKWARD", "1") != "0"
+SKIP_ZERO_DGRAD = os.environ.get("ONEPEACE_SKIP_ZERO_DGRAD", "1") != "0"
 
 
 def _live_ktiles(segs, probs, device):
@@ -984,6 +985,7 @@
         kt1 = None
         if rowscale is not None and kept is None and N % rps == 0 and not any(sg.pad for sg in segs) and sum(sg.rows for sg in segs) == N:
             kt1 = _live_ktiles([(rowscale, 0, rps, N // rps)], [(0, N)], dx_mid.device)[0]
+        live1 = [(rowscale, 0, rps, N // rps)] if kt1 is not None and SKIP_ZERO_DGRAD else None
         if ctx.dg_fused:
             g0 = torch.empty(H, dtype=torch.float32, device=dx_mid.device)
             dy1 = _resid_backward(dx_mid, None, P["g1"], rowscale, rps, "g1", "bo", direct, G, needs, g0=g0, rows=xmap)
@@ -1004,7 +1006,7 @@
                 want = needs["aln_w"] or needs["aln_b"]
                 (tw, tb), acc = _targets(direct, "aln_w", "aln_b") if want else ((None, None), False)
                 dattn, dw_, db_ = hip.layernorm_bwd(daln, A["attn"], P["aln_w"], P["aln_b"], A["mean_a"], A["rstd_a"], dw=tw, db=tb,
-                                                    accumulate=acc, need_wgrad=want)
+                                                    accumulate=acc, need_wgrad=want, live=live1)
                 if want:
                     _finish(direct, G, ("aln_w", "aln_b"), (dw_, db_), acc)
             else:
@@ -1054,7 +1056,7 @@
                 (tw, tb), acc = _targets(direct, "ln1_w", "ln1_b") if want else ((None, None), False)
                 dx, dw_, db_ = hip.layernorm_bwd(dxln1, x2, P["ln1_w"], P["ln1_b"], A["mean1"], A["rstd1"], add=dx_mid, dw=tw, db=tb,
                                                  accumulate=acc, need_wgrad=want, dx=torch.empty_like(dx_full) if mapped else None,
-                                                 x_rows=xmap)
+                                                 x_rows=xmap, live=live1)
                 if want:
                     _finish(direct, G, ("ln1_w", "ln1_b"), (dw_, db_), acc)
         if dx is None and need_x:
@@ -1252,6 +1254,7 @@
         kts = [None] * nseg
         if kept is None and not any(sg.pad for sg in segs):
             kts = _live_ktiles([(pss[i], sg.row0, sg.S, sg.B) for i, sg in enumerate(segs)], [(sg.row0, sg.rows) for sg in segs], dev)
+        live2 = SKIP_ZERO_DGRAD and not fp8b and all(kt is not None for kt in kts)
         for i, sg in enumerate(segs):
             r = slice(sg.row0, sg.end)
             k = lambda n: "%s@%d" % (n, i)
@@ -1284,7 +1287,8 @@
                 want = needs[k("fln_w")] or needs[k("fln_b")]
                 (tw, tb2), acc = _targets(direct, k("fln_w"), k("fln_b")) if want else ((None, None), False)
                 _, _, dw_, db2_ = hip.ln_geglu_bwd(dgln[r], A["h0"][r], A["h1"][r], P[k("fln_w")], A["mean_f"][r], A["rstd_f"][r], dw=tw,
-                                                   db=tb2, accumulate=acc, need_wgrad=want, dh0=dpart[pair[0]], dh1=dpart[pair[1]])
+                                                   db=tb2, accumulate=acc, need_wgrad=want, dh0=dpart[pair[0]], dh1=dpart[pair[1]],
+                                                   live=(pss[i], sg.S) if live2 and pss[i] is not None else None)
                 if want:
                     _finish(direct, G, (k("fln_w"), k("fln_b")), (dw_, db2_), acc)
             else:
@@ -1316,7 +1320,8 @@
             want = needs["ln2_w"] or needs["ln2_b"]
             (tw, tb), acc = _targets(direct, "ln2_w", "ln2_b") if want else ((None, None), False)
             dx, dw_, db_ = hip.layernorm_bwd(dxln2, x2, P["ln2_w"], P["ln2_b"], A["mean2"], A["rstd2"], add=dout, dw=tw, db=tb,
-                                             accumulate=acc, need_wgrad=want, dx=torch.empty_like(dout_full) if mapped else None, x_rows=xmap)
+                                             accumulate=acc, need_wgrad=want, dx=torch.empty_like(dout_full) if mapped else None, x_rows=xmap,
+                                             live=[(pss[i], sg.row0, sg.S, sg.B) for i, sg in enumerate(segs)] if live2 else None)
             if want:
                 _finish(direct, G, ("ln2_w", "ln2_b"), (dw_, db_), acc)
         if dx is None and need_x:
```
